# nanoporetech/scrappie

Measured on AMD Instinct MI355X. Metric: raw samples/sec, rgrgr_r94 4k-sample reads, higher is better.
Workload: dtype f32 (3xf16 split products, 22-bit operands, fp32 accumulate)

## Files before the change

### scrappie_amd/csrc/scrappie_hip.hip

```cpp
#include <hip/hip_runtime.h>
#include <sched.h>

#include <algorithm>
#include <atomic>
#include <cmath>
#include <cstdarg>
#include <cstdio>
#include <cstdlib>
#include <cstring>
#include <mutex>
#include <numeric>
#include <string>
#include <thread>
#include <type_traits>
#include <vector>
#include <chrono>
#include <condition_variable>
#include <deque>
#include <functional>
#include <map>
#include <memory>

#include "scrappie_hip.h"
#include "sh_internal.h"
// ... 223 lines not shown
        return tot;
    }
    bool create_events() {
        bool ok = true;
        for (auto &x : ev) ok &= hipEventCreate(&x) == hipSuccess;
        for (hipEvent_t *x : {&done, &kdone, &hdone, &pdone, &up}) ok &= hipEventCreateWithFlags(x, hipEventDisableTiming) == hipSuccess;
        return ok;
    }
    ~Slot() {
        for (auto &x : ev) if (x) (void)hipEventDestroy(x);
        for (hipEvent_t x : {done, kdone, hdone, pdone, up}) if (x) (void)hipEventDestroy(x);
    }
};

struct AltInput {
    const float *data = nullptr;
    std::vector<uint64_t> off;
    DBuf d_off;
    uint64_t key = 0; bool valid = false;
    explicit operator bool() const { return data != nullptr; }
    int set(const char *who, const float *d, const uint64_t *o, size_t n) {
        valid = false;
        if (!d) { data = nullptr; off.clear(); return 0; }
        if (!o || n == 0) return set_err("%s: no offsets", who);
        data = d; off.assign(o, o + n);
        return 0;
    }
};

struct scrappie_hip_engine {
    int device = 0;
    hipStream_t stream = nullptr;
    hipStream_t cstream = nullptr;
    hipStream_t ustream = nullptr;
    hipStream_t pstream = nullptr;
    size_t total_mem = (size_t)64 << 30;
    size_t max_launch_blocks = 0;
    std::vector<Model *> models;
    size_t max_launch_reads = 16384;
    bool profiling = false;
    scrappie_hip_timing timing{};
    bool ev_ok = false;
    Slot slots[2];
    int cur = 0;
    int oldest = 0;
    Slot &current() { return slots[cur]; }
    Slot &other(const Slot &sl) { return slots[&sl == &slots[0] ? 1 : 0]; }
    int index(const Slot &sl) const { return (int)(&sl - slots); }
    bool any_pending() const { return slots[0].pending || slots[1].pending; }
    void drain() {
        (void)sh_stream_wait(pstream); (void)sh_stream_wait(stream); (void)sh_stream_wait(cstream);
        slots[0].pending = slots[1].pending = false;
    }
    DBuf d_hstate, d_vstate, d_vflag;
    DBuf d_act[3];
    DBuf d_xaff, d_E, d_sums, d_tb, d_tbend, d_fstate;
    int ncu = 256;
    bool handover = true;
    AltInput alt_prob; DBuf d_Ealt, d_sums_alt;
    AltInput alt_trunk; DBuf d_act_alt;
    bool dbg_ff_separate = false;
    bool dbg_fv_single = false;
    bool dbg_dump_final = false;
    int dbg_fail_run = 0;
    bool dbg_redo_all = false;
    int dbg_gru_tiles = 0;
    bool dbg_force_f32 = false;
    int dbg_gru32 = -1;
    scrappie_hip_engine *tail = nullptr;
    scrappie_hip_engine *tail2 = nullptr;
    bool is_tail = false;
    int tail_mode = -1;
    int dbg_fail_tail = 0;
    double mem_frac = 0.7;
    struct Blob { std::string name; std::vector<unsigned char> bytes; bool force_f32; };
    std::vector<Blob> blobs;
    unsigned long long n_tail_calls = 0, n_tail_reads = 0;
    struct TailTicket {
        long id = 0; int model = 0; scrappie_hip_params p{};
        std::vector<raw_table> reads; std::vector<scrappie_hip_call> calls;
        std::vector<float> own;
        int rc = 0; std::string err; bool done = false;
    };
    std::thread tail_th, tail_th2;
    bool tail_th_live = false, tail_th2_live = false, tail_stop = false;
    int tail_busy = 0;
    std::mutex tail_mu;
    std::condition_variable tail_cv;
    std::deque<std::shared_ptr<TailTicket>> tail_q;
    std::map<long, std::shared_ptr<TailTicket>> tail_open;
    long tail_next = 1;
    unsigned long long n_redo_tail = 0;
    unsigned long long n_tail_groups = 0;
    unsigned host_thread_budget = 0;
    unsigned long long n_redo = 0;
    struct Carry { bool live = false; int slot = 0; std::vector<uint32_t> perm; scrappie_hip_call *out = nullptr; scrappie_hip_params p{}; } carry;
    std::mutex mu;
    double tail_frac = 0.3;
    double dbg_tail_free_frac = 0;
    BatchCoalescer batch_co;
    ShPresence batch_presence;
    PostStage post_stage[2]; unsigned post_turn = 0;
    HBuf h_dec_in, h_dec_out; DBuf d_dec[7];
    HBuf h_crf_in, h_crf_out; DBuf d_crf[4];
    DpBufs dp_map; DBuf d_map_seq, d_map_band, d_map_post;
    double map_ms[3] = {0, 0, 0};
    DpBufs dp_sq; DBuf d_sq_sig, d_sq_tab;
    double squig_ms[3] = {0, 0, 0};
    DBuf d_sqn[2]; HBuf h_sqn;
    double sqnet_ms[3] = {0, 0, 0};
    DBuf d_ev_sig, d_ev_rd, d_ev_sum, d_ev_sumsq, d_ev_t1, d_ev_t2, d_ev_peaks, d_ev_np, d_ev_off, d_ev_out; HBuf h_ev, h_ev_out;
    double event_ms[3] = {0, 0, 0};
    size_t dbg_events_budget = 0;
    size_t dbg_sqnet_budget = 0;
    size_t dbg_squig_budget = 0;
    std::mutex call_mu;
    ~scrappie_hip_engine() {
        for (Model *m : models) delete m;
        for (hipStream_t st : {stream, cstream, ustream, pstream}) if (st) (void)hipStreamDestroy(st);
// ... 121 lines not shown
```

### scrappie_amd/csrc/sh_decode.h

```cpp
#ifndef SH_DECODE_H
#define SH_DECODE_H

struct ShVitArgs {
    const float *E;
    const float *sums;
    long long strideT;
    int strideQ, strideB;
    int want_log;
    float min_prob, stay_pen, skip_pen, local_pen;
    int use_slip;
    unsigned *tb;
    int *tb_end;
    int *final_state;
    float *final_score;
    float *hp_side;
    const long long *hp_off;
    unsigned long long *dbg;
    const ShGruSegD *seg;
    float *vstate;
    unsigned *flag;
    unsigned *err;
    int dump_final;
};

__device__ __forceinline__ void argmax_merge(float &v, int &i, float ov, int oi) {
    const bool take = (ov > v) | ((ov == v) & (oi < i));
    v = take ? ov : v;
    i = take ? oi : i;
}

__device__ __forceinline__ void rows_argmax(float &bv, int &bi) {
    float ov = __shfl_xor(bv, 16); int oi = __shfl_xor(bi, 16);
    argmax_merge(bv, bi, ov, oi);
    ov = __shfl_xor(bv, 32); oi = __shfl_xor(bi, 32);
    argmax_merge(bv, bi, ov, oi);
}

#ifndef SH_FVT_GAP
#define SH_FVT_GAP 4.76837158203125e-07f
#endif
#ifndef SH_MAX4_ASM
#define SH_MAX4_ASM 1
#endif
__device__ __forceinline__ float d_max4(const f32x4 v) {
#if !SH_MAX4_ASM
    return __builtin_fmaxf(__builtin_fmaxf(v[0], v[1]), __builtin_fmaxf(v[2], v[3]));
#endif
    float t;
    asm("v_max3_f32 %0, %1, %2, %3" : "=v"(t) : "v"(v[0]), "v"(v[1]), "v"(v[2]));
    asm("v_max_f32 %0, %1, %2" : "=v"(t) : "v"(t), "v"(v[3]));
    return t;
}

#define SH_CODE_LT(E, codes, a, b, x)                                                                                       \
    asm("v_cmp_lt_f32 vcc, %1, %2\n\tv_cndmask_b32_sdwa %0, %0, %3, vcc dst_sel:BYTE_" #E                                   \
        " dst_unused:UNUSED_PRESERVE src0_sel:BYTE_" #E " src1_sel:BYTE_0"                                                  \
        : "+v"(codes) : "v"(a), "v"(b), "v"(x) : "vcc")

#ifndef SH_VIT_RING
#define SH_VIT_RING 4
#endif
template <int NTH, int PPT, bool FIN, bool SLIP, bool SKIP0>
__global__ __launch_bounds__(NTH, NTH / 256) void k_viterbi(ShVitArgs a, ShMeta md) {
    constexpr int RING = (PPT >= SH_VIT_RING) ? SH_VIT_RING : PPT;
    constexpr int QSTR = NTH / 16, NW = NTH / 64;
    constexpr int NQ = QSTR * PPT, NH = 4 * NQ;
    constexpr int NSKIP = NH / 16, NSLIP = (NH / 64 > 0) ? NH / 64 : 1;
    extern __shared__ __attribute__((aligned(16))) float smem[];
    float *scA = smem;
    float *scB = scA + NH * 16;
    float *skv = scB + NH * 16;
    int *ski = (int *)(skv + NSKIP * 16);
    float *slv = (float *)(ski + NSKIP * 16);
    int *sli = (int *)(slv + NSLIP * 16);
    float *redv = (float *)(sli + NSLIP * 16);
    int *redi = (int *)(redv + 2 * NW * 16);

    const int tid = threadIdx.x, b = tid & 15, qq = tid >> 4, wave = tid >> 6, lane = tid & 63;
    const float mp = a.min_prob, mpm1 = 1.0f - a.min_prob;
    const float slip_pen = (float)(2.0 * a.skip_pen);
    constexpr bool slip = SLIP && (NH / 64 > 0);
    unsigned long long vA = 0, vB = 0, vC = 0, vD = 0, vt0 = 0, vt1;
    long long vblocks = 0;
#define VSTAMP(acc) do { if (a.dbg) { vt1 = __builtin_readcyclecounter(); acc += vt1 - vt0; vt0 = vt1; } } while (0)

    int tile = blockIdx.x, s0 = 0, s1 = -1, ord = 0;
    if (a.seg) { const ShGruSegD sg = a.seg[blockIdx.x]; tile = sg.tile; s0 = sg.s0; s1 = sg.s1; ord = sg.pad; }
    tile = __builtin_amdgcn_readfirstlane(tile); s0 = __builtin_amdgcn_readfirstlane(s0); s1 = __builtin_amdgcn_readfirstlane(s1);
    const int Tt = __builtin_amdgcn_readfirstlane(md.tile_T[tile]);
    if (s1 < 0) s1 = Tt;
    const long long boff = __builtin_amdgcn_readfirstlane((int)md.tile_boff[tile]);
    const int rd = tile * 16 + b;
    const int myT = md.rT[rd];
    float pstart = 0.0f, pend = -SH_BIG;
    if (s0 == 0) {
#pragma unroll
        for (int i = 0; i < PPT; i++)
            *(f32x4 *)(scA + ((qq + QSTR * i) * 16 + b) * 4) = (f32x4){-SH_BIG, -SH_BIG, -SH_BIG, -SH_BIG};
        if (lane < 16) { redv[wave * 16 + b] = -SH_BIG - a.local_pen; redi[wave * 16 + b] = 4 * wave; }
    } else {
        if (tid == 0) {
            if (!sh_wait_flag(a.flag + tile, (unsigned)ord, a.err)) __hip_atomic_store(a.err, 1u, __ATOMIC_RELAXED, __HIP_MEMORY_SCOPE_AGENT);
        }
        __syncthreads();
        __builtin_amdgcn_fence(__ATOMIC_ACQUIRE, "agent");
        const float *vst = a.vstate + (long long)tile * (NH * 16 + 32);
        float bv = -INFINITY;
        int bi = 0x7fffffff;
#pragma unroll
        for (int i = 0; i < PPT; i++) {
            const int Q = qq + QSTR * i;
            const f32x4 pv = *(const f32x4 *)(vst + (Q * 16 + b) * 4);
            *(f32x4 *)(scA + (Q * 16 + b) * 4) = pv;
            {
                const float ve = __builtin_fmaxf(__builtin_fmaxf(pv[0], pv[1]), __builtin_fmaxf(pv[2], pv[3])) - a.local_pen;
                bi = (ve > bv) ? Q : bi;
                bv = __builtin_fmaxf(bv, ve);
            }
        }
        pstart = vst[NH * 16 + b];
        pend = vst[NH * 16 + 16 + b];
        float ov = __shfl_xor(bv, 16); int oi = __shfl_xor(bi, 16);
        argmax_merge(bv, bi, ov, oi);
        ov = __shfl_xor(bv, 32); oi = __shfl_xor(bi, 32);
        argmax_merge(bv, bi, ov, oi);
        if (lane < 16) { redv[((s0 & 1) * NW + wave) * 16 + b] = bv; redi[((s0 & 1) * NW + wave) * 16 + b] = bi; }
    }
    __syncthreads();
    float *cur = scA, *nxt = scB;

    f32x4 ring[RING];
    float stay_nx = 0.f, sum_nx = 1.f;
    float hp_nx[4] = {0.f, 0.f, 0.f, 0.f};
    const bool hp_lane = FIN && a.hp_side && qq == 0;
    auto fetch = [&](int t) {
        const float *Ecb = a.E + (boff + t) * a.strideT + b * a.strideB;
        stay_nx = Ecb[NQ * a.strideQ];
        if (FIN) sum_nx = a.sums[(boff + t) * 16 + b];
        if (hp_lane) {
#pragma unroll
// ... 259 lines not shown
#define SH_FV_LDS_FLOATS (2 * 1024 * 16 + 2 * 64 * 16 + 2 * 16 * 16 + 4 * 8 * 16 + 2 * 3 * 512 + 2 * 9 * 16 + 65 * 16 + 3 * 2 * 4 * 4)

template <bool SLIP, bool SKIP0, bool DIV>
__global__ __launch_bounds__(512, 2) void k_ff_viterbi(ShFfArgs f, ShVitArgs a, ShMeta md) {
    constexpr int NTH = 512, NW = 8, PPT = 8, NQ = 256, NH = 1024, NSKIP = NH / 16, NSLIP = NH / 64, KS = 3, KQ = 6;
    static_assert(PPT == SH_SUM_GROUP, "a wave's tiles are one row-sum group");
    extern __shared__ __attribute__((aligned(16))) float smem[];
    float *scA = smem;
    float *scB = scA + NH * 16;
    float *skv = scB + NH * 16;
    int *ski = (int *)(skv + NSKIP * 16);
    float *slv = (float *)(ski + NSKIP * 16);
    int *sli = (int *)(slv + NSLIP * 16);
    float *redv = (float *)(sli + NSLIP * 16);
    int *redi = (int *)(redv + 2 * NW * 16);
    unsigned *xp = (unsigned *)(redi + 2 * NW * 16);
    float *gsum = (float *)(xp + 2 * KS * 512);
    float *sBias = gsum + 2 * (NW + 1) * 16;
    unsigned *sStay = (unsigned *)(sBias + 65 * 16);

    const int tid = threadIdx.x, lane = tid & 63, b = lane & 15, q = lane >> 4;
    const int wave = __builtin_amdgcn_readfirstlane(tid >> 6);
    const float mp = a.min_prob, mpm1 = 1.0f - a.min_prob;
    const float slip_pen = (float)(2.0 * a.skip_pen);
    const float lbound = (mp > 0.0f) ? 1.0e-3f - __logf(mp) : INFINITY;
    unsigned long long vA = 0, vB = 0, vC = 0, vD = 0, vt0 = 0, vt1;
#if SH_FV_YOUNG_PRIO
    if (wave >= 4) __builtin_amdgcn_s_setprio(SH_FV_YOUNG_PRIO);
#endif

    const unsigned *wmine = f.wpiece + (long long)(PPT * wave) * KS * 512;
    ShSplit W[2][KS];
    const unsigned lofs = (unsigned)lane * 4u, tofs = (unsigned)lane;
    typedef const __attribute__((address_space(1))) unsigned *gu32;
    typedef const __attribute__((address_space(1))) u32x4 *gu32x4;
    gu32 wp = (gu32)wmine;
    auto w_load = [&](int i) {
        static_assert(KS == 3, "two bases per tile: immediate offsets reach 4095 bytes");
        gu32 b0 = wp, b1 = wp + 1024;
        asm volatile("" : "+s"(b0), "+s"(b1));
        W[i & 1][0].p1 = __builtin_bit_cast(f16x8, *(gu32x4)(b0 + lofs));
        W[i & 1][0].p2 = __builtin_bit_cast(f16x8, *(gu32x4)(b0 + 256 + lofs));
        W[i & 1][1].p1 = __builtin_bit_cast(f16x8, *(gu32x4)(b0 + 512 + lofs));
        W[i & 1][1].p2 = __builtin_bit_cast(f16x8, *(gu32x4)(b0 + 768 + lofs));
        W[i & 1][2].p1 = __builtin_bit_cast(f16x8, *(gu32x4)(b1 + lofs));
        W[i & 1][2].p2 = __builtin_bit_cast(f16x8, *(gu32x4)(b1 + 256 + lofs));
        wp = (i == PPT - 1) ? (gu32)wmine : wp + KS * 512;
        asm volatile("" : "+s"(wp));
    };
    if (tid < KS * 2 * 4 * 4) sStay[tid] = f.wpiece[(long long)(PPT * NW) * KS * 512 + (tid >> 4) * 256 + ((tid >> 2) & 3) * 64 + (tid & 3)];
    for (int j = tid; j < 65 * 16; j += NTH) sBias[j] = f.bfrag[((j >> 4) * 64 + ((j >> 2) & 3) * 16) * 4 + (j & 3)];

    int tile = blockIdx.x, s0 = 0, s1 = -1, ord = 0;
    if (a.seg) { const ShGruSegD sg = a.seg[blockIdx.x]; tile = sg.tile; s0 = sg.s0; s1 = sg.s1; ord = sg.pad; }
    tile = __builtin_amdgcn_readfirstlane(tile); s0 = __builtin_amdgcn_readfirstlane(s0); s1 = __builtin_amdgcn_readfirstlane(s1);
    const int Tt = __builtin_amdgcn_readfirstlane(md.tile_T[tile]);
    if (s1 < 0) s1 = Tt;
    const long long boff = __builtin_amdgcn_readfirstlane((int)md.tile_boff[tile]);
    const int rd = tile * 16 + b;
    const int myT = md.rT[rd];
    const long long hpo = a.hp_side ? a.hp_off[rd] : 0;
    float pstart = 0.0f, pend = -SH_BIG;
    if (s0 == 0) {
#pragma unroll
        for (int i = 0; i < PPT; i++)
            *(f32x4 *)(scA + ((32 * wave + 4 * i + q) * 16 + b) * 4) = (f32x4){-SH_BIG, -SH_BIG, -SH_BIG, -SH_BIG};
        if (lane < 16) { redv[wave * 16 + b] = -SH_BIG - a.local_pen; redi[wave * 16 + b] = 32 * wave; }
    } else {
        if (tid == 0) {
            if (!sh_wait_flag(a.flag + tile, (unsigned)ord, a.err)) __hip_atomic_store(a.err, 1u, __ATOMIC_RELAXED, __HIP_MEMORY_SCOPE_AGENT);
        }
        __syncthreads();
        __builtin_amdgcn_fence(__ATOMIC_ACQUIRE, "agent");
        const float *vst = a.vstate + (long long)tile * (NH * 16 + 32);
        float bv = -INFINITY;
        int bi = 0x7fffffff;
#pragma unroll
        for (int i = 0; i < PPT; i++) {
            const int Q = 32 * wave + 4 * i + q;
            const f32x4 pv = *(const f32x4 *)(vst + (Q * 16 + b) * 4);
            *(f32x4 *)(scA + (Q * 16 + b) * 4) = pv;
            {
                const float ve = __builtin_fmaxf(__builtin_fmaxf(pv[0], pv[1]), __builtin_fmaxf(pv[2], pv[3])) - a.local_pen;
                bi = (ve > bv) ? Q : bi;
                bv = __builtin_fmaxf(bv, ve);
            }
        }
        pstart = vst[NH * 16 + b];
        pend = vst[NH * 16 + 16 + b];
        float ov = __shfl_xor(bv, 16); int oi = __shfl_xor(bi, 16);
        argmax_merge(bv, bi, ov, oi);
        ov = __shfl_xor(bv, 32); oi = __shfl_xor(bi, 32);
        argmax_merge(bv, bi, ov, oi);
        if (lane < 16) { redv[((s0 & 1) * NW + wave) * 16 + b] = bv; redi[((s0 & 1) * NW + wave) * 16 + b] = bi; }
    }
    float *cur = scA, *nxt = scB;

    f32x4 xr0 = {0.f, 0.f, 0.f, 0.f}, xr1 = xr0;
    auto xraw_load = [&](int t) {
        if (wave < KS) {
            const float *p = f.in + ((boff + min(t, s1 - 1)) * KQ + 2 * wave) * 256;
            xr0 = *(const f32x4 *)(p + lofs);
            xr1 = *(const f32x4 *)(p + 256 + lofs);
        }
    };
    auto xp_publish = [&](int buf) {
        if (wave < KS) {
// ... 476 lines not shown
```

### scrappie_amd/csrc/sh_decode_teams.h

```cpp
#ifndef SH_DECODE_TEAMS_H
#define SH_DECODE_TEAMS_H

#ifndef SH_FVT_WBUF
#define SH_FVT_WBUF 3
#endif
#ifndef SH_FVT_PROD_PRIO
#define SH_FVT_PROD_PRIO 1
#endif
#ifndef SH_FVT_ABL
#define SH_FVT_ABL 0
#endif
#ifndef SH_FVT_FLIP
#define SH_FVT_FLIP 3
#endif
#ifndef SH_FVT_STAMP
#ifdef SH_EXPERIMENTS
#define SH_FVT_STAMP 1
#else
#define SH_FVT_STAMP 0
#endif
#endif
__device__ __forceinline__ unsigned long long end_key(float v, int i) {
    const unsigned u = __builtin_bit_cast(unsigned, v);
    const unsigned hi = u ^ ((unsigned)((int)u >> 31) | 0x80000000u);
    return ((unsigned long long)hi << 32) | (unsigned)~i;
}
__device__ __forceinline__ void end_unkey(unsigned long long k, float &v, int &i) {
    const unsigned hi = (unsigned)(k >> 32);
    v = __builtin_bit_cast(float, hi ^ (~(unsigned)((int)hi >> 31) | 0x80000000u));
    i = (int)~(unsigned)k;
}

#define SH_FVT_NTH 768
#define SH_FVT_LDS_FLOATS (1024 * 16 + 64 * 256 + 2 * 64 * 16 + 2 * 2 * 8 * 16 + 4 * 9 * 16 + 65 * 16 + 2 * 3 * 512 + 3 * 2 * 4 * 4)

template <bool SKIP0, bool DIV, bool NOCLAMP = false>
__global__ __launch_bounds__(SH_FVT_NTH) void k_ff_viterbi_teams(ShFfArgs f, ShVitArgs a, ShMeta md) {
    static_assert(!(DIV && NOCLAMP), "with temperatures the clamp stays");
    constexpr int NCW = 8, NPW = 4, PPT = 8, NQ = 256, NH = 1024, KS = 3, KQ = 6, TPP = 16, HT = 8, NG = 9, WB = SH_FVT_WBUF;
    static_assert(SH_SUM_GROUP == HT, "half a pass of a producer is one row-sum group");
    static_assert(WB >= 2 && WB <= 4, "weight ring");
    extern __shared__ __attribute__((aligned(16))) float smem[];
    float *sc = smem;
    float *ring = sc + NH * 16;
    float *skk = ring + 64 * 256;
    float *redv = skk + 2 * 64 * 16;
    int *redi = (int *)(redv + 2 * NCW * 16);
    typedef __attribute__((address_space(3))) unsigned long long *ldsk;
    ldsk redk = (ldsk)redv;
    float *gsum = (float *)(redi + 2 * NCW * 16);
    float *sBias = gsum + 4 * NG * 16;
    unsigned *xp = (unsigned *)(sBias + 65 * 16);
    unsigned *sStay = xp + 2 * KS * 512;

    const int tid = threadIdx.x, lane = tid & 63, b = lane & 15, q = lane >> 4;
    const int wave = __builtin_amdgcn_readfirstlane(tid >> 6);
    const bool decoder = wave < NCW;
    const float mp = a.min_prob, mpm1 = 1.0f - a.min_prob;
    const float lbound = (mp > 0.0f) ? 1.0e-3f - __logf(mp) : INFINITY;
    const float lbgap = lbound * SH_FVT_GAP;
    unsigned long long vA = 0, vB = 0, vC = 0, vD = 0, vt0 = 0, vt1 = 0;
    (void)vt0; (void)vt1;
#undef VSTAMP
#if SH_FVT_STAMP
#define VSTAMP(acc) do { if (a.dbg) { vt1 = __builtin_readcyclecounter(); acc += vt1 - vt0; vt0 = vt1; } } while (0)
#else
#define VSTAMP(acc) do { } while (0)
#endif

    if (tid < KS * 2 * 4 * 4) sStay[tid] = f.wpiece[(long long)(64) * KS * 512 + (tid >> 4) * 256 + ((tid >> 2) & 3) * 64 + (tid & 3)];
    for (int j = tid; j < 65 * 16; j += SH_FVT_NTH) sBias[j] = f.bfrag[((j >> 4) * 64 + ((j >> 2) & 3) * 16) * 4 + (j & 3)];

    int tile = blockIdx.x, s0 = 0, s1 = -1, ord = 0;
    if (a.seg) { const ShGruSegD sg = a.seg[blockIdx.x]; tile = sg.tile; s0 = sg.s0; s1 = sg.s1; ord = sg.pad; }
    tile = __builtin_amdgcn_readfirstlane(tile); s0 = __builtin_amdgcn_readfirstlane(s0); s1 = __builtin_amdgcn_readfirstlane(s1);
    const int Tt = __builtin_amdgcn_readfirstlane(md.tile_T[tile]);
    if (s1 < 0) s1 = Tt;
    const long long boff = __builtin_amdgcn_readfirstlane((int)md.tile_boff[tile]);
    const int rd = tile * 16 + b;
    int myT = md.rT[rd];
    asm volatile("" : "+v"(myT));
    const long long hpo = a.hp_side ? a.hp_off[rd] : 0;
    float pstart = 0.0f, pend = -SH_BIG;

    const int cw = decoder ? wave : 0;
    float *myq = sc + cw * 256 + lane * 4;
    const float *mye = ring + cw * 512 + lane * 4;
    const float *mysrc = sc + cw * 64 + b * 4 + q;
#define SH_FVT_MT(i) (16 * ((i) >> 1) + 8 * ((i) & 1))

    if (s0 == 0) {
        if (decoder) {
#pragma unroll
            for (int i = 0; i < PPT; i++) *(f32x4 *)(myq + SH_FVT_MT(i) * 256) = (f32x4){-SH_BIG, -SH_BIG, -SH_BIG, -SH_BIG};
            if (wave == 0 && lane < 16) { redk[b] = end_key(-SH_BIG - a.local_pen, 0); redk[16 + b] = 0; }
        }
    } else {
        if (tid < 32) redk[tid] = 0;
        if (tid == 0) {
            if (!sh_wait_flag(a.flag + tile, (unsigned)ord, a.err)) __hip_atomic_store(a.err, 1u, __ATOMIC_RELAXED, __HIP_MEMORY_SCOPE_AGENT);
        }
        __syncthreads();
        __builtin_amdgcn_fence(__ATOMIC_ACQUIRE, "agent");
        if (decoder) {
            const float *vst = a.vstate + (long long)tile * (NH * 16 + 32);
            float bv = -INFINITY;
            int bi = 0x7fffffff;
#pragma unroll
            for (int i = 0; i < PPT; i++) {
                const int Q = 4 * (SH_FVT_MT(i) + cw) + q;
                const f32x4 pv = *(const f32x4 *)(vst + (Q * 16 + b) * 4);
                *(f32x4 *)(myq + SH_FVT_MT(i) * 256) = pv;
                {
                    const float ve = __builtin_fmaxf(__builtin_fmaxf(pv[0], pv[1]), __builtin_fmaxf(pv[2], pv[3])) - a.local_pen;
                    bi = (ve > bv) ? Q : bi;
                    bv = __builtin_fmaxf(bv, ve);
                }
            }
            pstart = vst[NH * 16 + b];
            pend = vst[NH * 16 + 16 + b];
            float ov = __shfl_xor(bv, 16); int oi = __shfl_xor(bi, 16);
            argmax_merge(bv, bi, ov, oi);
            ov = __shfl_xor(bv, 32); oi = __shfl_xor(bi, 32);
            argmax_merge(bv, bi, ov, oi);
            if (lane < 16) __hip_atomic_fetch_max(redk + b, end_key(bv, bi), __ATOMIC_RELAXED, __HIP_MEMORY_SCOPE_WORKGROUP);
        }
    }
// ... 437 lines not shown
```

### scrappie_amd/csrc/sh_eng_batch.inc

```

#ifndef SH_CHAIN_NS
#define SH_CHAIN_NS 11400.0
#endif
#ifndef SH_WORK_NS
#define SH_WORK_NS 3.5
#endif
extern "C" long scrappie_hip_plan_tail(const uint32_t *lengths, size_t n, int stride, size_t max_long_blocks, unsigned char *is_long) {
    if ((!lengths && n) || stride < 1 || !is_long) return -1;
    memset(is_long, 0, n);
    if (n < 2) return 0;
    double W = 0;
    std::vector<uint32_t> T(n);
    for (size_t i = 0; i < n; i++) { T[i] = (uint32_t)(((unsigned long long)lengths[i] + stride - 1) / stride); W += T[i]; }
    const double thr = std::max(4096.0, W * SH_WORK_NS / SH_CHAIN_NS);
    std::vector<uint32_t> cand;
    for (size_t i = 0; i < n; i++) if ((double)T[i] > thr) cand.push_back((uint32_t)i);
    if (cand.empty() || cand.size() == n) return 0;
    std::stable_sort(cand.begin(), cand.end(), [&](uint32_t a, uint32_t b) { return T[a] > T[b]; });
    double blocks = 0, work = 0;
    long cnt = 0;
    for (size_t k = 0; k < cand.size(); k++) {
        if (k % 16 == 0) { if (max_long_blocks && blocks + T[cand[k]] > (double)max_long_blocks) break; blocks += T[cand[k]]; }
        if (work + T[cand[k]] > 0.15 * W) break;
        work += T[cand[k]];
        is_long[cand[k]] = 1; cnt++;
    }
    return cnt;
}

static int basecall_batch_one(scrappie_hip_engine *e, int model, const raw_table *reads, size_t n, const scrappie_hip_params *p, scrappie_hip_call *out);

static bool tail_two_helpers();
static double tail_mem_frac() {
    static const double f = [] { const char *v = getenv("SCRAPPIE_HIP_TAIL_MEM"); const double x = v ? atof(v) : 0; return x > 0 && x <= 0.4 ? x : (tail_two_helpers() ? 0.15 : 0.3); }();
    return f;
}
static bool tail_two_helpers() {
    static const bool on = [] { const char *v = getenv("SCRAPPIE_HIP_TAIL"); return v && atoi(v) == 2; }();
    return on;
}
static bool tail_enabled(const scrappie_hip_engine *e) {
    if (e->is_tail) return false;
    if (e->tail_mode >= 0) return e->tail_mode != 0;
    static const bool env_on = [] { const char *v = getenv("SCRAPPIE_HIP_TAIL"); return !(v && atoi(v) == 0); }();
    return env_on;
}

static scrappie_hip_engine *make_helper(scrappie_hip_engine *e) {
    scrappie_hip_engine *t = scrappie_hip_engine_create(e->device);
    if (!t) return nullptr;
    t->is_tail = true;
    for (const auto &b : e->blobs) {
        t->dbg_force_f32 = b.force_f32;
        const int want = scrappie_hip_find_model(e, b.name.c_str());
        if (load_model_mem_one(t, b.name.c_str(), b.bytes.data(), b.bytes.size()) != want) { scrappie_hip_engine_destroy(t); set_err("helper engine: model '%s' did not load at index %d", b.name.c_str(), want); return nullptr; }
    }
    return t;
}
static void sync_helper(scrappie_hip_engine *e, scrappie_hip_engine *t) {
    t->handover = e->handover; t->max_launch_reads = e->max_launch_reads; t->max_launch_blocks = e->max_launch_blocks;
    t->dbg_ff_separate = e->dbg_ff_separate; t->dbg_fv_single = e->dbg_fv_single; t->dbg_gru32 = e->dbg_gru32; t->dbg_gru_tiles = e->dbg_gru_tiles; t->dbg_redo_all = e->dbg_redo_all;
    t->profiling = false;
}
static scrappie_hip_engine *tail_engine(scrappie_hip_engine *e) {
    if (!e->tail) {
        (void)hipSetDevice(e->device);
        double frac = tail_mem_frac();
        size_t fr = 0, tot = 0;
        if (hipMemGetInfo(&fr, &tot) == hipSuccess && e->total_mem) frac = std::min(frac, 0.85 * (double)fr / (double)e->total_mem);
        if (e->dbg_tail_free_frac > 0) frac = std::min(frac, e->dbg_tail_free_frac);
        if (frac < 0.03) { e->tail_mode = 0; return nullptr; }
        e->tail = make_helper(e);
        if (!e->tail) return nullptr;
        e->mem_frac = 0.45; e->tail->mem_frac = frac; e->tail_frac = frac;
    }
    std::lock_guard<std::mutex> lk(e->tail_mu);
    if (e->tail_busy == 0) {
        sync_helper(e, e->tail);
        if (e->tail2) sync_helper(e, e->tail2);
        if (e->dbg_fail_tail) { e->tail->dbg_fail_run = e->dbg_fail_tail; e->dbg_fail_tail = 0; }
    }
    return e->tail;
}

typedef std::shared_ptr<scrappie_hip_engine::TailTicket> TicketPtr;
static void tail_worker(scrappie_hip_engine *e, scrappie_hip_engine *helper) {
    for (;;) {
        std::unique_lock<std::mutex> lk(e->tail_mu);
        e->tail_cv.wait(lk, [&] { return e->tail_stop || !e->tail_q.empty(); });
        if (e->tail_q.empty()) break;
        std::vector<TicketPtr> batch;
        const TicketPtr f = e->tail_q.front();
        while (!e->tail_q.empty() && e->tail_q.front()->model == f->model && memcmp(&e->tail_q.front()->p, &f->p, sizeof f->p) == 0) {
            batch.push_back(e->tail_q.front());
            e->tail_q.pop_front();
        }
        e->tail_busy++;
        lk.unlock();
        std::vector<raw_table> all;
        for (const TicketPtr &t : batch) all.insert(all.end(), t->reads.begin(), t->reads.end());
        std::vector<scrappie_hip_call> calls(all.size());
        const int rc = basecall_batch_one(helper, f->model, all.data(), all.size(), &f->p, calls.data());
        const std::string err = rc ? std::string(g_err) : std::string();
        lk.lock();
        size_t at = 0;
        for (const TicketPtr &t : batch) {
            t->rc = rc; t->err = err;
            if (!rc) t->calls.assign(calls.begin() + (long)at, calls.begin() + (long)(at + t->reads.size()));
            at += t->reads.size();
            t->done = true;
        }
        e->n_tail_groups++;
        e->n_redo_tail += helper->n_redo; helper->n_redo = 0;
        e->tail_busy--;
// ... 442 lines not shown
```

### scrappie_amd/csrc/sh_eng_debug.inc

```

extern "C" int scrappie_hip_set_decoder_input(scrappie_hip_engine *e, const float *d_prob, const uint64_t *prob_off, size_t n_prob) {
    if (!e) return set_err("set_decoder_input: null engine");
    if (e->any_pending()) return set_err("set_decoder_input: launch groups are in flight");
    return e->alt_prob.set("set_decoder_input", d_prob, prob_off, n_prob);
}

extern "C" int scrappie_hip_set_trunk_input(scrappie_hip_engine *e, const float *d_trunk, const uint64_t *trunk_off, size_t n_trunk) {
    if (!e) return set_err("set_trunk_input: null engine");
    if (e->any_pending()) return set_err("set_trunk_input: launch groups are in flight");
    return e->alt_trunk.set("set_trunk_input", d_trunk, trunk_off, n_trunk);
}

extern "C" int scrappie_hip_debug_option(scrappie_hip_engine *e, const char *name, int value) {
    if (!e || !name) return set_err("debug_option: null argument");
    if (e->any_pending()) return set_err("debug_option: launch groups are in flight");
    if (!strcmp(name, "ff_separate")) e->dbg_ff_separate = value != 0;
    else if (!strcmp(name, "fv_single")) e->dbg_fv_single = value != 0;
    else if (!strcmp(name, "dump_final")) e->dbg_dump_final = value != 0;
    else if (!strcmp(name, "fail_run")) e->dbg_fail_run = value;
    else if (!strcmp(name, "redo_all")) e->dbg_redo_all = value != 0;
    else if (!strcmp(name, "gru_tiles")) e->dbg_gru_tiles = value;
    else if (!strcmp(name, "force_f32_layers")) e->dbg_force_f32 = value != 0;
#ifdef SH_EXPERIMENTS
    else if (!strcmp(name, "gru32")) e->dbg_gru32 = value;
#endif
    else if (!strcmp(name, "tail")) e->tail_mode = value;
    else if (!strcmp(name, "fail_tail")) e->dbg_fail_tail = value;
    else if (!strcmp(name, "tail_free_frac")) e->dbg_tail_free_frac = value / 1000.0;
    else if (!strcmp(name, "squiggle_budget_kb")) e->dbg_squig_budget = value > 0 ? (size_t)value << 10 : 0;
    else if (!strcmp(name, "sqnet_budget_kb")) e->dbg_sqnet_budget = value > 0 ? (size_t)value << 10 : 0;
    else if (!strcmp(name, "events_budget_samples")) e->dbg_events_budget = value > 0 ? (size_t)value : 0;
    else return set_err("debug_option: unknown option '%s'", name);
    return 0;
}

extern "C" long long scrappie_hip_debug_fetch(scrappie_hip_engine *e, const char *what, void *dst, size_t nbytes) {
    if (!e || !what) return set_err("debug_fetch: null argument");
    (void)hipSetDevice(e->device);
    HIPCHK(sh_stream_wait(e->stream));
    HIPCHK(sh_stream_wait(e->cstream));
    const Slot &sl = e->current(); const LaunchGroup &lg = sl.lg;
    if (!lg.valid) return set_err("debug_fetch: no launch group has run");
    Model *m = get_model(e, lg.model);
    if (!m) return -1;
    const size_t NH = (size_t)std::max(m->NS - 1, 0);
    const void *src = nullptr; size_t have = 0; bool host = false;
    const int gru_tiles = lg.gru_two ? 2 : 1;
    if (!strcmp(what, "tb")) { src = e->d_tb.p; have = (size_t)lg.ncb * NH * 16; }
    else if (!strcmp(what, "tb_end")) { src = e->d_tbend.p; have = (size_t)lg.ncb * 16 * 4; }
    else if (!strcmp(what, "final_state")) { src = e->d_fstate.p; have = lg.npad * 4; }
    else if (!strcmp(what, "final_score")) { src = sl.d_fscore.p; have = lg.npad * 4; }
    else if (!strcmp(what, "final_scores")) { src = e->d_vstate.p; have = lg.ntile * (NH * 16 + 32) * 4; }
    else if (!strcmp(what, "order")) { src = lg.order.data(); have = lg.npad * 4; host = true; }
    else if (!strcmp(what, "tile_boff")) { src = lg.tile_boff.data(); have = lg.ntile * 8; host = true; }
    else if (!strcmp(what, "n_redo")) { static thread_local unsigned long long tot; tot = e->n_redo + e->n_redo_tail; src = &tot; have = 8; host = true; }
    else if (!strcmp(what, "n_tail_groups")) { src = &e->n_tail_groups; have = 8; host = true; }
    else if (!strcmp(what, "n_tail_calls")) { src = &e->n_tail_calls; have = 8; host = true; }
    else if (!strcmp(what, "n_tail_reads")) { src = &e->n_tail_reads; have = 8; host = true; }
    else if (!strcmp(what, "gru_tiles")) { src = &gru_tiles; have = 4; host = true; }
    else if (!strcmp(what, "pinned_bytes")) {
        static thread_local unsigned long long tot;
        tot = e->slots[0].pinned_bytes() + e->slots[1].pinned_bytes();
        src = &tot; have = 8; host = true;
    }
    else return set_err("debug_fetch: unknown buffer '%s'", what);
    if (!src && have) return set_err("debug_fetch: buffer '%s' was not allocated", what);
    const size_t cnt = std::min(have, nbytes);
    if (dst && cnt) {
        if (host) memcpy(dst, src, cnt);
        else HIPCHK(hipMemcpy(dst, src, cnt, hipMemcpyDeviceToHost));
    }
    return (long long)have;
}

// ... 48 lines not shown
```

### scrappie_amd/csrc/sh_eng_launch.inc

```

struct MetaPtrs { ShMeta md; const long long *seq_off, *hp_off, *bases_off; ShGruLanes lanes, lanes1; ShGruPairs pairs, pairs2; const ShGruSegD *vseg; };

static int build_group(scrappie_hip_engine *e, Slot &sl, Model *m, const uint64_t *offsets, const uint32_t *lengths,
                       size_t n, bool hp_on, MetaPtrs &mp) {
    LaunchGroup &lg = sl.lg;
    lg.valid = false;
    lg.n = n; lg.hp_on = hp_on;
    lg.ntile = (n + 15) / 16; lg.npad = lg.ntile * 16;
    const int st = m->stride;
    std::vector<int> T(n);
    for (size_t i = 0; i < n; i++)
        T[i] = (lengths[i] >= m->min_samples) ? (int)((lengths[i] + st - 1) / st) : 0;
    lg.order.assign(lg.npad, -1);
    std::vector<int> idx(n);
    std::iota(idx.begin(), idx.end(), 0);
    std::stable_sort(idx.begin(), idx.end(), [&](int a, int b) { return T[a] > T[b]; });
    for (size_t i = 0; i < n; i++) lg.order[i] = idx[i];
    lg.rT.assign(lg.npad, 0); lg.rN.assign(lg.npad, 0);
    lg.seq_off.assign(lg.npad, 0); lg.hp_off.assign(lg.npad, 0); lg.bases_off.assign(lg.npad, 0);
    long long nbases = 0;
    const long long per_entry = (m->arch == 1) ? 1 : 5;
    std::vector<unsigned long long> sig_off(lg.npad, 0);
    std::vector<int> tile_T(lg.ntile, 0);
    std::vector<long long> &tile_boff = lg.tile_boff;
    tile_boff.assign(lg.ntile, 0);
    long long ncb = 0, nseq = 0, nhp = 0;
    for (size_t i = 0; i < lg.npad; i++) {
        const int o = lg.order[i];
        if (o >= 0 && T[o] > 0) {
            lg.rT[i] = T[o]; lg.rN[i] = (int)lengths[o]; sig_off[i] = offsets[o];
        }
        lg.hp_off[i] = nhp; nhp += lg.rT[i];
        lg.bases_off[i] = nbases; nbases += lg.rT[i] ? ((per_entry * ((long long)lg.rT[i] + 1) + 16 + 15) & ~15ll) : 0;
        tile_T[i >> 4] = std::max(tile_T[i >> 4], lg.rT[i]);
    }
    for (size_t t = 0; t < lg.ntile; t++) { tile_boff[t] = ncb; ncb += tile_T[t]; }
    for (size_t t = 0; t < lg.ntile; t++) {
        for (int b = 0; b < 16; b++) lg.seq_off[t * 16 + b] = nseq + b;
        nseq += tile_T[t] ? ((long long)tile_T[t] + 1) * SH_SEQ_STRIDE : 0;
    }
    lg.ncb = ncb; lg.nseq = nseq; lg.nhp = nhp; lg.nbases_cap = nbases;
    ShGruSchedule sched;
    sh_lane_schedule(tile_T.data(), lg.ntile, e->ncu, 2, sched, e->handover);
    lg.gru_nwg = sched.nwg;
    ShGruSchedule sched1;
    sh_lane_schedule(tile_T.data(), lg.ntile, e->ncu, 1, sched1, e->handover);
    lg.gru1_nwg = sched1.nwg;
    { long long nlive = 0; int tmax = 0; for (int t : tile_T) { nlive += t > 0; tmax = std::max(tmax, t); }
      const int w1 = sched1.wg_iter.empty() ? 0 : *std::max_element(sched1.wg_iter.begin(), sched1.wg_iter.end());
      const int w2 = sched.wg_iter.empty() ? 0 : *std::max_element(sched.wg_iter.begin(), sched.wg_iter.end());
      lg.gru_two = nlive > e->ncu && tmax < 65536 && (double)w2 * tun().gru_two_ratio < (double)w1;
      if (e->dbg_gru_tiles == 1) lg.gru_two = false;
      if (e->dbg_gru_tiles == 2 && tmax < 65536) lg.gru_two = true; }
    std::vector<int> pair_tile, pair_T;
    for (size_t t = 0; t < lg.ntile; ) {
        const bool two = t + 1 < lg.ntile && tile_T[t] < (1 << 18) && tile_T[t + 1] > 0;
        pair_tile.push_back((int)t); pair_tile.push_back(two ? (int)t + 1 : -1);
        pair_T.push_back(std::max(tile_T[t], two ? tile_T[t + 1] : 0));
        t += two ? 2 : 1;
    }
    ShGruSchedule sched32;
    sh_lane_schedule(pair_T.data(), pair_T.size(), e->ncu, 1, sched32, e->handover);
    lg.gru32_nwg = sched32.nwg;
    ShGruSchedule sched32b;
    sh_lane_schedule(pair_T.data(), pair_T.size(), e->ncu, 2, sched32b, e->handover);
    lg.gru32x2_nwg = sched32b.nwg;
    std::vector<ShGruSeg> vseg;
    sh_piece_schedule(tile_T.data(), lg.ntile, e->ncu, vseg, e->handover);
    lg.vit_nwg = (int)vseg.size();
    const size_t b_u64 = lg.npad * 8, b_i32 = lg.npad * 4;
    const size_t b_loff = sched.lane_off.size() * 4, b_seg = sched.seg.size() * sizeof(ShGruSeg), b_wit = sched.wg_iter.size() * 4;
    const size_t b_vloff = 0, b_vseg = vseg.size() * sizeof(ShGruSeg);
    const size_t b_loff1 = sched1.lane_off.size() * 4, b_seg1 = sched1.seg.size() * sizeof(ShGruSeg);
    const size_t b_loff32 = sched32.lane_off.size() * 4, b_seg32 = sched32.seg.size() * sizeof(ShGruSeg), b_pt = pair_tile.size() * 4;
    const size_t b_loff32b = sched32b.lane_off.size() * 4, b_seg32b = sched32b.seg.size() * sizeof(ShGruSeg);
    const size_t total = 4 * b_u64 + lg.ntile * 8 + 2 * b_i32 + lg.ntile * 4 + 16 + b_seg + b_loff + b_wit + 16 + b_vseg + b_vloff + 16 + b_seg1 + b_loff1 +
                         16 + b_seg32 + b_loff32 + b_pt + 16 + b_seg32b + b_loff32b;
    if (sl.h_meta.ensure(total + 16) || sl.d_meta.ensure(total + 16)) return -1;
    char *h = sl.h_meta.as<char>();
    size_t o = 0;
    memcpy(h + o, sig_off.data(), b_u64); const size_t o_sig = o; o += b_u64;
    memcpy(h + o, lg.seq_off.data(), b_u64); const size_t o_seq = o; o += b_u64;
    memcpy(h + o, lg.hp_off.data(), b_u64); const size_t o_hp = o; o += b_u64;
    memcpy(h + o, lg.bases_off.data(), b_u64); const size_t o_bs = o; o += b_u64;
    memcpy(h + o, tile_boff.data(), lg.ntile * 8); const size_t o_tb = o; o += lg.ntile * 8;
    memcpy(h + o, lg.rN.data(), b_i32); const size_t o_n = o; o += b_i32;
    memcpy(h + o, lg.rT.data(), b_i32); const size_t o_t = o; o += b_i32;
    memcpy(h + o, tile_T.data(), lg.ntile * 4); const size_t o_tt = o; o += lg.ntile * 4;
    o = (o + 15) & ~(size_t)15;
    memcpy(h + o, sched.seg.data(), b_seg); const size_t o_seg = o; o += b_seg;
    memcpy(h + o, sched.lane_off.data(), b_loff); const size_t o_loff = o; o += b_loff;
    memcpy(h + o, sched.wg_iter.data(), b_wit); const size_t o_wit = o; o += b_wit;
    o = (o + 15) & ~(size_t)15;
    memcpy(h + o, vseg.data(), b_vseg); const size_t o_vseg = o; o += b_vseg;
    o = (o + 15) & ~(size_t)15;
    memcpy(h + o, sched1.seg.data(), b_seg1); const size_t o_seg1 = o; o += b_seg1;
    memcpy(h + o, sched1.lane_off.data(), b_loff1); const size_t o_loff1 = o; o += b_loff1;
    o = (o + 15) & ~(size_t)15;
    memcpy(h + o, sched32.seg.data(), b_seg32); const size_t o_seg32 = o; o += b_seg32;
    memcpy(h + o, sched32.lane_off.data(), b_loff32); const size_t o_loff32 = o; o += b_loff32;
    memcpy(h + o, pair_tile.data(), b_pt); const size_t o_pt = o; o += b_pt;
    o = (o + 15) & ~(size_t)15;
    memcpy(h + o, sched32b.seg.data(), b_seg32b); const size_t o_seg32b = o; o += b_seg32b;
    memcpy(h + o, sched32b.lane_off.data(), b_loff32b); const size_t o_loff32b = o; o += b_loff32b;
    hipStream_t ps = e->ev_ok ? e->pstream : e->stream;
    if (e->ev_ok) {
        const long long n16 = (long long)((total + 15) / 16);
        hipLaunchKernelGGL(k_upload_words, dim3((unsigned)std::min<long long>((n16 + 255) / 256, 64)), dim3(256), 0, ps, (const u32x4 *)h, sl.d_meta.as<u32x4>(), n16);
    } else HIPCHK(hipMemcpyAsync(sl.d_meta.p, h, total, hipMemcpyHostToDevice, ps));
    char *d = sl.d_meta.as<char>();
    mp.md.sig_off = (const unsigned long long *)(d + o_sig);
    mp.seq_off = (const long long *)(d + o_seq);
    mp.hp_off = (const long long *)(d + o_hp);
    mp.bases_off = (const long long *)(d + o_bs);
    mp.md.tile_boff = (const long long *)(d + o_tb);
    mp.md.rN = (const int *)(d + o_n);
    mp.md.rT = (const int *)(d + o_t);
    mp.md.tile_T = (const int *)(d + o_tt);
    static_assert(sizeof(ShGruSeg) == sizeof(ShGruSegD), "segment layout");
    mp.lanes.seg = (const ShGruSegD *)(d + o_seg);
    mp.lanes.lane_off = (const int *)(d + o_loff);
    mp.lanes.wg_iter = (const int *)(d + o_wit);
    mp.lanes.ntile = (int)lg.ntile;
    mp.vseg = (const ShGruSegD *)(d + o_vseg);
    if (e->d_hstate.ensure(std::max<size_t>(lg.ntile, 1) * 12 * 256 * 4) || sl.d_gflag.ensure((lg.ntile + 1) * 4)) return -1;
    mp.lanes.hstate = e->d_hstate.as<float>();
    mp.lanes.flag = sl.d_gflag.as<unsigned>();
    HIPCHK(hipMemsetAsync(sl.d_gflag.p, 0, (lg.ntile + 1) * 4, ps));
    if (sl.d_bad.ensure(lg.npad * 4)) return -1;
    HIPCHK(hipMemsetAsync(sl.d_bad.p, 0, lg.npad * 4, ps));
    mp.lanes1 = mp.lanes;
    mp.lanes1.seg = (const ShGruSegD *)(d + o_seg1);
    mp.lanes1.lane_off = (const int *)(d + o_loff1);
    mp.lanes1.wg_iter = nullptr;
    mp.pairs.seg = (const ShGruSegD *)(d + o_seg32);
    mp.pairs.lane_off = (const int *)(d + o_loff32);
    mp.pairs.pair_tile = (const int *)(d + o_pt);
    mp.pairs.hstate = mp.lanes.hstate;
    mp.pairs.flag = mp.lanes.flag;
    mp.pairs.err = mp.lanes.flag + lg.ntile;
    mp.pairs2 = mp.pairs;
    mp.pairs2.seg = (const ShGruSegD *)(d + o_seg32b);
    mp.pairs2.lane_off = (const int *)(d + o_loff32b);
    return 0;
}

template <int KQ>
static int launch_affine_k(hipStream_t s, const float *in, float *out, const float *wf, const unsigned *wp, const float *bf,
                           long long ncb, int mtiles) {
    const int mt = pick_mt(mtiles);
    long long gx = std::min<long long>((ncb + 3) / 4, 2048);
    if (gx < 1) gx = 1;
    dim3 grid((unsigned)gx, (unsigned)(mtiles / mt));
    int rc = 0;
    if (pick_int<6, 4, 3, 2, 1>(mt, rc, [&](auto m) { return launch_k<k_affine<KQ, m()>>(grid, dim3(256), 0, s, in, out, wf, wp, bf, ncb, mtiles); })) return rc;
    return set_err("unsupported layer of %d m-tiles", mtiles);
}

template <int KQ>
static int launch_affine_lds_k(hipStream_t s, const float *in, float *out, const float *wf, const unsigned *wp, const float *bf,
                               long long ncb, int mtiles) {
    constexpr int NB = SH_AFF_NB, NTH = SH_AFF_NTH;
    const size_t lds = ((size_t)mtiles * KQ * 256 + (size_t)mtiles * 256) * 4 + 16;
    long long gx = std::min<long long>((ncb + (NTH / 64) * NB - 1) / ((NTH / 64) * NB), 256);
    if (gx < 1) gx = 1;
    return launch_k<k_affine_lds<KQ, NB, NTH>>(dim3((unsigned)gx), dim3(NTH), lds, s, in, out, wf, wp, bf, ncb, mtiles);
}

template <int KQ>
static int launch_affine_f32_k(hipStream_t s, const float *in, float *out, const float *wf, const float *bf, long long ncb, int mtiles) {
    const int mt = (mtiles % 6 == 0) ? 6 : (mtiles % 2 == 0) ? 2 : 1;
    long long gx = std::min<long long>((ncb + 3) / 4, 2048);
    if (gx < 1) gx = 1;
    dim3 grid((unsigned)gx, (unsigned)(mtiles / mt));
    int rc = 0;
    if (pick_int<6, 2, 1>(mt, rc, [&](auto m) { return launch_k<k_affine<KQ, m(), true>>(grid, dim3(256), 0, s, in, out, wf, (const unsigned *)nullptr, bf, ncb, mtiles); })) return rc;
    return set_err("unsupported layer of %d m-tiles", mtiles);
}

static int launch_affine(hipStream_t s, int K, const float *in, float *out, const float *wf, const unsigned *wp, const float *bf_nat,
                         const float *bf_acc, long long ncb, int mtiles, bool force_f32 = false) {
    int rc = 0;
    if (force_f32 && pick_int<2, 4, 6, 8>(K / 16, rc, [&](auto kq) { return launch_affine_f32_k<kq()>(s, in, out, wf, bf_nat, ncb, mtiles); })) return rc;
    if (K % 32 == 0 && (!wp || !bf_acc)) return set_err("layer weights were not cut into pieces (input size %d)", K);
    const float *bf = (K % 32 == 0) ? bf_acc : bf_nat;
    const size_t lds_need = ((size_t)mtiles * (K / 16) * 256 + (size_t)mtiles * 256) * 4;
    if (mtiles >= 12 && lds_need <= 150 * 1024 && ncb >= 4096 && !tun().affine_reg &&
        pick_int<1, 2, 4, 6>(K / 16, rc, [&](auto kq) { return launch_affine_lds_k<kq()>(s, in, out, wf, wp, bf, ncb, mtiles); })) return rc;
    if (pick_int<1, 2, 4, 6, 8>(K / 16, rc, [&](auto kq) { return launch_affine_k<kq()>(s, in, out, wf, wp, bf, ncb, mtiles); })) return rc;
    return set_err("unsupported layer input size %d (need 16, 32, 64, 96 or 128)", K);
}

template <int KQ>
static int launch_affine2_k(hipStream_t s, const float *inF, const float *inB, float *out, const unsigned *wF, const unsigned *wB,
                            const float *bf, long long ncb, int mtiles) {
    long long gx = std::min<long long>((ncb + 3) / 4, 2048);
    if (gx < 1) gx = 1;
    const int mt = mtiles / 2;
    int rc = 0;
    if (mt * 2 == mtiles &&
        pick_int<3, 2, 1>(mt, rc, [&](auto m) { return launch_k<k_affine2_tanh<KQ, m()>>(dim3((unsigned)gx), dim3(512), 0, s, inF, inB, out, wF, wB, bf, ncb, mtiles); })) return rc;
    return set_err("unsupported joining layer of %d m-tiles", mtiles);
}

static int launch_affine2(hipStream_t s, int K, const float *inF, const float *inB, float *out, const unsigned *wF, const unsigned *wB,
                          const float *bf, long long ncb, int mtiles) {
    int rc = 0;
    if (pick_int<2, 4, 6>(K / 16, rc, [&](auto kq) { return launch_affine2_k<kq()>(s, inF, inB, out, wF, wB, bf, ncb, mtiles); })) return rc;
    return set_err("unsupported bi-GRU size %d (need 32, 64 or 96)", K);
}

static int launch_gru(hipStream_t s, int S, const float *xaff, float *out, const float *resid, const float *sW,
                      const float *sW2, const unsigned *sWp, const unsigned *sW2p, const ShMeta &md, int backward, size_t ntile, const ShGruLanes &lanes, int nwg,
                      bool force_f32 = false) {
    const int NU = S / 16;
    int rc = 0;
    if (!tun().gru_single && !tun().gru_stamp && tun().gru_debug < 0 && NU <= 6 && S % 32 == 0) {
        if (nwg <= 0) return 0;
        HIPCHK(hipMemsetAsync(lanes.flag, 0, (size_t)lanes.ntile * 4, s));
        dim3 lgrid((unsigned)nwg);
        const bool stamp = tun().gru_lanes_stamp;
        const bool f32_env = tun().gru_f32 || force_f32;
        if (!stamp && !f32_env) {
            const size_t plds = (size_t)2 * 2 * (NU / 2) * 2 * 64 * 4 * 4;
            if (pick_int<2, 4, 6>(NU, rc, [&](auto nu) { return launch_k<k_gru_split<nu()>>(lgrid, dim3(128 * nu()), plds, s, xaff, out, resid, sWp, sW2p, md, backward, lanes); })) return rc;
            return set_err("unsupported GRU size %d (need 32, 64 or 96 here)", S);
        }
        const size_t lds = (size_t)2 * 2 * NU * 256 * 4;
        static StampBuf st;
        if (!pick_int<2, 4, 6>(NU, rc, [&](auto nu) {
#ifdef SH_EXPERIMENTS
            if constexpr (nu() == 6)
                if (stamp) return launch_k<k_gru_lanes<6, true>>(lgrid, dim3(768), lds, s, xaff, out, resid, sW, sW2, md, backward, lanes, st.dev(4096 * 16 * 8));
#endif
            return launch_k<k_gru_lanes<nu(), false>>(lgrid, dim3(128 * nu()), lds, s, xaff, out, resid, sW, sW2, md, backward, lanes, (unsigned long long *)nullptr);
            })) return set_err("unsupported GRU size %d (need 32, 64 or 96 here)", S);
        if (stamp && NU == 6)
            st.dump_on(7, s, (size_t)nwg * 12 * 8, [&](const unsigned long long *h) {
                for (size_t g : {(size_t)nwg / 2}) for (int w = 0; w < 12; w++) {
                    const unsigned long long *d = &h[(g * 12 + w) * 8];
                    fprintf(stderr, "gru lanes stamp wg %zu wave %2d: phase1 %.0f bar %.0f phase2 %.0f bar %.0f cycles/step (%llu steps)\n",
                            g, w, d[0] / (double)d[4], d[1] / (double)d[4], d[2] / (double)d[4], d[3] / (double)d[4], d[4]);
                }
            });
        return rc;
    }
    if (tun().gru_debug >= 0) backward |= tun().gru_debug << 8;
    static StampBuf st1;
    unsigned long long *dbgbuf = tun().gru_stamp ? st1.dev(4096 * 8 * 8) : nullptr;
    if (dbgbuf)
        st1.dump_on(8, s, ntile * NU * 8, [&](const unsigned long long *h) {
            { unsigned long long first_end = ~0ull, mn = ~0ull, mx = 0; size_t late = 0;
              for (size_t tl = 0; tl < ntile; tl++) { first_end = std::min(first_end, h[tl * NU * 8 + 7]); mn = std::min(mn, h[tl * NU * 8 + 6]); mx = std::max(mx, h[tl * NU * 8 + 7]); }
              for (size_t tl = 0; tl < ntile; tl++) if (h[tl * NU * 8 + 6] >= first_end) late++;
              fprintf(stderr, "residency: %zu tiles, %zu started after the first one finished; span %.1f us\n", ntile, late, (mx - mn) / 100.0); }
            for (size_t tl : {size_t(0)}) for (int w = 0; w < 1; w++) {
                const unsigned long long *d = &h[(tl * NU + w) * 8];
                fprintf(stderr, "stamp tile %zu wave %d: rgemm %.0f zgemm+valu %.0f bar1 %.0f gemm2+valu %.0f bar2 %.0f (cycles/step)\n", tl, w, d[0] / (double)d[5], d[1] / (double)d[5], d[2] / (double)d[5], d[3] / (double)d[5], d[4] / (double)d[5]);
            }
        });
    if (pick_int<2, 4, 6, 8>(NU, rc, [&](auto nu) { return launch_k<k_gru<nu()>>(dim3((unsigned)ntile), dim3(64 * nu()), 0, s, xaff, out, resid, sW, sW2, md, backward, dbgbuf); })) return rc;
    return set_err("unsupported GRU size %d (need 32, 64, 96 or 128)", S);
}

#ifndef SH_FFL_NB
#define SH_FFL_NB 3
#endif
#ifndef SH_FFL_NTH
#define SH_FFL_NTH 512
#endif
static int ff_mtp(int KQ, int mtiles) {
    const size_t per_mt = ((size_t)KQ * 256 + 256) * 4;
// ... 25 lines not shown
}

static int launch_ff(hipStream_t s, int S, const float *in, float *E, float *sums, const unsigned *wf, const float *bf,
                     long long ncb, int mtiles, int NS, float in_div, float out_div, int ncu) {
    int rc = 0;
    if (ncb >= 8192 && !tun().ff_reg &&
        pick_int<2, 4, 6>(S / 16, rc, [&](auto kq) { return launch_ff_lds_k<kq()>(s, in, E, sums, wf, bf, ncb, mtiles, NS, in_div, out_div, ncu); })) return rc;
    constexpr int NB = SH_FF_NB;
    const int mtp = ff_mtp(S / 16, mtiles);
    const long long gx = (ncb + 4 * NB - 1) / (4 * NB);
    dim3 grid((unsigned)std::max<long long>(gx, 1));
    if (pick_int<2, 4, 6, 8>(S / 16, rc, [&](auto kq) {
            constexpr int KQ = kq();
            return pick_bool([&](auto dv) { return launch_k<k_ff_exp<KQ, NB, dv()>>(grid, dim3(256), 0, s, in, E, sums, wf, bf, ncb, mtiles, mtp, NS, in_div, out_div); },
                             out_div != 1.0f);
        })) return rc;
    return set_err("unsupported size %d", S);
}

static bool gru_proj_ok(int K, int S) { return K == S && S % 32 == 0 && S / 16 <= 6; }

static bool conv_edge_words(const ShConvGeom &g, int N, int T, int out[4]) {
    out[0] = out[1] = out[2] = out[3] = 0;
    if (T <= 0) return true;
    unsigned irr = 0;
    bool ok = true;
    for (int t = std::max(g.c0, T - 64); t < T; t++) {
        const int kk = (t - g.c0) / g.nstepC, ii = (t - g.c0) - kk * g.nstepC;
        if (!((kk + 1) * g.nstepX <= N - g.shiftX - ii * g.st)) {
            const int j = T - 1 - t;
            if (j >= 32) ok = false; else irr |= 1u << j;
        }
    }
    const int maxCol = (N - g.shiftX) / g.nstepX;
    const int rem = (N - g.shiftX) % g.nstepX;
    const int colR = g.c0 + g.nstepC * (maxCol - 1) + rem / g.st + 1;
    const int startR = g.st - (g.padL + N - g.WL) % g.st - 1;
    out[0] = (int)irr; out[1] = colR + startR / g.st; out[2] = startR; out[3] = N;
    return ok;
}

extern "C" int scrappie_hip_conv_edge_words(int WL, int st, int F, int N, int out[4]) {
    if (WL < 1 || st < 1 || N < 1 || !out) return -1;
    return conv_edge_words(conv_geom(WL, st, F), N, (N + st - 1) / st, out) ? 1 : 0;
}

#ifdef SH_EXPERIMENTS
static int launch_gru_conv(hipStream_t s, int kst, int act, float *out, const unsigned *iW, const float *ib, const unsigned *sW,
                           const unsigned *sW2, const ShMeta &md, int backward, const ShGruLanes &lanes1, int nwg1,
                           const ShGruLanes &lanes2, int nwg2, bool two, const ShConvFuse &cf) {
    const ShGruLanes &lanes = two ? lanes2 : lanes1;
    const int nwg = two ? nwg2 : nwg1;
    if (nwg <= 0) return 0;
    HIPCHK(hipMemsetAsync(lanes.flag, 0, (size_t)lanes.ntile * 4, s));
    const size_t lds = (two ? 2 : 1) * ((size_t)4 * 3 * 2 * 64 * 4 + (size_t)2 * 3 * 6 * 256) * 4;
    dim3 grid((unsigned)nwg);
    if (tun().proj_stamp && two && kst == 3 && !act) {
        static StampBuf st;
        if (launch_k<k_gru_conv_stamp<2, 3, 0>>(grid, dim3(768), lds, s, out, iW, ib, sW, sW2, md, backward, lanes, cf, st.dev(1024 * 12 * 16))) return -1;
        st.dump_on(3, s, (size_t)nwg * 12 * 16, [&](const unsigned long long *h) {
            for (int w = 0; w < 12; w++) {
                const unsigned long long *d = &h[((size_t)(nwg / 2) * 12 + w) * 16];
                fprintf(stderr, "conv-layer stamp wave %2d (%s): A %.0f bar %.0f B %.0f bar %.0f cycles per double step (%llu steps); chunk+fetch part of B (projection) / reads+MFMA issue (recurrence) %.0f\n", w,
                        w < 6 ? "recurrence" : "projection", d[0] / (double)d[4], d[1] / (double)d[4], d[2] / (double)d[4], d[3] / (double)d[4], d[4], d[5] / (double)d[4]);
            }
        });
        return 0;
    }
    return pick_bool([&](auto t2, auto k3, auto ac) {
        return launch_k<k_gru_conv<t2() ? 2 : 1, k3() ? 3 : 5, ac() ? 1 : 0>>(grid, dim3(768), lds, s, out, iW, ib, sW, sW2, md, backward, lanes, cf);
    }, two, kst == 3, act != 0);
}
#endif
static int launch_gru_proj(hipStream_t s, int S, const float *in, float *out, const float *resid, const unsigned *iW, const float *ib,
                           const unsigned *sW, const unsigned *sW2, const ShMeta &md, int backward, const ShGruLanes &lanes1, int nwg1,
                           const ShGruLanes &lanes2, int nwg2, bool two) {
    const ShGruLanes &lanes = two ? lanes2 : lanes1;
    const int nwg = two ? nwg2 : nwg1;
    if (nwg <= 0) return 0;
    HIPCHK(hipMemsetAsync(lanes.flag, 0, (size_t)lanes.ntile * 4, s));
    const int NU = S / 16;
    size_t lds = (two ? 2 : 1) * ((size_t)4 * (NU / 2) * 2 * 64 * 4 + (size_t)2 * 3 * NU * 256) * 4;
    if (resid && SH_RESID_LDS && lds + (size_t)(two ? 2 : 1) * 3 * NU * 256 * 4 <= 160 * 1024) lds += (size_t)(two ? 2 : 1) * 3 * NU * 256 * 4;
    dim3 grid((unsigned)nwg);
    unsigned long long *const no_dbg = nullptr;
    int rc = 0;
#ifdef SH_EXPERIMENTS
    static const bool mx_on = [] { const char *v = getenv("SH_GRU_MX"); return v && atoi(v) != 0; }();
    if (mx_on && NU == 6 && two) {
        static const bool mx_stamp = getenv("SH_MX_STAMP") != nullptr;
        if (mx_stamp && !resid) {
            static StampBuf st;
            if (launch_k<k_gru_mx<false, true>>(grid, dim3(1024), lds, s, in, out, resid, iW, ib, sW, sW2, md, backward, lanes, st.dev((size_t)1024 * 16 * 10))) return -1;
            st.dump_on(7, s, (size_t)nwg * 16 * 10, [&](const unsigned long long *hb) {
                for (int w = 0; w < 16; w++) {
                    const unsigned long long *d = &hb[((size_t)(nwg / 2) * 16 + w) * 10];
                    const double n = (double)std::max<unsigned long long>(d[8], 1);
                    fprintf(stderr, "mx stamp wave %2d (%s): P1 %.0f +bar %.0f | P2 %.0f +bar %.0f | P3 %.0f +bar %.0f | P4 %.0f +bar %.0f cycles per double step (%llu steps)\n", w,
                            w < 6 ? "recurrence " : w < 12 ? "projection " : "elementwise", d[0] / n, d[1] / n, d[2] / n, d[3] / n, d[4] / n, d[5] / n, d[6] / n, d[7] / n, d[8]);
                }
            });
            return 0;
        }
        if (pick_bool([&](auto rs) { return launch_k<k_gru_mx<rs()>>(grid, dim3(1024), lds, s, in, out, resid, iW, ib, sW, sW2, md, backward, lanes, no_dbg); }, resid != nullptr))
            return -1;
        HIPCHK(hipGetLastError());
        return 0;
    }
    const bool stamp = tun().proj_stamp && NU == 6 && two && !resid;
    const bool free_run = SH_GRU_FREE_DEFAULT ? !tun().gru_barrier : tun().gru_free;
    if (free_run) {
        const size_t flds = (two ? 2 : 1) * ((size_t)4 * (NU / 2) * 2 * 64 * 4 + (size_t)3 * 3 * NU * 256) * 4 + 64;
        if (stamp) {
            static StampBuf st;
            if (launch_k<k_gru_free<6, 2, false, true>>(grid, dim3(768), flds, s, in, out, resid, iW, ib, sW, sW2, md, backward, lanes, st.dev(1024 * 12 * 16))) return -1;
            st.dump_on(7, s, (size_t)nwg * 12 * 16, [&](const unsigned long long *h) {
                for (int w = 0; w < 12; w++) {
                    const unsigned long long *d = &h[((size_t)(nwg / 2) * 12 + w) * 16];
                    if (w < 6) fprintf(stderr, "free stamp wave %2d (recurrence): work %.0f, waiting for gate inputs %.0f, for r*h of all waves %.0f, for h of all waves %.0f cycles per double step (%llu steps)\n",
                                       w, d[0] / (double)d[4], d[1] / (double)d[4], d[2] / (double)d[4], d[3] / (double)d[4], d[4]);
                    else fprintf(stderr, "free stamp wave %2d (projection): work %.0f, waiting for the column's pieces %.0f, for a free ring slot %.0f cycles per double step (%llu steps)\n",
                                 w, d[0] / (double)d[4], d[1] / (double)d[4], d[2] / (double)d[4], d[4]);
                }
            });
            return 0;
        }
        if (pick_int<2, 4, 6>(NU, rc, [&](auto nu) {
                constexpr int N = nu();
                return pick_bool([&](auto t2, auto rs) {
                    return launch_k<k_gru_free<N, t2() ? 2 : 1, rs(), false>>(grid, dim3(128 * N), flds, s, in, out, resid, iW, ib, sW, sW2, md, backward, lanes, no_dbg);
                }, two, resid != nullptr);
            })) return rc;
        return set_err("unsupported GRU size %d (need 32, 64 or 96 here)", S);
    }
    if (stamp) {
        static StampBuf st;
        if (launch_k<k_gru_proj<6, 2, false, true>>(grid, dim3(768), lds, s, in, out, resid, iW, ib, sW, sW2, md, backward, lanes, st.dev(1024 * 12 * 16))) return -1;
        st.dump_on(7, s, (size_t)nwg * 12 * 16, [&](const unsigned long long *h) {
            for (int w = 0; w < 12; w++) {
                const unsigned long long *d = &h[((size_t)(nwg / 2) * 12 + w) * 16];
                fprintf(stderr, "proj stamp wave %2d (%s): A %.0f bar %.0f B %.0f bar %.0f cycles per double step (%llu steps)", w, w < 6 ? "recurrence" : "projection",
                        d[0] / (double)d[4], d[1] / (double)d[4], d[2] / (double)d[4], d[3] / (double)d[4], d[4]);
                if (w < 6) fprintf(stderr, "; inside B: reads+MFMA issue %.0f, logistic z %.0f, tanh+blend %.0f, store+bookkeeping %.0f, cut+publish %.0f",
                                   d[5] / (double)d[4], d[6] / (double)d[4], d[7] / (double)d[4], d[8] / (double)d[4], d[9] / (double)d[4]);
                fprintf(stderr, "\n");
            }
        });
        return 0;
    }
#endif
    if (pick_int<2, 4, 6>(NU, rc, [&](auto nu) {
            constexpr int N = nu();
            return pick_bool([&](auto t2) {
                constexpr int NT = t2() ? 2 : 1;
                if (resid) return launch_k<k_gru_proj_res<N, NT>>(grid, dim3(128 * N), lds, s, in, out, resid, iW, ib, sW, sW2, md, backward, lanes);
                return launch_k<k_gru_proj<N, NT, false>>(grid, dim3(128 * N), lds, s, in, out, resid, iW, ib, sW, sW2, md, backward, lanes, no_dbg);
            }, two);
        })) return rc;
    return set_err("unsupported GRU size %d (need 32, 64 or 96 here)", S);
}

#ifdef SH_EXPERIMENTS
#ifndef SH_GRU32_DEFAULT
#define SH_GRU32_DEFAULT 0
#endif
static int use_gru32(const scrappie_hip_engine *e) {
    if (e->dbg_gru32 >= 0) return e->dbg_gru32;
    if (SH_GRU32_DEFAULT ? tun().gru16 : !tun().gru32) return 0;
    const char *v = getenv("SH_GRU32");
    return (v && atoi(v) == 2) ? 2 : (SH_GRU32_DEFAULT ? SH_GRU32_DEFAULT : 1);
}
static const char *const g32_role[8] = {"R0 chain", "R1 chain", "R2 chain", "C cand-proj", "G0 z/r", "G1 z/r", "G2 z/r", "L loader"};
static int launch_gru_proj32x2(hipStream_t s, const float *in, float *out, bool resid, const unsigned *iW, const float *ib, const unsigned *sW,
                               const unsigned *sW2, const ShMeta &md, int backward, const ShGruPairs &pairs, int nwg, size_t ntile) {
    if (nwg <= 0) return 0;
    HIPCHK(hipMemsetAsync(pairs.flag, 0, ntile * 4, s));
    const size_t lds = (size_t)SH_G32X2_LDS_WORDS * 4;
    dim3 grid((unsigned)nwg);
    if (tun().gru32_stamp && !resid) {
        static StampBuf st;
        if (launch_k<k_gru_proj32x2<false, true>>(grid, dim3(512), lds, s, in, out, iW, ib, sW, sW2, md, backward, pairs, st.dev(1024 * 8 * 16))) return -1;
        st.dump_on(7, s, (size_t)nwg * 8 * 16, [&](const unsigned long long *h) {
            for (int w = 0; w < 8; w++) {
                const unsigned long long *d = &h[((size_t)(nwg / 2) * 8 + w) * 16];
                fprintf(stderr, "gru32x2 stamp wave %d (%s): work %.0f bar %.0f cycles per interval (%llu intervals = one tile-step of 32 reads each)\n", w, g32_role[w],
                        d[0] / (double)d[4], d[1] / (double)d[4], d[4]);
            }
        });
        return 0;
    }
    return pick_bool([&](auto rs) { return launch_k<k_gru_proj32x2<rs(), false>>(grid, dim3(512), lds, s, in, out, iW, ib, sW, sW2, md, backward, pairs, (unsigned long long *)nullptr); }, resid);
}
static int launch_gru_proj32(hipStream_t s, const float *in, float *out, bool resid, const unsigned *iW, const float *ib, const unsigned *sW,
                             const unsigned *sW2, const ShMeta &md, int backward, const ShGruPairs &pairs, int nwg, size_t ntile) {
    if (nwg <= 0) return 0;
    HIPCHK(hipMemsetAsync(pairs.flag, 0, ntile * 4, s));
    const size_t lds = (size_t)SH_G32_LDS_WORDS * 4;
    dim3 grid((unsigned)nwg);
    if (tun().gru32_stamp && !resid) {
        static StampBuf st;
        if (launch_k<k_gru_proj32<false, true>>(grid, dim3(512), lds, s, in, out, iW, ib, sW, sW2, md, backward, pairs, st.dev(1024 * 8 * 16))) return -1;
        st.dump_on(7, s, (size_t)nwg * 8 * 16, [&](const unsigned long long *h) {
            for (int w = 0; w < 8; w++) {
                const unsigned long long *d = &h[((size_t)(nwg / 2) * 8 + w) * 16];
                fprintf(stderr, "gru32 stamp wave %d (%s): A %.0f bar %.0f B %.0f bar %.0f cycles per step (%llu steps)", w, g32_role[w],
                        d[0] / (double)d[4], d[1] / (double)d[4], d[2] / (double)d[4], d[3] / (double)d[4], d[4]);
                if (w < 3) fprintf(stderr, "; A: reads+r products %.0f, logistic*h %.0f, cut+write %.0f; B: reads+candidate products %.0f, z/tanh/blend %.0f, store %.0f, cut+write %.0f",
                                   d[5] / (double)d[4], d[6] / (double)d[4], d[7] / (double)d[4], d[8] / (double)d[4], d[9] / (double)d[4], d[10] / (double)d[4], d[11] / (double)d[4]);
                fprintf(stderr, "\n");
            }
        });
        return 0;
    }
    return pick_bool([&](auto rs) { return launch_k<k_gru_proj32<rs(), false>>(grid, dim3(512), lds, s, in, out, iW, ib, sW, sW2, md, backward, pairs, (unsigned long long *)nullptr); }, resid);
}

#endif
static int launch_lstm(hipStream_t s, int S, const float *xaff, float *out, const unsigned *sW, const float *pf,
                       const ShMeta &md, int backward, const ShGruLanes &lanes, int nwg) {
    if (nwg <= 0) return 0;
    HIPCHK(hipMemsetAsync(lanes.flag, 0, (size_t)lanes.ntile * 4, s));
    int rc = 0;
    if (pick_int<2, 4, 6>(S / 16, rc, [&](auto nu) { return launch_k<k_lstm_lanes<nu()>>(dim3((unsigned)nwg), dim3(128 * nu()), 0, s, xaff, out, sW, pf, md, backward, lanes); })) return rc;
    return set_err("unsupported LSTM size %d (need 32, 64 or 96)", S);
}

static int launch_lstm_proj(hipStream_t s, int S, int I, const float *in, float *out, const unsigned *iW, const float *ib,
                            const unsigned *sW, const float *pf, const ShMeta &md, int backward, const ShGruLanes &lanes, int nwg) {
    if (nwg <= 0) return 0;
    HIPCHK(hipMemsetAsync(lanes.flag, 0, (size_t)lanes.ntile * 4, s));
    const int NU = S / 16;
    const size_t lds = ((size_t)4 * (NU / 2) * 2 * 64 * 4 + (size_t)2 * 4 * NU * 256 + (size_t)3 * NU * 256) * 4;
    if (I != S && I != 16) return set_err("unsupported LSTM input width %d", I);
    int rc = 0;
    if (pick_int<2, 4, 6>(NU, rc, [&](auto nu) {
            constexpr int N = nu();
            return pick_bool([&](auto wide) { return launch_k<k_lstm_proj<N, wide() ? N : 1>>(dim3((unsigned)nwg), dim3(128 * N), lds, s, in, out, iW, ib, sW, pf, md, backward, lanes); },
                             I == S);
        })) return rc;
    return set_err("unsupported LSTM size %d (need 32, 64 or 96)", S);
}

static size_t viterbi_lds_bytes(int NH) {
    const int nskip = NH / 16, nslip = std::max(NH / 64, 1);
    return (size_t)NH * 16 * 4 * 2 + (size_t)nskip * 16 * 8 + (size_t)nslip * 16 * 8 + 2 * 16 * 16 * 8;
}

static int launch_viterbi(hipStream_t s, int NH, const ShVitArgs &a, const ShMeta &md, size_t nwg) {
    const size_t lds = viterbi_lds_bytes(NH);
    if (nwg == 0) return 0;
    const bool fin = a.sums != nullptr, slip = a.use_slip != 0, skip0 = a.skip_pen == 0.0f;
    if (fin && !a.want_log) return set_err("decode: exp-value input implies log output");
    const auto go = [&](auto nth, auto ppt) {
        constexpr int NTH = nth(), PPT = ppt();
        return pick_bool([&](auto fi, auto sl, auto sk) { return launch_k<k_viterbi<NTH, PPT, fi(), sl(), sk()>>(dim3((unsigned)nwg), dim3(NTH), lds, s, a, md); },
                         fin, slip, skip0);
    };
    switch (NH) {
    case 64: return go(int_c<256>(), int_c<1>());
    case 256: return go(int_c<256>(), int_c<4>());
    case 1024:
#ifdef SH_EXPERIMENTS
        if (getenv("SH_VIT_1024")) return go(int_c<1024>(), int_c<4>());
#endif
        return go(int_c<512>(), int_c<8>());
    default: return set_err("unsupported transducer state count %d (need 4^3, 4^4 or 4^5 k-mers)", NH);
    }
}

static int launch_ff_viterbi(hipStream_t s, const ShFfArgs &f, const ShVitArgs &a, const ShMeta &md, size_t nwg, bool single) {
    const size_t lds = (size_t)SH_FV_LDS_FLOATS * 4;
    if (nwg == 0) return 0;
    dim3 grid((unsigned)nwg);
    const bool slip = a.use_slip != 0, skip0 = a.skip_pen == 0.0f, dv = f.out_div != 1.0f || f.in_div != 1.0f;
    if (!a.use_slip && !single) {
        const size_t ldt = (size_t)SH_FVT_LDS_FLOATS * 4;
        static const bool keep_clamp = getenv("SH_FVT_KEEP_CLAMP") != nullptr;
        const bool nc = f.no_clamp && !dv && !keep_clamp;
        return pick_bool([&](auto sk, auto d, auto n) {
            if constexpr (d() && n()) return -1;
            else return launch_k<k_ff_viterbi_teams<sk(), d(), n()>>(grid, dim3(SH_FVT_NTH), ldt, s, f, a, md);
        }, skip0, dv, nc);
    }
// ... 3 lines not shown
```

### scrappie_amd/csrc/sh_eng_load.inc

```

static const HostMat *find_mat(const std::vector<std::pair<std::string, HostMat>> &ms, const char *nm) {
    for (auto &kv : ms) if (kv.first == nm) return &kv.second;
    return nullptr;
}

static int load_model_mem_one(scrappie_hip_engine *e, const char *name, const void *blob, size_t nbytes);
static int sqnet_load(Model *m, const std::vector<std::pair<std::string, HostMat>> &mats);
extern "C" int scrappie_hip_load_model_mem(scrappie_hip_engine *e, const char *name, const void *blob, size_t nbytes) {
    const int idx = load_model_mem_one(e, name, blob, nbytes);
    if (idx < 0 || e->is_tail) return idx;
    scrappie_hip_engine::Blob b{name, std::vector<unsigned char>((const unsigned char *)blob, (const unsigned char *)blob + nbytes), e->dbg_force_f32};
    bool found = false;
    for (auto &x : e->blobs) if (x.name == b.name) { x = b; found = true; }
    if (!found) e->blobs.push_back(b);
    if (e->tail || e->tail2) {
        std::unique_lock<std::mutex> lk(e->tail_mu);
        e->tail_cv.wait(lk, [&] { return e->tail_busy == 0 && e->tail_q.empty(); });
    }
    for (scrappie_hip_engine **tp : {&e->tail, &e->tail2}) if (*tp) {
        (*tp)->dbg_force_f32 = e->dbg_force_f32;
        if (load_model_mem_one(*tp, name, blob, nbytes) != idx) return set_err("model '%s' did not load at the same index on the helper engine", name);
    }
    return idx;
}
// ... 178 lines not shown
    m->min_samples = (size_t)(g.shiftX + 2 * g.nstepX + g.WL);
    if (m->min_samples < (size_t)(g.st + 1)) m->min_samples = (size_t)(g.st + 1);
    }
    std::lock_guard<std::mutex> lk(e->mu);
    for (size_t i = 0; i < e->models.size(); i++)
        if (e->models[i]->name == name) { delete e->models[i]; e->models[i] = m; return (int)i; }
    e->models.push_back(m);
    return (int)e->models.size() - 1;
}

extern "C" int scrappie_hip_load_model(scrappie_hip_engine *e, const char *name, const char *path) {
    if (!path) return set_err("load_model: null path");
    FILE *fh = fopen(path, "rb");
    if (!fh) return set_err("cannot open model file %s", path);
    fseek(fh, 0, SEEK_END);
    long sz = ftell(fh);
    fseek(fh, 0, SEEK_SET);
    std::vector<unsigned char> buf((size_t)std::max(0L, sz));
    const size_t got = fread(buf.data(), 1, buf.size(), fh);
    fclose(fh);
    if (got != buf.size()) return set_err("short read on %s", path);
    return scrappie_hip_load_model_mem(e, name, buf.data(), buf.size());
}

extern "C" int scrappie_hip_find_model(scrappie_hip_engine *e, const char *name) {
    if (!e || !name) return -1;
    std::lock_guard<std::mutex> lk(e->mu);
    for (size_t i = 0; i < e->models.size(); i++) if (e->models[i]->name == name) return (int)i;
    return -1;
}

static Model *get_model(scrappie_hip_engine *e, int model) {
    if (!e || model < 0 || (size_t)model >= e->models.size()) { set_err("invalid model handle %d", model); return nullptr; }
    if (e->models[model]->arch == 4) { set_err("model '%s' predicts squiggles from sequences; it takes no signal", e->models[model]->name.c_str()); return nullptr; }
    return e->models[model];
}

extern "C" size_t scrappie_hip_min_samples(scrappie_hip_engine *e, int model) {
    Model *m = get_model(e, model);
    return m ? m->min_samples : 0;
}
extern "C" int scrappie_hip_model_stride(scrappie_hip_engine *e, int model) {
    Model *m = get_model(e, model);
    return m ? m->stride : -1;
}
extern "C" void scrappie_hip_set_profiling(scrappie_hip_engine *e, int on) { if (e) e->profiling = on != 0; }
static int resolve_spans(scrappie_hip_engine *e, Slot &sl) {
    scrappie_hip_timing &tm = sl.timing;
    float dbg_wait = 0.f, dbg_lead = 0.f;
    float *fields[F_COUNT] = {&tm.conv_ms, &tm.affine_ms, &tm.gru_ms, &tm.ff_ms, &tm.decode_ms, &tm.backtrace_ms, &tm.total_ms, &tm.fused_ms, &tm.stitch_ms,
                              &dbg_wait, &dbg_lead};
    for (auto &sp : sl.spans) {
        float ms = 0;
        HIPCHK(hipEventElapsedTime(&ms, sl.ev[sp.i], sl.ev[sp.j]));
        *fields[sp.field] += ms;
    }
    sl.spans.clear();
    if (tun().host_stamp) fprintf(stderr, "host stamp: main stream waited %.2f ms for the prologue; the convolution had ended %.2f ms before the main stream got there (negative: after)\n", dbg_wait, dbg_lead);
    e->timing = tm;
    return 0;
}

extern "C" int scrappie_hip_get_timing(scrappie_hip_engine *e, scrappie_hip_timing *t) {
    if (!e || !t) return -1;
    (void)hipSetDevice(e->device);
    Slot &sl = e->current();
    if (!sl.spans.empty() && !sl.pending) {
        HIPCHK(sh_stream_wait(e->stream));
        if (resolve_spans(e, sl)) return -1;
    }
    *t = e->timing;
    return 0;
}
extern "C" void scrappie_hip_set_max_launch_reads(scrappie_hip_engine *e, size_t n) { if (e && n >= 16) e->max_launch_reads = n; }
extern "C" void scrappie_hip_set_max_launch_blocks(scrappie_hip_engine *e, size_t n) { if (e) e->max_launch_blocks = n; }
extern "C" void *scrappie_hip_device_alloc(scrappie_hip_engine *e, size_t nbytes) {
    if (!e) return nullptr;
    (void)hipSetDevice(e->device);
    void *p = nullptr;
    if (hipMalloc(&p, nbytes) != hipSuccess) { set_err("hipMalloc(%zu) failed", nbytes); return nullptr; }
    return p;
}
extern "C" void scrappie_hip_device_free(scrappie_hip_engine *e, void *dptr) {
    if (e && dptr) { (void)hipSetDevice(e->device); (void)hipFree(dptr); }
}
extern "C" int scrappie_hip_memcpy_h2d(scrappie_hip_engine *e, void *dst, const void *src, size_t nbytes) {
    if (!e) return -1;
    (void)hipSetDevice(e->device);
    HIPCHK(hipMemcpy(dst, src, nbytes, hipMemcpyHostToDevice));
    return 0;
}
extern "C" int scrappie_hip_synchronize(scrappie_hip_engine *e) {
    if (!e) return -1;
    (void)hipSetDevice(e->device);
    HIPCHK(sh_stream_wait(e->stream));
    return 0;
}

extern "C" long scrappie_hip_lane_schedule(const int *tile_T, size_t ntile, int ncu, int lanes_per_wg, int *nwg, int *capacity,
                                           int *lane_off, int *seg, size_t cap) {
    if (!tile_T || ncu < 1 || lanes_per_wg < 1 || lanes_per_wg > 2) return -1;
    ShGruSchedule sc;
    sh_lane_schedule(tile_T, ntile, ncu, lanes_per_wg, sc);
    if (nwg) *nwg = sc.nwg;
    if (capacity) *capacity = sc.capacity;
    if (lane_off) memcpy(lane_off, sc.lane_off.data(), sc.lane_off.size() * sizeof(int));
    if (seg) for (size_t i = 0; i < sc.seg.size() && i < cap; i++) memcpy(seg + 4 * i, &sc.seg[i], 16);
// ... 56 lines not shown
```

### scrappie_amd/csrc/sh_eng_pipeline.inc

```

enum StopAt { STOP_NONE = 0, STOP_TRUNK = 1, STOP_POST = 2 };

struct RunOut {
    const float *act = nullptr;
    int act_units = 0;
    const float *E = nullptr;
    const float *sums = nullptr;
};

struct HostStamp {
    const std::chrono::steady_clock::time_point t0 = std::chrono::steady_clock::now();
    void operator()(const char *what, const char *after = "") const {
        if (tun().host_stamp) fprintf(stderr, "host stamp: %s %.2f ms%s\n", what, std::chrono::duration<double, std::milli>(std::chrono::steady_clock::now() - t0).count(), after);
    }
};

struct Marks {
    enum Mark { PROLOGUE_BEGIN, PROLOGUE_END,
                WAIT_BEGIN, MAIN_BEGIN,
                LAYER_BEGIN, LAYER_SPLIT, LAYER_END,
                S1_BEGIN, S1_END, DECODE_END, MAIN_END,
                WALK_BEGIN, WALK_END, STITCH_BEGIN, STITCH_END,
                N_MARKS };
    Slot *sl = nullptr;
    bool on = false;
    int at[N_MARKS] = {0};
    int mark(Mark k, hipStream_t st) {
        if (on && sl->nev < 48) { at[k] = sl->nev++; HIPCHK(hipEventRecord(sl->ev[at[k]], st)); }
        return 0;
    }
    void span(SpanField field, Mark from, Mark to) { if (on) sl->spans.push_back({field, at[from], at[to]}); }
};

struct GroupRun {
    scrappie_hip_engine *e = nullptr;
    const float *d_signal = nullptr; const uint64_t *offsets = nullptr; const scrappie_hip_params *p = nullptr;
    StopAt stop = STOP_NONE; int trunk_upto = 5; RunOut *ro = nullptr;
    bool transducer = false, hp_on = false;
    MetaPtrs mp;
    hipStream_t s = nullptr, ps = nullptr, cs = nullptr;
    long long ncb = 0; size_t act_bytes = 0;
    float *abuf[3] = {nullptr, nullptr, nullptr};
    bool fuse_conv = false;
    bool walk_on_cs = false;
    bool fold_tail = false;
    Marks pf;
    HostStamp stamp;
};

static int longest_tile(const LaunchGroup &lg) {
    int maxT = 0;
    for (size_t i = 0; i < lg.npad; i += 16) maxT = std::max(maxT, lg.rT[i]);
    return maxT;
}

static void mark_pending(scrappie_hip_engine *e, Slot &sl) {
    sl.pending = true;
    if (!e->other(sl).pending) e->oldest = e->index(sl);
}

static int begin_group(scrappie_hip_engine *e, Model *m, const uint32_t *lengths, size_t n, GroupRun &c, Slot **slot, bool *empty) {
    Slot *slp = nullptr;
    for (int k = 0; k < 2 && !slp; k++) { Slot &cand = e->slots[(e->cur + 1 + k) & 1]; if (!cand.pending) slp = &cand; }
    if (!slp) return set_err("two launch groups are already in flight: call scrappie_hip_collect first");
    Slot &sl = *slp;
    e->cur = e->index(sl);
    if (build_group(e, sl, m, c.offsets, lengths, n, c.hp_on, c.mp)) return -1;
    c.stamp("build_group");
    *slot = slp;
    *empty = sl.lg.ncb == 0;
    if (*empty) {
        sl.lg.valid = true; sl.lg.model = (int)(std::find(e->models.begin(), e->models.end(), m) - e->models.begin());
        if (c.stop == STOP_NONE) { if (e->ev_ok) HIPCHK(hipEventRecord(sl.done, c.s)); mark_pending(e, sl); }
    }
    return 0;
}

static int stage_prologue(Slot &sl, Model *m, GroupRun &c) {
    scrappie_hip_engine *e = c.e;
    LaunchGroup &lg = sl.lg;
    const hipStream_t s = c.s; hipStream_t &ps = c.ps;
    const int F = m->F;
#ifdef SH_EXPERIMENTS
// ... 12 lines not shown
    c.fuse_conv = tun().conv_in_layer && !tun().conv_valu && m->arch == 0 && F == 96 && m->S == 96 && (kst == 3 || kst == 5) &&
                  c.stop == STOP_NONE && c.trunk_upto >= 5 && !tun().gru_separate && !m->layer_f32[0] &&
                  !(SH_GRU_FREE_DEFAULT ? !tun().gru_barrier : tun().gru_free);
    if (c.fuse_conv) {
        if (sl.h_edge.ensure(lg.npad * 16) || sl.d_edge.ensure(lg.npad * 16)) return -1;
        int *ew = sl.h_edge.as<int>();
        for (size_t i = 0; i < lg.npad && c.fuse_conv; i++) {
            const int o = lg.order[i];
            if (!conv_edge_words(m->geom, lg.rN[i], lg.rT[i], ew + 4 * i)) c.fuse_conv = false;
            if (o >= 0 && lg.rT[i] > 0 && c.offsets[o] + (uint64_t)lg.rN[i] >= ((uint64_t)1 << 30)) c.fuse_conv = false;
        }
    }
#endif
    if (c.pf.mark(Marks::PROLOGUE_BEGIN, ps)) return -1;
    if (m->arch == 3) {
        dim3 grid((unsigned)lg.ntile, (unsigned)std::min(64, (longest_tile(lg) + 3) / 4));
        hipLaunchKernelGGL(k_feat_in, grid, dim3(256), 0, ps, c.d_signal, c.mp.md, m->nfeat, c.abuf[0], c.ncb, sl.d_bad.as<unsigned>());
    } else if (c.fuse_conv) {
        hipLaunchKernelGGL(k_upload_words, dim3((unsigned)std::min<size_t>((lg.npad + 255) / 256, 256)), dim3(256), 0, ps,
                           (const u32x4 *)sl.h_edge.p, sl.d_edge.as<u32x4>(), (long long)lg.npad);
    } else {
        const int tchunk = tun().conv_tchunk;
        dim3 grid((unsigned)lg.ntile, (unsigned)std::min(65535, (longest_tile(lg) + tchunk - 1) / tchunk));
        const bool bg = e->ev_ok && e->other(sl).pending && ps != s;
#ifdef SH_EXPERIMENTS
        static const int fake = getenv("SH_CONV_FAKE") ? atoi(getenv("SH_CONV_FAKE")) : 0;
#else
        const int fake = 0;
#endif
        const bool mfma_ok = !tun().conv_valu && F == 96 && (kst == 3 || kst == 5);
        const bool areg = kst == 3 && !bg;
        const size_t lds = ((size_t)m->WL * F + F + (mfma_ok && !areg ? (size_t)6 * kst * 64 : 0) + 16 * ((size_t)(tchunk - 1) * m->stride + m->WL)) * 4;
        using ConvKernel = void (*)(const float *, ShMeta, const float *, const float *, ShConvGeom, float *, int, unsigned *);
        auto act = [&](ConvKernel none, ConvKernel tanh_) { return m->conv_act == 1 ? tanh_ : none; };
        const ConvKernel kern = !mfma_ok ? (bg ? act(k_conv_act_bg<0>, k_conv_act_bg<1>) : act(k_conv_act<0>, k_conv_act<1>))
                              : areg     ? act(k_conv_mfma<0, 6, 3, true>, k_conv_mfma<1, 6, 3, true>)
                              : kst == 3 ? (bg ? act(k_conv_mfma_bg<0, 6, 3, false>, k_conv_mfma_bg<1, 6, 3, false>) : act(k_conv_mfma<0, 6, 3, false>, k_conv_mfma<1, 6, 3, false>))
                                         : (bg ? act(k_conv_mfma_bg<0, 6, 5, false>, k_conv_mfma_bg<1, 6, 5, false>) : act(k_conv_mfma<0, 6, 5, false>, k_conv_mfma<1, 6, 5, false>));
        if (fake == 1) HIPCHK(hipMemsetAsync(c.abuf[0], 0, c.act_bytes, ps));
        else if (fake != 2) hipLaunchKernelGGL(kern, grid, dim3(256), lds, ps, c.d_signal, c.mp.md, m->conv_W.as<float>(), m->conv_b.as<float>(), m->geom, c.abuf[0], tchunk, sl.d_bad.as<unsigned>());
    }
    if (c.pf.mark(Marks::PROLOGUE_END, ps)) return -1;
    c.pf.span(F_CONV, Marks::PROLOGUE_BEGIN, Marks::PROLOGUE_END);
    c.stamp("prologue enqueued at");
    if (c.pf.mark(Marks::WAIT_BEGIN, s)) return -1;
    if (e->ev_ok && ps != s) { HIPCHK(hipEventRecord(sl.pdone, ps)); HIPCHK(hipStreamWaitEvent(s, sl.pdone, 0)); }
    c.stamp("wait enqueued at");
    if (c.pf.mark(Marks::MAIN_BEGIN, s)) return -1;
    c.pf.span(F_WAIT, Marks::WAIT_BEGIN, Marks::MAIN_BEGIN); c.pf.span(F_LEAD, Marks::PROLOGUE_END, Marks::WAIT_BEGIN);
    if (tun().helper_fence && e->ev_ok && e->other(sl).pending) HIPCHK(hipStreamWaitEvent(s, e->other(sl).hdone, 0));
    return 0;
}

static int recurrent_layer(Slot &sl, Model *m, GroupRun &c, int l, int I, const float *in, float *out, int backward) {
    scrappie_hip_engine *e = c.e;
    const LaunchGroup &lg = sl.lg; const MetaPtrs &mp = c.mp;
    const hipStream_t s = c.s;
    const bool lstm = m->arch == 3;
    const int S = m->S, gates = lstm ? 4 : 3;
    const float *resid = m->arch == 1 ? in : nullptr;
    const bool f32 = !lstm && m->layer_f32[l];
    const bool one_kernel = !tun().gru_separate && (lstm ? (I == S || I == 16) && S % 32 == 0 : gru_proj_ok(I, S) && !f32);
    if (c.pf.mark(Marks::LAYER_BEGIN, s)) return -1;
#ifdef SH_EXPERIMENTS
    if (l == 0 && c.fuse_conv) {
        if (c.pf.mark(Marks::LAYER_SPLIT, s)) return -1;
        ShConvFuse cf;
        cf.sig = c.d_signal; cf.W = m->conv_W.as<float>(); cf.bias = m->conv_b.as<float>(); cf.edge = sl.d_edge.as<int>();
        cf.bad = sl.d_bad.as<unsigned>(); cf.g = m->geom;
        if (launch_gru_conv(s, (m->WL + 3) / 4, m->conv_act, out, m->iWp[l].as<unsigned>(), m->ibs[l].as<float>(), m->sWp[l].as<unsigned>(),
                            m->sW2p[l].as<unsigned>(), mp.md, 1, mp.lanes1, lg.gru1_nwg, mp.lanes, lg.gru_nwg, lg.gru_two, cf)) return -1;
    } else if (!lstm && one_kernel && use_gru32(e) && S == 96 && I == 96 && m->has32) {
        if (c.pf.mark(Marks::LAYER_SPLIT, s)) return -1;
        if (use_gru32(e) == 2 ? launch_gru_proj32x2(s, in, out, m->arch == 1, m->iWp32[l].as<unsigned>(), m->ib32[l].as<float>(), m->sWp32[l].as<unsigned>(),
                                                    m->sW2p32[l].as<unsigned>(), mp.md, backward, mp.pairs2, lg.gru32x2_nwg, lg.ntile)
                              : launch_gru_proj32(s, in, out, m->arch == 1, m->iWp32[l].as<unsigned>(), m->ib32[l].as<float>(), m->sWp32[l].as<unsigned>(),
                                                  m->sW2p32[l].as<unsigned>(), mp.md, backward, mp.pairs, lg.gru32_nwg, lg.ntile)) return -1;
    } else
#endif
    if (one_kernel) {
        if (c.pf.mark(Marks::LAYER_SPLIT, s)) return -1;
        if (lstm ? launch_lstm_proj(s, S, I, in, out, m->iWp[l].as<unsigned>(), m->ibs[l].as<float>(), m->sWp[l].as<unsigned>(), m->lp[l].as<float>(),
                                    mp.md, backward, mp.lanes1, lg.gru1_nwg)
                 : launch_gru_proj(s, S, in, out, resid, m->iWp[l].as<unsigned>(), m->ibs[l].as<float>(), m->sWp[l].as<unsigned>(), m->sW2p[l].as<unsigned>(),
                                   mp.md, backward, mp.lanes1, lg.gru1_nwg, mp.lanes, lg.gru_nwg, lg.gru_two)) return -1;
    } else {
        if (e->d_xaff.ensure((size_t)c.ncb * gates * S * 16 * 4)) return -1;
        if (launch_affine(s, I, in, e->d_xaff.as<float>(), m->iW[l].as<float>(), m->iWp[l].as<unsigned>(), m->ib[l].as<float>(), m->ibs[l].as<float>(), c.ncb, gates * S / 16, f32)) return -1;
        if (c.pf.mark(Marks::LAYER_SPLIT, s)) return -1;
        if (lstm ? launch_lstm(s, S, e->d_xaff.as<float>(), out, m->sWp[l].as<unsigned>(), m->lp[l].as<float>(), mp.md, backward, mp.lanes, lg.gru_nwg)
                 : launch_gru(s, S, e->d_xaff.as<float>(), out, resid, m->sW[l].as<float>(), m->sW2[l].as<float>(), m->sWp[l].as<unsigned>(), m->sW2p[l].as<unsigned>(),
                              mp.md, backward, lg.ntile, mp.lanes, lg.gru_nwg, f32)) return -1;
    }
    if (c.pf.mark(Marks::LAYER_END, s)) return -1;
    c.pf.span(F_AFFINE, Marks::LAYER_BEGIN, Marks::LAYER_SPLIT);
    c.pf.span(F_GRU, Marks::LAYER_SPLIT, Marks::LAYER_END);
    if (c.pf.on) {
        scrappie_hip_timing &tm = sl.timing;
        const double af = 2.0 * I * gates * S * 16.0 * (double)c.ncb, gf = 2.0 * gates * S * S * 16.0 * (double)c.ncb;
        tm.n_affine_launches++; tm.n_gru_launches++; tm.affine_flops += af; tm.gru_flops += gf;
        if (one_kernel) { tm.n_fused_launches++; tm.fused_flops += af + gf; }
    }
    if (one_kernel) c.pf.span(F_FUSED, Marks::LAYER_SPLIT, Marks::LAYER_END);
    return 0;
}

static int stage_trunk(Slot &sl, Model *m, GroupRun &c, int *top) {
    const hipStream_t s = c.s;
    const int S = m->S, F = m->F;
    float **abuf = c.abuf; *top = 0;
    if (m->arch == 2 || m->arch == 3) {
        for (int lvl = 0; lvl < 2 && lvl < c.trunk_upto; lvl++) {
            for (int dir = 0; dir < 2; dir++) if (recurrent_layer(sl, m, c, 2 * lvl + dir, lvl == 0 ? F : S, abuf[0], abuf[1 + dir], dir)) return -1;
            if (c.pf.mark(Marks::LAYER_BEGIN, s)) return -1;
            if (launch_affine2(s, S, abuf[1], abuf[2], abuf[0], m->ff2W[lvl][0].as<unsigned>(), m->ff2W[lvl][1].as<unsigned>(), m->ff2b[lvl].as<float>(), c.ncb, S / 16)) return -1;
            if (c.pf.mark(Marks::LAYER_SPLIT, s)) return -1;
            c.pf.span(F_AFFINE, Marks::LAYER_BEGIN, Marks::LAYER_SPLIT);
            if (c.pf.on) sl.timing.affine_flops += 2.0 * 2 * S * S * 16.0 * (double)c.ncb;
        }
    } else {
        for (int l = 0; l < 5 && l < c.trunk_upto; l++, *top ^= 1)
            if (recurrent_layer(sl, m, c, l, l == 0 ? F : S, abuf[*top], abuf[*top ^ 1], (l % 2 == 0) ? 1 : 0)) return -1;
    }
    HIPCHK(hipGetLastError());
    c.stamp("layers enqueued at");
    return 0;
}

template <class Grow, class Launch>
static int inject_alt(const Slot &sl, GroupRun &c, AltInput &alt, uint64_t seed, Grow grow, Launch launch) {
    const LaunchGroup &lg = sl.lg;
    std::vector<unsigned long long> aoff(lg.npad, ~0ull);
    uint64_t key = 1469598103934665603ull ^ seed;
    for (size_t i = 0; i < lg.npad; i++) {
        const int o = lg.order[i];
        if (o >= 0 && lg.rT[i] > 0) aoff[i] = alt.off[(size_t)o % alt.off.size()];
        key = (key ^ (uint64_t)(aoff[i] + 0x9e3779b97f4a7c15ull * (uint64_t)(lg.rT[i] + 1))) * 1099511628211ull;
    }
    if (alt.valid && key == alt.key) return 0;
    if (grow() || alt.d_off.ensure(lg.npad * 8)) return -1;
    HIPCHK(hipMemcpyAsync(alt.d_off.p, aoff.data(), lg.npad * 8, hipMemcpyHostToDevice, c.s));
    HIPCHK(sh_stream_wait(c.s));
    launch(dim3((unsigned)lg.ntile, (unsigned)std::min(longest_tile(lg), 1024)), alt.d_off.as<unsigned long long>());
    alt.key = key; alt.valid = true;
    return 0;
}

static int stage_decode_transducer(Slot &sl, Model *m, GroupRun &c, const float *top, bool fused, bool *stopped) {
    scrappie_hip_engine *e = c.e;
    LaunchGroup &lg = sl.lg; const MetaPtrs &mp = c.mp;
    const hipStream_t s = c.s; const scrappie_hip_params *p = c.p;
    const int S = m->S, mtiles = m->ff_mtiles;
    const long long ncb = c.ncb;
    if (e->d_sums.ensure((size_t)ncb * 16 * 4)) return -1;
    if (c.pf.mark(Marks::S1_BEGIN, s)) return -1;
    if (!fused && launch_ff(s, S, top, e->d_E.as<float>(), e->d_sums.as<float>(), m->ffWp.as<unsigned>(), m->ffbs.as<float>(),
                            ncb, mtiles, m->NS, p->tempW / p->tempb, p->tempb, e->ncu)) return -1;
    if (c.pf.mark(Marks::S1_END, s)) return -1;
    c.pf.span(F_FF, Marks::S1_BEGIN, Marks::S1_END);
    if (c.pf.on) sl.timing.ff_flops += 2.0 * S * m->NS * 16.0 * (double)ncb;
    const float *E_use = e->d_E.as<float>(), *sums_use = e->d_sums.as<float>();
    if (e->alt_prob) {
        if (inject_alt(sl, c, e->alt_prob, (uint64_t)lg.model,
                       [&] { return e->d_Ealt.ensure((size_t)ncb * mtiles * 256 * 4) || e->d_sums_alt.ensure((size_t)ncb * 16 * 4); },
                       [&](dim3 grid, const unsigned long long *off) {
                           hipLaunchKernelGGL(k_inject_prob, grid, dim3(256), 0, s, e->alt_prob.data, off, mp.md, m->NS, mtiles, e->d_Ealt.as<float>(), e->d_sums_alt.as<float>());
                       })) return -1;
        E_use = e->d_Ealt.as<float>(); sums_use = e->d_sums_alt.as<float>();
    }
    if (c.ro) { c.ro->E = E_use; c.ro->sums = sums_use; }
    if (c.stop == STOP_POST) { HIPCHK(hipGetLastError()); *stopped = true; return 0; }
    const int NH = m->NS - 1, NQ = NH / 4;
    if (e->d_tb.ensure((size_t)ncb * NQ * 16 * 4) || e->d_tbend.ensure((size_t)ncb * 16 * 4) || e->d_fstate.ensure(lg.npad * 4)) return -1;
    if (c.hp_on && sl.d_hp.ensure((size_t)std::max<long long>(lg.nhp, 1) * 5 * 4)) return -1;
    ShVitArgs va;
    va.E = E_use; va.sums = sums_use;
    va.strideT = (long long)mtiles * 256; va.strideQ = 64; va.strideB = 4;
    va.want_log = 1; va.min_prob = p->min_prob;
    va.stay_pen = p->stay_pen; va.skip_pen = p->skip_pen; va.local_pen = p->local_pen; va.use_slip = p->use_slip;
    va.tb = e->d_tb.as<unsigned>(); va.tb_end = e->d_tbend.as<int>();
    va.final_state = e->d_fstate.as<int>(); va.final_score = sl.d_fscore.as<float>();
    va.hp_side = c.hp_on ? sl.d_hp.as<float>() : nullptr; va.hp_off = mp.hp_off;
    va.dbg = nullptr;
    va.dump_final = e->dbg_dump_final ? 1 : 0;
    static StampBuf vst;
    if (tun().vit_stamp) va.dbg = vst.dev(4096 * 16 * 8);
    if (e->d_vstate.ensure(std::max<size_t>(lg.ntile, 1) * ((size_t)NH * 16 + 32) * 4) || e->d_vflag.ensure(std::max<size_t>(lg.ntile, 1) * 4)) return -1;
    HIPCHK(hipMemsetAsync(e->d_vflag.p, 0, std::max<size_t>(lg.ntile, 1) * 4, s));
    va.seg = mp.vseg;
    va.vstate = e->d_vstate.as<float>(); va.flag = e->d_vflag.as<unsigned>(); va.err = sl.d_gflag.as<unsigned>() + lg.ntile;
    if (e->ev_ok && e->other(sl).pending) HIPCHK(hipStreamWaitEvent(s, e->other(sl).done, 0));
    if (fused) {
        ShFfArgs fa;
        fa.in = top; fa.wpiece = m->ffWp.as<unsigned>(); fa.bfrag = m->ffbs.as<float>();
        fa.in_div = p->tempW / p->tempb; fa.out_div = p->tempb;
        fa.no_clamp = (m->ff_no_clamp && !e->alt_trunk) ? 1 : 0;
        va.E = nullptr; va.sums = nullptr;
        if (launch_ff_viterbi(s, fa, va, mp.md, (size_t)lg.vit_nwg, tun().fv_single || e->dbg_fv_single)) return -1;
    } else if (launch_viterbi(s, NH, va, mp.md, (size_t)lg.vit_nwg)) return -1;
    if (va.dbg) vst.dump_on(0, s, (size_t)std::max(lg.vit_nwg, 1) * 16 * 8, [&](const unsigned long long *h) {
        const int nwv = (fused && !va.use_slip && !(tun().fv_single || e->dbg_fv_single)) ? 12 : 8;
        for (int w = 0; w < nwv; w++) { const unsigned long long *d = &h[((size_t)(lg.vit_nwg / 2) * nwv + w) * 8]; fprintf(stderr, "vit stamp wave %d: phaseB %.0f bar %.0f phaseC %.0f bar %.0f cycles/block\n", w, d[0] / (double)d[4], d[1] / (double)d[4], d[2] / (double)d[4], d[3] / (double)d[4]); }
    });
    if (c.pf.mark(Marks::DECODE_END, s)) return -1;
    c.pf.span(F_DECODE, Marks::S1_END, Marks::DECODE_END);
    c.stamp("decoder enqueued at");
    c.walk_on_cs = e->ev_ok;
    if (c.walk_on_cs) { HIPCHK(hipEventRecord(sl.kdone, s)); HIPCHK(hipStreamWaitEvent(e->cstream, sl.kdone, 0)); }
    c.fold_tail = c.walk_on_cs && !tun().split_tail && !tun().host_stitch;
    if (!c.fold_tail) {
        hipStream_t bs = c.walk_on_cs ? e->cstream : s;
        if (c.pf.mark(Marks::WALK_BEGIN, bs)) return -1;
        hipLaunchKernelGGL(k_backtrace, dim3((unsigned)((lg.npad + 63) / 64)), dim3(64), 0, bs, e->d_tb.as<unsigned>(), e->d_tbend.as<int>(),
                           e->d_fstate.as<int>(), mp.md, mp.seq_off, sl.d_seq.as<int>(), (int)lg.npad, NQ, SH_SEQ_STRIDE);
        if (c.pf.mark(Marks::WALK_END, bs)) return -1;
        c.pf.span(F_BACKTRACE, Marks::WALK_BEGIN, Marks::WALK_END);
    }
    return 0;
}

static int stage_decode_crf(Slot &sl, Model *m, GroupRun &c, const float *top, bool *stopped) {
    scrappie_hip_engine *e = c.e;
    const LaunchGroup &lg = sl.lg; const MetaPtrs &mp = c.mp;
    const hipStream_t s = c.s;
    const int S = m->S, mtiles = m->ff_mtiles;
    const long long ncb = c.ncb;
    if (c.pf.mark(Marks::S1_BEGIN, s)) return -1;
    if (launch_affine(s, S, top, e->d_E.as<float>(), m->ffW.as<float>(), m->ffWp.as<unsigned>(), m->ffb.as<float>(), m->ffbs.as<float>(), ncb, mtiles)) return -1;
    if (c.pf.mark(Marks::S1_END, s)) return -1;
    c.pf.span(F_FF, Marks::S1_BEGIN, Marks::S1_END);
    if (c.pf.on) sl.timing.ff_flops += 2.0 * S * m->NS * 16.0 * (double)ncb;
    if (e->d_tb.ensure((size_t)ncb * 16 * 8)) return -1;
    if (e->ev_ok && e->other(sl).pending) HIPCHK(hipStreamWaitEvent(s, e->other(sl).done, 0));
    hipLaunchKernelGGL((c.ro || c.stop == STOP_POST) ? k_crf<true> : k_crf<false>, dim3((unsigned)(lg.npad / 16)), dim3(128), 0, s, e->d_E.as<float>(), mp.md,
                       e->d_tb.as<unsigned char>(), mp.seq_off, sl.d_seq.as<int>(), sl.d_fscore.as<float>(), (int)lg.npad, SH_SEQ_STRIDE);
    if (c.pf.mark(Marks::DECODE_END, s)) return -1;
    c.pf.span(F_DECODE, Marks::S1_END, Marks::DECODE_END);
    if (c.ro) { c.ro->E = e->d_E.as<float>(); c.ro->sums = nullptr; }
    if (c.stop == STOP_POST) { HIPCHK(hipGetLastError()); *stopped = true; }
    return 0;
}

static int stage_tail(Slot &sl, Model *m, GroupRun &c) {
    scrappie_hip_engine *e = c.e;
    LaunchGroup &lg = sl.lg; const MetaPtrs &mp = c.mp;
    const hipStream_t s = c.s, cs = c.cs;
    if (sl.h_score.ensure(lg.npad * 4)) return -1;
    if (sl.h_err.ensure(4) || sl.h_bad.ensure(lg.npad * 4)) return -1;
    if (c.pf.mark(Marks::MAIN_END, s)) return -1;
    c.pf.span(F_TOTAL, Marks::MAIN_BEGIN, Marks::MAIN_END);
    if (e->ev_ok && !c.walk_on_cs) { HIPCHK(hipEventRecord(sl.kdone, s)); HIPCHK(hipStreamWaitEvent(cs, sl.kdone, 0)); }
    lg.dev_stitch = !tun().host_stitch;
    lg.dev_pos = lg.dev_stitch && c.p->want_pos != 0 && c.transducer;
    if (lg.dev_stitch) {
        const size_t nseq = (size_t)std::max<long long>(lg.nseq, 1), ncap = (size_t)std::max<long long>(lg.nbases_cap, 1);
        if (sl.d_bases.ensure(ncap) || sl.d_blen.ensure(lg.npad * 4) || sl.d_redo.ensure(lg.npad * 4) ||
            sl.h_bases.ensure(ncap) || sl.h_blen.ensure(lg.npad * 4) || sl.h_redo.ensure(lg.npad * 4)) return -1;
        if (lg.dev_pos && (sl.d_pos.ensure(nseq * 4 + 16) || sl.h_pos.ensure(nseq * 4 + 16))) return -1;
        ShStitchArgs sa;
        sa.seq = sl.d_seq.as<int>(); sa.seq_off = mp.seq_off;
        sa.hp = c.hp_on ? sl.d_hp.as<float>() : nullptr; sa.hp_off = mp.hp_off;
        sa.pos = lg.dev_pos ? sl.d_pos.as<int>() : nullptr;
        sa.bases = sl.d_bases.as<char>(); sa.bases_off = mp.bases_off;
        sa.blen = sl.d_blen.as<int>(); sa.redo = sl.d_redo.as<unsigned>();
        sa.npad = (int)lg.npad; sa.nstate = m->NS; sa.crf = c.transducer ? 0 : 1; sa.sstride = SH_SEQ_STRIDE;
        ShResultArgs ra;
        ra.d_bases = sl.d_bases.as<char>(); ra.h_bases = sl.h_bases.as<char>(); ra.bases_off = mp.bases_off;
        ra.d_blen = sl.d_blen.as<int>(); ra.h_blen = sl.h_blen.as<int>();
        ra.d_redo = sl.d_redo.as<unsigned>(); ra.h_redo = sl.h_redo.as<unsigned>();
        ra.d_score = sl.d_fscore.as<float>(); ra.h_score = sl.h_score.as<float>();
        ra.d_bad = sl.d_bad.as<unsigned>(); ra.h_bad = sl.h_bad.as<unsigned>();
        ra.d_err = sl.d_gflag.as<unsigned>() + lg.ntile; ra.h_err = sl.h_err.as<unsigned>();
        ra.npad = (int)lg.npad;
        if (c.pf.mark(Marks::STITCH_BEGIN, cs)) return -1;
        if (c.fold_tail) {
            ShWalkArgs wa;
            wa.tb = e->d_tb.as<unsigned>(); wa.tb_end = e->d_tbend.as<int>(); wa.final_state = e->d_fstate.as<int>();
            wa.seq_off = mp.seq_off; wa.seq = sl.d_seq.as<int>(); wa.NQ = (m->NS - 1) / 4;
            hipLaunchKernelGGL(k_walk_stitch_out, dim3((unsigned)((lg.npad + 63) / 64)), dim3(64), 0, cs, wa, sa, ra, mp.md);
        } else
            hipLaunchKernelGGL(k_stitch, dim3((unsigned)((lg.npad + 63) / 64)), dim3(64), 0, cs, sa, mp.md);
        if (c.pf.mark(Marks::STITCH_END, cs)) return -1;
        c.pf.span(F_STITCH, Marks::STITCH_BEGIN, Marks::STITCH_END);
        if (e->ev_ok) HIPCHK(hipEventRecord(sl.hdone, cs));
        c.stamp("stitch enqueued at");
        if (!c.fold_tail) hipLaunchKernelGGL(k_results_out, dim3((unsigned)((lg.npad + 3) / 4)), dim3(256), 0, cs, ra);
        if (lg.dev_pos) {
            const long long n16 = (lg.nseq * 4 + 15) / 16;
            hipLaunchKernelGGL(k_upload_words, dim3((unsigned)std::min<long long>((n16 + 255) / 256, 256)), dim3(256), 0, cs, (const u32x4 *)sl.d_pos.p, sl.h_pos.as<u32x4>(), n16);
        }
    } else {
        if (sl.h_seq.ensure((size_t)std::max<long long>(lg.nseq, 1) * 4)) return -1;
        if (c.hp_on && sl.h_hp.ensure((size_t)std::max<long long>(lg.nhp, 1) * 5 * 4)) return -1;
        HIPCHK(hipMemcpyAsync(sl.h_seq.p, sl.d_seq.p, (size_t)lg.nseq * 4, hipMemcpyDeviceToHost, cs));
        if (c.hp_on) HIPCHK(hipMemcpyAsync(sl.h_hp.p, sl.d_hp.p, (size_t)lg.nhp * 5 * 4, hipMemcpyDeviceToHost, cs));
        HIPCHK(hipMemcpyAsync(sl.h_score.p, sl.d_fscore.p, lg.npad * 4, hipMemcpyDeviceToHost, cs));
        HIPCHK(hipMemcpyAsync(sl.h_err.p, sl.d_gflag.as<unsigned>() + lg.ntile, 4, hipMemcpyDeviceToHost, cs));
        HIPCHK(hipMemcpyAsync(sl.h_bad.p, sl.d_bad.p, lg.npad * 4, hipMemcpyDeviceToHost, cs));
    }
    HIPCHK(hipGetLastError());
    c.stamp("copies enqueued at");
    if (e->ev_ok) HIPCHK(hipEventRecord(sl.done, cs));
    return 0;
}

static int run_pipeline(scrappie_hip_engine *e, Model *m, const float *d_signal, const uint64_t *offsets,
                        const uint32_t *lengths, size_t n, const scrappie_hip_params *p, StopAt stop,
                        int trunk_upto, RunOut *ro) {
    (void)hipSetDevice(e->device);
    if (n == 0) return set_err("empty batch");
    GroupRun c;
    c.e = e; c.d_signal = d_signal; c.offsets = offsets; c.p = p; c.stop = stop; c.trunk_upto = trunk_upto; c.ro = ro;
    c.transducer = (m->arch != 1);
    c.hp_on = c.transducer && p->homopolymer == HOMOPOLYMER_MEAN && stop == STOP_NONE;
    c.s = e->stream; c.ps = e->ev_ok ? e->pstream : e->stream; c.cs = e->ev_ok ? e->cstream : e->stream;
    Slot *slp = nullptr; bool empty = false;
    if (begin_group(e, m, lengths, n, c, &slp, &empty)) return -1;
    if (empty) return 0;
    Slot &sl = *slp;
    LaunchGroup &lg = sl.lg;
    const long long ncb = c.ncb = lg.ncb;
    const int S = m->S, F = m->F;
    c.act_bytes = (size_t)ncb * std::max(S, F) * 16 * 4;
    if (e->d_act[1].ensure(c.act_bytes)) return -1;
    bool any_f32 = false;
    for (bool b : m->layer_f32) any_f32 |= b;
    const bool need_xaff = m->arch == 3 || !gru_proj_ok(F, S) || tun().gru_separate || any_f32;
    if (need_xaff && e->d_xaff.ensure((size_t)ncb * (m->arch == 3 ? 4 : 3) * S * 16 * 4)) return -1;
    if ((m->arch == 2 || m->arch == 3) && e->d_act[2].ensure(c.act_bytes)) return -1;
    c.pf.sl = &sl; c.pf.on = e->profiling && e->ev_ok;
    if (c.pf.on) { memset(&sl.timing, 0, sizeof sl.timing); sl.nev = 0; sl.spans.clear(); }
    if (stage_prologue(sl, m, c)) return -1;
    int cur = 0;
    if (stage_trunk(sl, m, c, &cur)) return -1;
    if (ro) { ro->act = c.abuf[cur]; ro->act_units = (trunk_upto == 0) ? F : S; }
    lg.model = (int)(std::find(e->models.begin(), e->models.end(), m) - e->models.begin());
    if (stop == STOP_TRUNK) { lg.valid = true; return 0; }
    const float *top = c.abuf[cur];
    if (e->alt_trunk) {
        if (inject_alt(sl, c, e->alt_trunk, (uint64_t)lg.model ^ ((uint64_t)S << 32),
                       [&] { return e->d_act_alt.ensure((size_t)ncb * S * 16 * 4); },
                       [&](dim3 grid, const unsigned long long *off) {
                           hipLaunchKernelGGL(k_inject_trunk, grid, dim3(256), 0, c.s, e->alt_trunk.data, off, c.mp.md, S, e->d_act_alt.as<float>());
                       })) return -1;
        top = e->d_act_alt.as<float>();
    }
    const bool fused = c.transducer && stop == STOP_NONE && decoder_fused(e, m);
    if (!fused && e->d_E.ensure((size_t)ncb * m->ff_mtiles * 256 * 4)) return -1;
    if (sl.d_seq.ensure((size_t)std::max<long long>(lg.nseq, 1) * 4) || sl.d_fscore.ensure(lg.npad * 4)) return -1;
    bool stopped = false;
// ... 37 lines not shown
```

### scrappie_amd/csrc/sh_gru.h

```cpp
#ifndef SH_GRU_H
#define SH_GRU_H

template <int NU>
__global__ __launch_bounds__(64 * NU) void k_gru(const float *__restrict__ xaff, float *__restrict__ out,
                                                 const float *__restrict__ resid,
                                                 const float *__restrict__ sWfrag ,
                                                 const float *__restrict__ sW2frag ,
                                                 ShMeta md, int backward, unsigned long long *dbgbuf) {
    constexpr int KR = NU * 4;
    const int dbg = backward >> 8;
    backward &= 1;
    __shared__ __attribute__((aligned(16))) float lds[2 * NU * 256];
    float *lds_h = lds, *lds_rh = lds + NU * 256;
    const int lane = threadIdx.x & 63, u = threadIdx.x >> 6;
    const int tile = blockIdx.x;
    const int Tt = md.tile_T[tile];
    const long long boff = md.tile_boff[tile];
    const int myT = md.rT[tile * 16 + (lane & 15)];

    float wz[KR], wr[KR], wh[KR];
#pragma unroll
    for (int r = 0; r < KR; r++) {
        wz[r] = sWfrag[((long long)u * KR + r) * 64 + lane];
        wr[r] = sWfrag[((long long)(NU + u) * KR + r) * 64 + lane];
// ... 55 lines not shown
        if (dbg != 1)
#pragma unroll
        for (int mm = 0; mm < NU; mm++) {
            accz = mfma4(wz[mm * 4 + 0], hb[mm][0], accz);
            accz2 = mfma4(wz[mm * 4 + 1], hb[mm][1], accz2);
            accz = mfma4(wz[mm * 4 + 2], hb[mm][2], accz);
            accz2 = mfma4(wz[mm * 4 + 3], hb[mm][3], accz2);
        }
        f32x4 acch2 = {0.f, 0.f, 0.f, 0.f};
        if (dbg != 1)
#pragma unroll
        for (int mm = 0; mm < NU; mm++) {
            acch = mfma4(wh[mm * 4 + 0], rb[mm][0], acch);
            acch2 = mfma4(wh[mm * 4 + 1], rb[mm][1], acch2);
            acch = mfma4(wh[mm * 4 + 2], rb[mm][2], acch);
            acch2 = mfma4(wh[mm * 4 + 3], rb[mm][3], acch2);
        }
        accz += accz2;
        f32x4 z;
#pragma unroll
        for (int i = 0; i < 4; i++) z[i] = d_logistic(accz[i]);
        acch += acch2;
        const bool active = t < myT;
        f32x4 o;
#pragma unroll
        for (int i = 0; i < 4; i++) {
            const float hbar = d_tanh(acch[i]);
            const float hn = z[i] * h[i] + (1.0f - z[i]) * hbar;
            h[i] = active ? hn : 0.0f;
            o[i] = h[i];
        }
        *(f32x4 *)(lds_h + u * 256 + lane * 4) = h;
        if (resid) {
            const f32x4 rv = *(const f32x4 *)(resid + ((boff + t) * NU + u) * 256 + lane * 4);
            o += rv;
        }
        if (dbg != 2) *(f32x4 *)(out + ((boff + t) * NU + u) * 256 + lane * 4) = o;
        STAMP(tD);
        __syncthreads();
        STAMP(tE);
    }
    if (dbgbuf && lane == 0) { unsigned long long *d = dbgbuf + ((long long)blockIdx.x * NU + u) * 8; d[0] = tA; d[1] = tB; d[2] = tC; d[3] = tD; d[4] = tE; d[5] = Tt; d[6] = wall0; d[7] = wall_clock64(); }
    if (dbg == 2) *(f32x4 *)(out + (boff * NU + u) * 256 + lane * 4) = h;
}


struct ShGruSegD { int tile, s0, s1, pad; };
struct ShGruLanes {
    const int *lane_off;
    const ShGruSegD *seg;
    const int *wg_iter;
    float *hstate;
    unsigned *flag;
    int ntile;
};

struct ShGruPairs {
    const int *lane_off;
    const ShGruSegD *seg;
    const int *pair_tile;
    float *hstate;
    unsigned *flag;
    unsigned *err;
};

template <int NU, bool STAMP = false>
__global__ __launch_bounds__(128 * NU) void k_gru_lanes(const float *__restrict__ xaff, float *__restrict__ out,
                                                       const float *__restrict__ resid,
                                                       const float *__restrict__ sWfrag,
                                                       const float *__restrict__ sW2frag, ShMeta md,
                                                       int backward, ShGruLanes L, unsigned long long *dbgbuf = nullptr) {
    constexpr int KR = NU * 4;
    extern __shared__ __attribute__((aligned(16))) float lds[];
    const int lane = threadIdx.x & 63;
    const int wave = __builtin_amdgcn_readfirstlane(threadIdx.x >> 6);
    const int u = wave % NU, grp = wave / NU;
    const int ln = blockIdx.x * 2 + grp;

    float wz[KR], wr[KR], wh[KR];
#pragma unroll
    for (int r = 0; r < KR; r++) {
        wz[r] = sWfrag[((long long)u * KR + r) * 64 + lane];
        wr[r] = sWfrag[((long long)(NU + u) * KR + r) * 64 + lane];
        wh[r] = sW2frag[((long long)u * KR + r) * 64 + lane];
    }
    float *lds_h = lds + grp * 2 * NU * 256, *lds_rh = lds_h + NU * 256;
    const long long xstride = 3LL * NU * 256;
    const int nit = L.wg_iter[blockIdx.x];
    int sgi = __builtin_amdgcn_readfirstlane(L.lane_off[ln]);
    const int sge = __builtin_amdgcn_readfirstlane(L.lane_off[ln + 1]);
    int my_it = 0;
    for (int i = sgi; i < sge; i++) my_it += L.seg[i].s1 - L.seg[i].s0;
    my_it = __builtin_amdgcn_readfirstlane(my_it);

    int tile = 0, s = 0, s1 = 0, Tt = 0, boff = 0;
    int n_tile = 0, n_s0 = 0, n_s1 = 0, n_Tt = 0, n_boff = 0;
    bool n_ok = false;
    int myT = 0, n_myT = 0;
    auto fetch_next = [&](int i) {
        n_ok = i < sge;
        if (n_ok) {
            const ShGruSegD sg = L.seg[i];
            n_tile = __builtin_amdgcn_readfirstlane(sg.tile);
            n_s0 = __builtin_amdgcn_readfirstlane(sg.s0);
            n_s1 = __builtin_amdgcn_readfirstlane(sg.s1);
            n_Tt = __builtin_amdgcn_readfirstlane(md.tile_T[n_tile]);
            n_boff = __builtin_amdgcn_readfirstlane((int)md.tile_boff[n_tile]);
            n_myT = md.rT[n_tile * 16 + (lane & 15)];
        }
    };
    auto advance = [&]() { tile = n_tile; s = n_s0; s1 = n_s1; Tt = n_Tt; boff = n_boff; myT = n_myT; };
    f32x4 h = {0.f, 0.f, 0.f, 0.f};
    auto take_over = [&]() {
        h = (f32x4){0.f, 0.f, 0.f, 0.f};
        if (s > 0) {
            if (!sh_wait_flag(L.flag + tile, (unsigned)NU, L.flag + L.ntile) && lane == 0)
                __hip_atomic_store(L.flag + L.ntile, 1u, __ATOMIC_RELAXED, __HIP_MEMORY_SCOPE_AGENT);
            __builtin_amdgcn_fence(__ATOMIC_ACQUIRE, "agent");
            const float *hs = L.hstate + ((long long)tile * NU + u) * 256 + lane * 4;
#pragma unroll
            for (int k = 0; k < 4; k++) h[k] = __hip_atomic_load(hs + k, __ATOMIC_RELAXED, __HIP_MEMORY_SCOPE_AGENT);
        }
    };
    f32x4 xz = h, xr = h, xh = h;
    auto xload = [&](long long col) {
        const float *p = xaff + col * xstride + lane * 4;
        xz = *(const f32x4 *)(p + u * 256);
        xr = *(const f32x4 *)(p + (NU + u) * 256);
        xh = *(const f32x4 *)(p + (2 * NU + u) * 256);
    };
    if (my_it > 0) {
        fetch_next(sgi);
        advance();
        fetch_next(++sgi);
        take_over();
        *(f32x4 *)(lds_h + u * 256 + lane * 4) = h;
        xload(boff + (backward ? Tt - 1 - s : s));
    }
    __syncthreads();

    unsigned long long g1 = 0, g2 = 0, g3 = 0, g4 = 0, gt0 = 0, gt1;
#define LSTAMP(acc) do { if (STAMP) { gt1 = __builtin_readcyclecounter(); acc += gt1 - gt0; gt0 = gt1; } } while (0)
    if (STAMP) gt0 = __builtin_readcyclecounter();
    int it = 0;
    for (; it < my_it; it++) {
        f32x4 hb[NU];
#pragma unroll
        for (int mm = 0; mm < NU; mm++) hb[mm] = *(const f32x4 *)(lds_h + mm * 256 + lane * 4);
        f32x4 ar = xr, ar2 = {0.f, 0.f, 0.f, 0.f}, az = xz, ah = xh;
        const int t = backward ? Tt - 1 - s : s;
        {
            long long ncol = boff + t;
            if (s + 1 < s1) ncol = boff + (backward ? t - 1 : t + 1);
            else if (n_ok) ncol = n_boff + (backward ? n_Tt - 1 - n_s0 : n_s0);
            xload(ncol);
        }
#pragma unroll
        for (int mm = 0; mm < NU; mm++) {
            ar = mfma4(wr[mm * 4 + 0], hb[mm][0], ar);
            ar2 = mfma4(wr[mm * 4 + 1], hb[mm][1], ar2);
            ar = mfma4(wr[mm * 4 + 2], hb[mm][2], ar);
            ar2 = mfma4(wr[mm * 4 + 3], hb[mm][3], ar2);
        }
        ar += ar2;
        const f32x4 rh = d_logistic4(ar) * h;
        *(f32x4 *)(lds_rh + u * 256 + lane * 4) = rh;
        LSTAMP(g1);
        lds_barrier();
        LSTAMP(g2);
        f32x4 rb[NU];
// ... 64 lines not shown
    const int lane = threadIdx.x & 63;
    const int wave = __builtin_amdgcn_readfirstlane(threadIdx.x >> 6);
    const int u = wave % NU, grp = wave / NU;
    const int ln = blockIdx.x * 2 + grp;

    ShSplit wz[KS], wr[KS], wh[KS];
#pragma unroll
    for (int ks = 0; ks < KS; ks++) {
        wz[ks] = load_pieces(sWp + ((long long)u * KS + ks) * 512, lane);
        wr[ks] = load_pieces(sWp + ((long long)(NU + u) * KS + ks) * 512, lane);
        wh[ks] = load_pieces(sW2p + ((long long)u * KS + ks) * 512, lane);
    }
    unsigned *lds_h = ldsw + grp * 2 * PBUF, *lds_rh = lds_h + PBUF;
    const int wofs = (((u >> 1) * 2) * 64 + lane) * 4 + (u & 1) * 2;
    auto publish = [&](unsigned *buf, f32x4 v) {
        unsigned a1, a2, b1, b2;
        split_pair(v[0], v[1], a1, a2);
        split_pair(v[2], v[3], b1, b2);
        *(uint2 *)(buf + wofs) = make_uint2(a1, b1);
        *(uint2 *)(buf + wofs + 256) = make_uint2(a2, b2);
    };
    auto pieces = [&](const unsigned *buf, int ks) {
        return load_pieces(buf + ks * 512, lane);
    };
    const long long xstride = 3LL * NU * 256;
    const int nit = L.wg_iter[blockIdx.x];
    int sgi = __builtin_amdgcn_readfirstlane(L.lane_off[ln]);
    const int sge = __builtin_amdgcn_readfirstlane(L.lane_off[ln + 1]);
    int my_it = 0;
    for (int i = sgi; i < sge; i++) my_it += L.seg[i].s1 - L.seg[i].s0;
    my_it = __builtin_amdgcn_readfirstlane(my_it);

    int tile = 0, s = 0, s1 = 0, Tt = 0, boff = 0;
    int n_tile = 0, n_s0 = 0, n_s1 = 0, n_Tt = 0, n_boff = 0;
    bool n_ok = false;
    int myT = 0, n_myT = 0;
    auto fetch_next = [&](int i) {
        n_ok = i < sge;
        if (n_ok) {
            const ShGruSegD sg = L.seg[i];
            n_tile = __builtin_amdgcn_readfirstlane(sg.tile);
            n_s0 = __builtin_amdgcn_readfirstlane(sg.s0);
            n_s1 = __builtin_amdgcn_readfirstlane(sg.s1);
            n_Tt = __builtin_amdgcn_readfirstlane(md.tile_T[n_tile]);
            n_boff = __builtin_amdgcn_readfirstlane((int)md.tile_boff[n_tile]);
            n_myT = md.rT[n_tile * 16 + (lane & 15)];
        }
    };
    auto advance = [&]() { tile = n_tile; s = n_s0; s1 = n_s1; Tt = n_Tt; boff = n_boff; myT = n_myT; };
    f32x4 h = {0.f, 0.f, 0.f, 0.f};
    auto take_over = [&]() {
        h = (f32x4){0.f, 0.f, 0.f, 0.f};
        if (s > 0) {
            if (!sh_wait_flag(L.flag + tile, (unsigned)NU, L.flag + L.ntile) && lane == 0)
                __hip_atomic_store(L.flag + L.ntile, 1u, __ATOMIC_RELAXED, __HIP_MEMORY_SCOPE_AGENT);
            __builtin_amdgcn_fence(__ATOMIC_ACQUIRE, "agent");
            const float *hs = L.hstate + ((long long)tile * NU + u) * 256 + lane * 4;
#pragma unroll
            for (int k = 0; k < 4; k++) h[k] = __hip_atomic_load(hs + k, __ATOMIC_RELAXED, __HIP_MEMORY_SCOPE_AGENT);
        }
    };
    f32x4 xz = h, xr = h, xh = h;
    auto xload = [&](long long col) {
        const float *p = xaff + col * xstride + lane * 4;
        xz = *(const f32x4 *)(p + u * 256);
        xr = *(const f32x4 *)(p + (NU + u) * 256);
        xh = *(const f32x4 *)(p + (2 * NU + u) * 256);
    };
    if (my_it > 0) {
        fetch_next(sgi);
        advance();
        fetch_next(++sgi);
        take_over();
        publish(lds_h, h);
        xload(boff + (backward ? Tt - 1 - s : s));
    }
    __syncthreads();

    int it = 0;
    for (; it < my_it; it++) {
        f32x4 ar = xr * SH_OSCALE, az = xz * SH_OSCALE, ah = xh * SH_OSCALE;
        const int t = backward ? Tt - 1 - s : s;
        {
            long long ncol = boff + t;
            if (s + 1 < s1) ncol = boff + (backward ? t - 1 : t + 1);
            else if (n_ok) ncol = n_boff + (backward ? n_Tt - 1 - n_s0 : n_s0);
            xload(ncol);
        }
        {
            ShSplit hp[KS];
#pragma unroll
            for (int ks = 0; ks < KS; ks++) hp[ks] = pieces(lds_h, ks);
            split_dot2<KS>(wr, wz, hp, ar, az);
        }
        publish(lds_rh, d_logistic4_acc(ar) * h);
        const f32x4 z = d_logistic4_acc(az);
        lds_barrier();
        {
            ShSplit rp[KS];
#pragma unroll
            for (int ks = 0; ks < KS; ks++) rp[ks] = pieces(lds_rh, ks);
            ah = split_dot<KS>(wh, rp, ah);
        }
        const bool active = t < myT;
        {
            const f32x4 hbar = d_tanh4_acc(ah);
            const f32x4 hn = z * h + (1.0f - z) * hbar;
#pragma unroll
// ... 333 lines not shown
        } else
        for (int it = 0; it < nit; it++) {
            const int np = (it + 1) & 1;
            if (SH_PDELAY_A) __builtin_amdgcn_s_sleep(SH_PDELAY_A);
#pragma unroll
            for (int tl = 0; tl < NT; tl++) project_h(lds_in(tl, np), lds_x(tl, np));
            PSTAMP(pa);
            lds_barrier();
            PSTAMP(pb);
            if (SH_PROJ_VALU_FIRST) {
#pragma unroll
                for (int tl = 0; tl < NT; tl++) {
                    publish(lds_in(tl, it & 1), chunk_of(xq1[tl]));
                    if constexpr (RLDS) *(f32x4 *)lds_raw(tl, wslot) = chunk_of(xq1[tl]);
                    xq1[tl] = xq2[tl];
                    xq2[tl] = fetch(c[tl], tl);
                }
                __builtin_amdgcn_sched_barrier(0);
            }
            if (SH_PDELAY_B) __builtin_amdgcn_s_sleep(SH_PDELAY_B);
#pragma unroll
            for (int tl = 0; tl < NT; tl++) project_zr(lds_in(tl, np), lds_x(tl, np));
            if (!SH_PROJ_VALU_FIRST) {
#pragma unroll
                for (int tl = 0; tl < NT; tl++) {
                    publish(lds_in(tl, it & 1), chunk_of(xq1[tl]));
                    if constexpr (RLDS) *(f32x4 *)lds_raw(tl, wslot) = chunk_of(xq1[tl]);
                    xq1[tl] = xq2[tl];
                    xq2[tl] = fetch(c[tl], tl);
                }
            }
            if constexpr (RLDS) wslot = wslot == 2 ? 0 : wslot + 1;
            PSTAMP(pc);
            lds_barrier();
            PSTAMP(pd);
        }
        PDUMP();
        return;
    }

    if (SH_REC_PRIO) __builtin_amdgcn_s_setprio(SH_REC_PRIO);
    if (SH_REC45_PRIO && NU == 6 && wave >= 4) __builtin_amdgcn_s_setprio(SH_REC45_PRIO);
    static_assert(NT <= 2, "two block counts per register");
    unsigned myT2 = 0;
    f32x4 h[NT];
    auto take_over = [&](int tl) {
        h[tl] = (f32x4){0.f, 0.f, 0.f, 0.f};
        int mt = 0;
        if (c[tl].ok) mt = md.rT[c[tl].tile * 16 + (lane & 15)];
        if (NT == 1) myT2 = (unsigned)mt;
        else myT2 = tl ? ((myT2 & 0xffffu) | ((unsigned)mt << 16)) : ((myT2 & 0xffff0000u) | ((unsigned)mt & 0xffffu));
        if (!c[tl].ok) return;
        if (c[tl].s > 0) {
            if (!sh_wait_flag(L.flag + c[tl].tile, (unsigned)NU, L.flag + L.ntile) && lane == 0)
                __hip_atomic_store(L.flag + L.ntile, 1u, __ATOMIC_RELAXED, __HIP_MEMORY_SCOPE_AGENT);
            __builtin_amdgcn_fence(__ATOMIC_ACQUIRE, "agent");
            const float *hs = L.hstate + ((long long)c[tl].tile * NU + u) * 256 + lane * 4;
#pragma unroll
            for (int k = 0; k < 4; k++) h[tl][k] = __hip_atomic_load(hs + k, __ATOMIC_RELAXED, __HIP_MEMORY_SCOPE_AGENT);
        }
        asm volatile("" : "+v"(myT2), "+v"(h[tl][0]), "+v"(h[tl][1]), "+v"(h[tl][2]), "+v"(h[tl][3]));
    };
    long long oix[NT];
    const long long dstep = backward ? -(long long)(NU * 256) : (long long)(NU * 256);
    auto cur_off = [&](int tl) {
        const long long v = c[tl].ok ? (column(c[tl]) * NU + u) * 256 : (long long)(u * 256);
        const unsigned lo = __builtin_amdgcn_readfirstlane((unsigned)v), hi = __builtin_amdgcn_readfirstlane((unsigned)(v >> 32));
        return (long long)(((unsigned long long)hi << 32) | lo);
    };
#pragma unroll
    for (int tl = 0; tl < NT; tl++) {
        enter(c[tl]);
        take_over(tl);
        oix[tl] = cur_off(tl);
        publish(lds_h(tl), h[tl]);
    }
    lds_barrier();
    lds_barrier();
    if (STAMP) pt0 = __builtin_readcyclecounter();
    f32x4 rs[NT];
    auto resid_fetch = [&](int tl) {
        rs[tl] = gload(resid + oix[tl]);
    };
    if (RESID && !RLDS) {
#pragma unroll
        for (int tl = 0; tl < NT; tl++) resid_fetch(tl);
    }
    int rslot = 0;
    for (int it = 0; it < nit; it++) {
        const int par = it & 1;
        f32x4 cr[NT], cz[NT];
        f32x4 z[NT];
        if (SH_RFIRST) {
            ShSplit hp[NT][KS];
#pragma unroll
            for (int tl = 0; tl < NT; tl++) {
                const float *xs = lds_x(tl, par);
                cz[tl] = *(const f32x4 *)(xs + (u * 64 + lane) * 4);
                cr[tl] = *(const f32x4 *)(xs + ((NU + u) * 64 + lane) * 4);
#pragma unroll
                for (int ks = 0; ks < KS; ks++) hp[tl][ks] = pieces(lds_h(tl), ks);
                cr[tl] = split_dot<KS>(w1, hp[tl], cr[tl]);
            }
#pragma unroll
            for (int tl = 0; tl < NT; tl++) cz[tl] = split_dot<KS>(w0, hp[tl], cz[tl]);
#pragma unroll
            for (int tl = 0; tl < NT; tl++) publish(lds_rh(tl), abl_logistic4(cr[tl]) * h[tl]);
        } else {
// ... 134 lines not shown
```

### scrappie_amd/csrc/sh_gru_free.h

```cpp
#ifndef SH_GRU_FREE_H
#define SH_GRU_FREE_H

template <int NU, int NT, bool RESID, bool STAMP = false>
__global__ __launch_bounds__(128 * NU) void k_gru_free(const float *__restrict__ in, float *__restrict__ out,
                                                       const float *__restrict__ resid,
                                                       const unsigned *__restrict__ iWp, const float *__restrict__ ibfrag,
                                                       const unsigned *__restrict__ sWp, const unsigned *__restrict__ sW2p,
                                                       ShMeta md, int backward, ShGruLanes L,
                                                       unsigned long long *dbg = nullptr) {
    static_assert(NU % 2 == 0, "k steps of 32 units");
    constexpr int KS = NU / 2, RING = 3;
    constexpr int PBUF = KS * 2 * 64 * 4;
    constexpr int XBUF = 3 * NU * 256;
    constexpr int TBUF = 4 * PBUF + RING * XBUF;
    enum { C_FULL = 0, C_SYNCA = 1, C_SYNCB = 2, C_PCNT = 3 };
    extern __shared__ __attribute__((aligned(16))) unsigned ldsw[];
    volatile unsigned *cnt = (volatile unsigned *)(ldsw + NT * TBUF);
    unsigned long long s_work = 0, s_w0 = 0, s_w1 = 0, s_w2 = 0, s_t0 = 0, s_t1;
#define FSTAMP(acc) do { if (STAMP) { s_t1 = __builtin_readcyclecounter(); acc += s_t1 - s_t0; s_t0 = s_t1; } } while (0)
    const int lane = threadIdx.x & 63;
    const unsigned lofs = (unsigned)lane * 4u;
    typedef __attribute__((address_space(1))) float *gf32;
    typedef __attribute__((address_space(1))) f32x4 *gf32x4;
    auto gload = [&](const float *base) { gf32 b = (gf32)base; asm volatile("" : "+s"(b)); return *(gf32x4)(b + lofs); };
// ... 91 lines not shown
        f32x4 q0[NT], q1[NT], q2[NT];
#pragma unroll
        for (int tl = 0; tl < NT; tl++) {
            enter(c[tl]);
            q0[tl] = fetch(c[tl]); q1[tl] = fetch(c[tl]); q2[tl] = fetch(c[tl]);
        }
        if (STAMP) s_t0 = __builtin_readcyclecounter();
        int slot = 0;
        for (int j = 0; j < nit; j++) {
#pragma unroll
            for (int tl = 0; tl < NT; tl++) {
                publish(lds_in(tl, j & 1), q0[tl]);
                q0[tl] = q1[tl]; q1[tl] = q2[tl];
                q2[tl] = fetch(c[tl]);
            }
            arrive(C_PCNT);
            FSTAMP(s_work);
            wait_for(C_PCNT, (unsigned)NU * (unsigned)(j + 1));
            FSTAMP(s_w0);
            if (j >= RING) wait_for(C_SYNCB, (unsigned)NU * (unsigned)(j - RING + 2));
            FSTAMP(s_w1);
#pragma unroll
            for (int tl = 0; tl < NT; tl++) {
                ShSplit ip[KS];
#pragma unroll
                for (int ks = 0; ks < KS; ks++) ip[ks] = pieces(lds_in(tl, j & 1), ks);
                const f32x4 ah = split_dot<KS>(w2, ip, bh);
                f32x4 cz = bz, cr = br;
                split_dot2<KS>(w0, w1, ip, cz, cr);
                float *xdst = lds_x(tl, slot);
                *(f32x4 *)(xdst + (u * 64 + lane) * 4) = cz;
                *(f32x4 *)(xdst + ((NU + u) * 64 + lane) * 4) = cr;
                *(f32x4 *)(xdst + ((2 * NU + u) * 64 + lane) * 4) = ah;
            }
            arrive(C_FULL);
            slot = (slot == RING - 1) ? 0 : slot + 1;
            FSTAMP(s_work);
        }
        if (STAMP && dbg && lane == 0) { unsigned long long *d_ = dbg + ((long long)blockIdx.x * 2 * NU + wave) * 16; d_[0] = s_work; d_[1] = s_w0; d_[2] = s_w1; d_[3] = 0; d_[4] = nit; }
        return;
    }

    static_assert(NT <= 2, "two block counts per register");
    unsigned myT2 = 0;
    f32x4 h[NT];
    auto take_over = [&](int tl) {
        h[tl] = (f32x4){0.f, 0.f, 0.f, 0.f};
        int mt = 0;
        if (c[tl].ok) mt = md.rT[c[tl].tile * 16 + (lane & 15)];
        if (NT == 1) myT2 = (unsigned)mt;
        else myT2 = tl ? ((myT2 & 0xffffu) | ((unsigned)mt << 16)) : ((myT2 & 0xffff0000u) | ((unsigned)mt & 0xffffu));
        if (!c[tl].ok) return;
        if (c[tl].s > 0) {
            if (!sh_wait_flag(L.flag + c[tl].tile, (unsigned)NU, L.flag + L.ntile) && lane == 0)
                __hip_atomic_store(L.flag + L.ntile, 1u, __ATOMIC_RELAXED, __HIP_MEMORY_SCOPE_AGENT);
            __builtin_amdgcn_fence(__ATOMIC_ACQUIRE, "agent");
            const float *hs = L.hstate + ((long long)c[tl].tile * NU + u) * 256 + lane * 4;
#pragma unroll
            for (int k = 0; k < 4; k++) h[tl][k] = __hip_atomic_load(hs + k, __ATOMIC_RELAXED, __HIP_MEMORY_SCOPE_AGENT);
        }
        asm volatile("" : "+v"(myT2), "+v"(h[tl][0]), "+v"(h[tl][1]), "+v"(h[tl][2]), "+v"(h[tl][3]));
    };
#pragma unroll
    for (int tl = 0; tl < NT; tl++) {
        enter(c[tl]);
        take_over(tl);
        publish(lds_h(tl), h[tl]);
    }
    arrive(C_SYNCB);
    f32x4 rs[NT];
    auto resid_fetch = [&](int tl) {
        const long long col = c[tl].ok ? column(c[tl]) : 0;
        rs[tl] = gload(resid + (col * NU + u) * 256);
    };
    if (RESID) {
#pragma unroll
        for (int tl = 0; tl < NT; tl++) resid_fetch(tl);
    }
    if (STAMP) s_t0 = __builtin_readcyclecounter();
    int slot = 0;
    for (int it = 0; it < nit; it++) {
        const unsigned need = (unsigned)NU * (unsigned)(it + 1);
        wait_for(C_FULL, need);
        FSTAMP(s_w0);
        wait_for(C_SYNCB, need);
        FSTAMP(s_w2);
        f32x4 cr[NT], cz[NT], z[NT];
        {
            ShSplit hp[NT][KS];
#pragma unroll
            for (int tl = 0; tl < NT; tl++) {
                const float *xs = lds_x(tl, slot);
                cz[tl] = *(const f32x4 *)(xs + (u * 64 + lane) * 4);
                cr[tl] = *(const f32x4 *)(xs + ((NU + u) * 64 + lane) * 4);
#pragma unroll
                for (int ks = 0; ks < KS; ks++) hp[tl][ks] = pieces(lds_h(tl), ks);
                cr[tl] = split_dot<KS>(w1, hp[tl], cr[tl]);
            }
#pragma unroll
            for (int tl = 0; tl < NT; tl++) cz[tl] = split_dot<KS>(w0, hp[tl], cz[tl]);
#pragma unroll
            for (int tl = 0; tl < NT; tl++) publish(lds_rh(tl), d_logistic4_acc(cr[tl]) * h[tl]);
        }
        arrive(C_SYNCA);
        FSTAMP(s_work);
        wait_for(C_SYNCA, need);
        FSTAMP(s_w1);
        f32x4 ch[NT];
// ... 52 lines not shown
```

### scrappie_amd/csrc/sh_gru_mx.h

```cpp
#ifndef SH_GRU_MX_H
#define SH_GRU_MX_H

template <bool RESID, bool STAMP = false>
__global__ __launch_bounds__(1024) __attribute__((amdgpu_num_vgpr(64))) void k_gru_mx(const float *__restrict__ in, float *__restrict__ out,
                                                       const float *__restrict__ resid,
                                                       const unsigned *__restrict__ iWp, const float *__restrict__ ibfrag,
                                                       const unsigned *__restrict__ sWp, const unsigned *__restrict__ sW2p,
                                                       ShMeta md, int backward, ShGruLanes L, unsigned long long *dbg = nullptr) {
    constexpr int NU = 6, NT = 2, KS = 3;
    unsigned long long st[8] = {0, 0, 0, 0, 0, 0, 0, 0}, st0 = 0;
#define MXS(i) do { if (STAMP) { const unsigned long long t_ = __builtin_readcyclecounter(); st[i] += t_ - st0; st0 = t_; } } while (0)
#define MXBAR(i) do { MXS(2 * (i)); lds_barrier(); MXS(2 * (i) + 1); } while (0)
#define MXDUMP() do { if (STAMP && dbg && lane == 0) { unsigned long long *d_ = dbg + ((long long)blockIdx.x * 16 + wave) * 10; for (int i_ = 0; i_ < 8; i_++) d_[i_] = st[i_]; d_[8] = (unsigned long long)nit; } } while (0)
    constexpr int PBUF = KS * 2 * 64 * 4;
    constexpr int XBUF = 3 * NU * 256;
    constexpr int TBUF = 4 * PBUF + 2 * XBUF;
    extern __shared__ __attribute__((aligned(16))) unsigned ldsw[];
    const int lane = threadIdx.x & 63;
    const unsigned lofs = (unsigned)lane * 4u;
    typedef __attribute__((address_space(1))) float *gf32;
    typedef __attribute__((address_space(1))) f32x4 *gf32x4;
    auto gload = [&](const float *base) { gf32 b = (gf32)base; asm volatile("" : "+s"(b)); return *(gf32x4)(b + lofs); };
    auto gstore = [&](float *base, f32x4 v) { gf32 b = (gf32)base; asm volatile("" : "+s"(b)); *(gf32x4)(b + lofs) = v; };
    const int wave = __builtin_amdgcn_readfirstlane(threadIdx.x >> 6);
// ... 100 lines not shown
            MXBAR(1);
            if (spread) project_h(1, np);
            MXBAR(2);
            if (!spread) project_h(1, np);
            project_zr(1, np);
            MXBAR(3);
        }
        MXDUMP();
        return;
    }

    const int v = wave - 2 * NU, tl = v >> 1, u0 = 3 * (v & 1);
    auto wofs = [&](int u) { return (((u >> 1) * 2) * 64 + lane) * 4 + (u & 1) * 2; };
    auto publish = [&](unsigned *buf, int u, f32x4 x) {
        unsigned a1, a2, b1, b2;
        split_pair(x[0], x[1], a1, a2); split_pair(x[2], x[3], b1, b2);
        *(uint2 *)(buf + wofs(u)) = make_uint2(a1, b1);
        *(uint2 *)(buf + wofs(u) + 256) = make_uint2(a2, b2);
    };
    ShLaneCursor ci = {}, co = {};
    ci.sgi = co.sgi = sgi0[tl]; ci.sge = co.sge = sge0[tl];
    auto enter = [&](ShLaneCursor &cc) {
        cc.ok = cc.sgi < cc.sge;
        if (cc.ok) {
            const ShGruSegD sg = L.seg[cc.sgi];
            cc.tile = __builtin_amdgcn_readfirstlane(sg.tile);
            cc.s = __builtin_amdgcn_readfirstlane(sg.s0);
            cc.s1 = __builtin_amdgcn_readfirstlane(sg.s1);
            cc.Tt = __builtin_amdgcn_readfirstlane(md.tile_T[cc.tile]);
            cc.boff = __builtin_amdgcn_readfirstlane((int)md.tile_boff[cc.tile]);
        }
    };
    auto column = [&](const ShLaneCursor &cc) { return (long long)cc.boff + (backward ? cc.Tt - 1 - cc.s : cc.s); };
    struct X3 { f32x4 a[3]; };
    auto fetch = [&]() {
        X3 x;
        const long long col = ci.ok ? column(ci) : 0;
#pragma unroll
        for (int k = 0; k < 3; k++) x.a[k] = gload(in + (col * NU + u0 + k) * 256);
        if (ci.ok) {
            ci.s++;
            if (ci.s == ci.s1) { ci.sgi++; enter(ci); }
        }
        return x;
    };
    f32x4 h[3], z[3];
    int myT = 0;
    auto take_over = [&]() {
#pragma unroll
        for (int k = 0; k < 3; k++) h[k] = (f32x4){0.f, 0.f, 0.f, 0.f};
        myT = co.ok ? md.rT[co.tile * 16 + (lane & 15)] : 0;
        if (!co.ok) return;
        if (co.s > 0) {
            if (!sh_wait_flag(L.flag + co.tile, (unsigned)NU, L.flag + L.ntile) && lane == 0)
                __hip_atomic_store(L.flag + L.ntile, 1u, __ATOMIC_RELAXED, __HIP_MEMORY_SCOPE_AGENT);
            __builtin_amdgcn_fence(__ATOMIC_ACQUIRE, "agent");
#pragma unroll
            for (int k = 0; k < 3; k++) {
                const float *hs = L.hstate + ((long long)co.tile * NU + u0 + k) * 256 + lane * 4;
#pragma unroll
                for (int j = 0; j < 4; j++) h[k][j] = __hip_atomic_load(hs + j, __ATOMIC_RELAXED, __HIP_MEMORY_SCOPE_AGENT);
            }
        }
        asm volatile("" : "+v"(myT), "+v"(h[0]), "+v"(h[1]), "+v"(h[2]));
    };
    enter(ci); enter(co);
    take_over();
    {
        const X3 x0 = fetch();
#pragma unroll
        for (int k = 0; k < 3; k++) { publish(lds_in(tl, 0), u0 + k, x0.a[k]); publish(lds_h(tl), u0 + k, h[k]); }
    }
    X3 xq1 = fetch(), xq2 = fetch();
    lds_barrier();
#pragma unroll
    for (int k = 0; k < 3; k++) publish(lds_in(tl, 1), u0 + k, xq1.a[k]);
    xq1 = xq2; xq2 = fetch();
    lds_barrier();
    f32x4 rs[3];
    auto resid_fetch = [&]() {
        const long long col = co.ok ? column(co) : 0;
#pragma unroll
        for (int k = 0; k < 3; k++) rs[k] = gload(resid + (col * NU + u0 + k) * 256);
    };
    if (RESID) resid_fetch();
    if (STAMP) st0 = __builtin_readcyclecounter();
    for (int it = 0; it < nit; it++) {
        const int par = it & 1;
        const float *xs = lds_x(tl, par);
#pragma unroll
        for (int k = 0; k < 3; k++) publish(lds_in(tl, par), u0 + k, xq1.a[k]);
        xq1 = xq2; xq2 = fetch();
        MXBAR(0);
#pragma unroll
        for (int k = 0; k < 3; k++) {
            const f32x4 cr = *(const f32x4 *)(xs + ((NU + u0 + k) * 64 + lane) * 4);
            publish(lds_rh(tl), u0 + k, d_logistic4_acc(cr) * h[k]);
        }
        MXBAR(1);
#pragma unroll
        for (int k = 0; k < 3; k++) z[k] = d_logistic4_acc(*(const f32x4 *)(xs + ((u0 + k) * 64 + lane) * 4));
        MXBAR(2);
        const bool live = it < my_it[tl];
        const int t = backward ? co.Tt - 1 - co.s : co.s;
        const bool active = t < myT;
#pragma unroll
        for (int k = 0; k < 3; k++) {
            const f32x4 hbar = d_tanh4_acc(*(const f32x4 *)(xs + ((2 * NU + u0 + k) * 64 + lane) * 4));
// ... 41 lines not shown
```

### scrappie_amd/csrc/sh_lstm.h

```cpp
#ifndef SH_LSTM_H
#define SH_LSTM_H

__global__ __launch_bounds__(256) void k_feat_in(const float *__restrict__ feat, ShMeta md, int nfeat,
                                                 float *__restrict__ act, long long ncb_total, unsigned *__restrict__ bad ) {
    bool out_of_range = false;
    const int tile = blockIdx.x;
    const int Tt = md.tile_T[tile];
    const long long boff = md.tile_boff[tile];
    const int lane = threadIdx.x & 63, b = lane & 15, q = lane >> 4;
    const int rd = tile * 16 + b;
    const int myT = md.rT[rd];
    const unsigned long long off = md.sig_off[rd];
    for (int t = blockIdx.y * 4 + (threadIdx.x >> 6); t < Tt; t += gridDim.y * 4) {
        f32x4 v = {0.f, 0.f, 0.f, 0.f};
        if (t < myT) {
#pragma unroll
            for (int k = 0; k < 4; k++) if (4 * q + k < nfeat) v[k] = feat[off + (unsigned long long)t * nfeat + 4 * q + k];
#pragma unroll
            for (int k = 0; k < 4; k++) {
                out_of_range |= !(__builtin_fabsf(v[k]) < SH_ACT_LIMIT);
                v[k] = (v[k] == v[k]) ? __builtin_amdgcn_fmed3f(v[k], -SH_ACT_LIMIT, SH_ACT_LIMIT) : 0.0f;
            }
        }
        *(f32x4 *)(act + (boff + t) * 256 + lane * 4) = v;
// ... 21 lines not shown
    for (int ks = 0; ks < KS; ks++) {
        wi[ks] = load_pieces(sWp + ((long long)u * KS + ks) * 512, lane);
        wu[ks] = load_pieces(sWp + ((long long)(NU + u) * KS + ks) * 512, lane);
        wf[ks] = load_pieces(sWp + ((long long)(2 * NU + u) * KS + ks) * 512, lane);
        wo[ks] = load_pieces(sWp + ((long long)(3 * NU + u) * KS + ks) * 512, lane);
    }
    if (grp == 0) {
#pragma unroll
        for (int g = 0; g < 3; g++)
            *(f32x4 *)(peep + ((g * NU + u) * 64 + lane) * 4) = *(const f32x4 *)(pfrag + ((long long)(g * NU + u) * 64 + lane) * 4);
    }
#pragma unroll
    for (int ks = 0; ks < KS; ks++)
        asm volatile("" : "+v"(wi[ks].p1), "+v"(wi[ks].p2), "+v"(wu[ks].p1), "+v"(wu[ks].p2), "+v"(wf[ks].p1), "+v"(wf[ks].p2), "+v"(wo[ks].p1), "+v"(wo[ks].p2));
    unsigned *lds_h = lds + grp * 2 * PBUF;
    const int wofs = (((u >> 1) * 2) * 64 + lane) * 4 + (u & 1) * 2;
    auto publish = [&](unsigned *buf, f32x4 v) {
        unsigned a1, a2, b1, b2;
        split_pair(v[0], v[1], a1, a2);
        split_pair(v[2], v[3], b1, b2);
        *(uint2 *)(buf + wofs) = make_uint2(a1, b1);
        *(uint2 *)(buf + wofs + 256) = make_uint2(a2, b2);
    };
    const long long xstride = 4LL * NU * 256;
    const int nit = L.wg_iter[blockIdx.x];
    int sgi = __builtin_amdgcn_readfirstlane(L.lane_off[ln]);
    const int sge = __builtin_amdgcn_readfirstlane(L.lane_off[ln + 1]);
    int my_it = 0;
    for (int i = sgi; i < sge; i++) my_it += L.seg[i].s1 - L.seg[i].s0;
    my_it = __builtin_amdgcn_readfirstlane(my_it);

    int tile = 0, s = 0, s1 = 0, Tt = 0, boff = 0;
    int n_tile = 0, n_s0 = 0, n_s1 = 0, n_Tt = 0, n_boff = 0;
    bool n_ok = false;
    int myT = 0, n_myT = 0;
    auto fetch_next = [&](int i) {
        n_ok = i < sge;
        if (n_ok) {
            const ShGruSegD sg = L.seg[i];
            n_tile = __builtin_amdgcn_readfirstlane(sg.tile);
            n_s0 = __builtin_amdgcn_readfirstlane(sg.s0);
            n_s1 = __builtin_amdgcn_readfirstlane(sg.s1);
            n_Tt = __builtin_amdgcn_readfirstlane(md.tile_T[n_tile]);
            n_boff = __builtin_amdgcn_readfirstlane((int)md.tile_boff[n_tile]);
            n_myT = md.rT[n_tile * 16 + (lane & 15)];
            asm volatile("" : "+v"(n_myT));
        }
    };
    auto advance = [&]() { tile = n_tile; s = n_s0; s1 = n_s1; Tt = n_Tt; boff = n_boff; myT = n_myT; };
    f32x4 h = {0.f, 0.f, 0.f, 0.f}, c = h;
    auto take_over = [&]() {
        h = (f32x4){0.f, 0.f, 0.f, 0.f}; c = h;
        if (s > 0) {
            if (!sh_wait_flag(L.flag + tile, (unsigned)NU, L.flag + L.ntile) && lane == 0)
                __hip_atomic_store(L.flag + L.ntile, 1u, __ATOMIC_RELAXED, __HIP_MEMORY_SCOPE_AGENT);
            __builtin_amdgcn_fence(__ATOMIC_ACQUIRE, "agent");
            const float *hs = L.hstate + ((long long)tile * 2 * NU + u) * 256 + lane * 4;
#pragma unroll
            for (int k = 0; k < 4; k++) {
                h[k] = __hip_atomic_load(hs + k, __ATOMIC_RELAXED, __HIP_MEMORY_SCOPE_AGENT);
                c[k] = __hip_atomic_load(hs + NU * 256 + k, __ATOMIC_RELAXED, __HIP_MEMORY_SCOPE_AGENT);
            }
            asm volatile("" : "+v"(h), "+v"(c));
        }
    };
    f32x4 xi = h, xu = h, xf = h, xo = h;
    auto xload = [&](long long col) {
        const float *p = xaff + col * xstride + lane * 4;
        xi = *(const f32x4 *)(p + u * 256);
        xu = *(const f32x4 *)(p + (NU + u) * 256);
        xf = *(const f32x4 *)(p + (2 * NU + u) * 256);
        xo = *(const f32x4 *)(p + (3 * NU + u) * 256);
    };
    int par = 0;
    if (my_it > 0) {
        fetch_next(sgi);
        advance();
        fetch_next(++sgi);
        take_over();
        publish(lds_h + par * PBUF, h);
        xload(boff + (backward ? Tt - 1 - s : s));
    }
    __syncthreads();

    int it = 0;
    for (; it < my_it; it++) {
        const int t = backward ? Tt - 1 - s : s;
        ShSplit hp[KS];
#pragma unroll
        for (int ks = 0; ks < KS; ks++) hp[ks] = load_pieces(lds_h + par * PBUF + ks * 512, lane);
        f32x4 ai = xi * SH_OSCALE, au = xu * SH_OSCALE, af = xf * SH_OSCALE, ao = xo * SH_OSCALE;
        {
            long long ncol = boff + t;
            if (s + 1 < s1) ncol = boff + (backward ? t - 1 : t + 1);
            else if (n_ok) ncol = n_boff + (backward ? n_Tt - 1 - n_s0 : n_s0);
            xload(ncol);
        }
#pragma unroll
        for (int ks = 0; ks < KS; ks++) {
            ai = mfma16(wi[ks].p1, hp[ks].p2, ai); au = mfma16(wu[ks].p1, hp[ks].p2, au);
            af = mfma16(wf[ks].p1, hp[ks].p2, af); ao = mfma16(wo[ks].p1, hp[ks].p2, ao);
        }
#pragma unroll
        for (int ks = 0; ks < KS; ks++) {
            ai = mfma16(wi[ks].p2, hp[ks].p1, ai); au = mfma16(wu[ks].p2, hp[ks].p1, au);
            af = mfma16(wf[ks].p2, hp[ks].p1, af); ao = mfma16(wo[ks].p2, hp[ks].p1, ao);
        }
#pragma unroll
// ... 133 lines not shown
#pragma unroll
            for (int ks = 0; ks < KSI; ks++) ip[ks] = load_pieces(ibuf + ks * 512, lane);
            f32x4 a0 = bias[0], a1 = bias[1], a2 = bias[2], a3 = bias[3];
            split_dot2<KSI>(w[0], w[1], ip, a0, a1);
            split_dot2<KSI>(w[2], w[3], ip, a2, a3);
            *(f32x4 *)(xdst + ((0 * NU + u) * 64 + lane) * 4) = a0;
            *(f32x4 *)(xdst + ((1 * NU + u) * 64 + lane) * 4) = a1;
            *(f32x4 *)(xdst + ((2 * NU + u) * 64 + lane) * 4) = a2;
            *(f32x4 *)(xdst + ((3 * NU + u) * 64 + lane) * 4) = a3;
        };
        enter(c);
        f32x4 xq1, xq2;
        {
            const f32x4 x0 = fetch();
            xq1 = fetch(); xq2 = fetch();
            if (u < NUI) publish(lds_in, x0);
        }
        lds_barrier();
        project(lds_in, lds_x);
        if (u < NUI) publish(lds_in + PBUF, xq1);
        xq1 = xq2;
        xq2 = fetch();
        lds_barrier();
        auto step = [&](int it, f32x4 &e) {
            const int np = (it + 1) & 1;
            if (u < NUI) publish(lds_in + (it & 1) * PBUF, e);
            e = fetch();
            project(lds_in + np * PBUF, lds_x + np * XBUF);
            lds_barrier();
        };
        for (int it = 0; it < nit; it += 2) {
            step(it, xq1);
            if (it + 1 < nit) step(it + 1, xq2);
        }
        return;
    }

    ShSplit w[4][KS];
#pragma unroll
    for (int g = 0; g < 4; g++)
#pragma unroll
        for (int ks = 0; ks < KS; ks++) {
            w[g][ks] = load_pieces(sWp + ((long long)(g * NU + u) * KS + ks) * 512, lane);
            asm volatile("" : "+v"(w[g][ks].p1), "+v"(w[g][ks].p2));
        }
    int myT = 0;
    f32x4 h = {0.f, 0.f, 0.f, 0.f}, cs = h;
    auto take_over = [&]() {
        h = (f32x4){0.f, 0.f, 0.f, 0.f}; cs = h;
        myT = 0;
        if (!c.ok) return;
        myT = md.rT[c.tile * 16 + (lane & 15)];
        if (c.s > 0) {
            if (!sh_wait_flag(L.flag + c.tile, (unsigned)NU, L.flag + L.ntile) && lane == 0)
                __hip_atomic_store(L.flag + L.ntile, 1u, __ATOMIC_RELAXED, __HIP_MEMORY_SCOPE_AGENT);
            __builtin_amdgcn_fence(__ATOMIC_ACQUIRE, "agent");
            const float *hs = L.hstate + ((long long)c.tile * 2 * NU + u) * 256 + lane * 4;
#pragma unroll
            for (int k = 0; k < 4; k++) {
                h[k] = __hip_atomic_load(hs + k, __ATOMIC_RELAXED, __HIP_MEMORY_SCOPE_AGENT);
                cs[k] = __hip_atomic_load(hs + NU * 256 + k, __ATOMIC_RELAXED, __HIP_MEMORY_SCOPE_AGENT);
            }
        }
        asm volatile("" : "+v"(myT), "+v"(h), "+v"(cs));
    };
    enter(c);
    take_over();
    publish(lds_h, h);
    lds_barrier();
    lds_barrier();
    for (int it = 0; it < nit; it++) {
        const int par = it & 1;
        ShSplit hp[KS];
#pragma unroll
        for (int ks = 0; ks < KS; ks++) hp[ks] = load_pieces(lds_h + par * PBUF + ks * 512, lane);
        const float *xs = lds_x + par * XBUF;
        f32x4 ai = *(const f32x4 *)(xs + ((0 * NU + u) * 64 + lane) * 4), au = *(const f32x4 *)(xs + ((1 * NU + u) * 64 + lane) * 4);
        f32x4 af = *(const f32x4 *)(xs + ((2 * NU + u) * 64 + lane) * 4), ao = *(const f32x4 *)(xs + ((3 * NU + u) * 64 + lane) * 4);
#pragma unroll
        for (int ks = 0; ks < KS; ks++) { ai = mfma16(w[0][ks].p1, hp[ks].p2, ai); au = mfma16(w[1][ks].p1, hp[ks].p2, au); af = mfma16(w[2][ks].p1, hp[ks].p2, af); ao = mfma16(w[3][ks].p1, hp[ks].p2, ao); }
#pragma unroll
        for (int ks = 0; ks < KS; ks++) { ai = mfma16(w[0][ks].p2, hp[ks].p1, ai); au = mfma16(w[1][ks].p2, hp[ks].p1, au); af = mfma16(w[2][ks].p2, hp[ks].p1, af); ao = mfma16(w[3][ks].p2, hp[ks].p1, ao); }
#pragma unroll
        for (int ks = 0; ks < KS; ks++) { ai = mfma16(w[0][ks].p1, hp[ks].p1, ai); au = mfma16(w[1][ks].p1, hp[ks].p1, au); af = mfma16(w[2][ks].p1, hp[ks].p1, af); ao = mfma16(w[3][ks].p1, hp[ks].p1, ao); }
        const int t = backward ? c.Tt - 1 - c.s : c.s;
        const bool active = t < myT;
        const f32x4 ti = d_tanh4_acc(ai);
        const f32x4 pu = *(const f32x4 *)(peep + (u * 64 + lane) * 4);
        const f32x4 pf = *(const f32x4 *)(peep + ((NU + u) * 64 + lane) * 4);
        const f32x4 po = *(const f32x4 *)(peep + ((2 * NU + u) * 64 + lane) * 4);
#pragma unroll
        for (int k = 0; k < 4; k++) {
            const float forget = d_logistic(af[k] * SH_OINV + cs[k] * pf[k]) * cs[k];
            const float update = d_logistic(au[k] * SH_OINV + cs[k] * pu[k]) * ti[k];
            const float ns = forget + update;
            const float ho = d_logistic(ao[k] * SH_OINV + ns * po[k]) * d_tanh(ns);
            cs[k] = active ? ns : 0.0f;
            h[k] = active ? ho : 0.0f;
        }
        gstore(out + ((long long)(c.boff + t) * NU + u) * 256, h);
        c.s++;
        if (c.s == c.s1) {
            if (c.s1 < c.Tt) {
                float *hs = L.hstate + ((long long)c.tile * 2 * NU + u) * 256 + lane * 4;
#pragma unroll
                for (int k = 0; k < 4; k++) {
                    __hip_atomic_store(hs + k, h[k], __ATOMIC_RELAXED, __HIP_MEMORY_SCOPE_AGENT);
                    __hip_atomic_store(hs + NU * 256 + k, cs[k], __ATOMIC_RELAXED, __HIP_MEMORY_SCOPE_AGENT);
// ... 15 lines not shown
```

### scrappie_amd/csrc/sh_sched.h

```cpp
#ifndef SH_SCHED_H
#define SH_SCHED_H
#include <algorithm>
#include <vector>

struct ShGruSeg { int tile, s0, s1, pad; };

struct ShGruSchedule {
    int nwg = 0;
    int capacity = 0;
    std::vector<int> lane_off;
    std::vector<ShGruSeg> seg;
    std::vector<int> wg_iter;
};

static inline void sh_lane_schedule(const int *tile_T, size_t ntile, int ncu, int lpw, ShGruSchedule &out,
                                    bool allow_split = true) {
    out = ShGruSchedule();
    std::vector<int> live;
    long long W = 0;
    int maxT = 0;
    for (size_t t = 0; t < ntile; t++) if (tile_T[t] > 0) { live.push_back((int)t); W += tile_T[t]; maxT = std::max(maxT, tile_T[t]); }
    if (live.empty()) { out.lane_off.assign(1, 0); return; }
    const long long nlive = (long long)live.size();
    const int nwg = (int)std::min<long long>(ncu, nlive);
// ... 12 lines not shown
        }
    } else if (!allow_split) {
        std::vector<int> load(L, 0);
        for (long long i = 0; i < nlive; i++) {
            const int p = (int)(std::min_element(load.begin(), load.end()) - load.begin());
            pos[p].push_back({live[i], 0, tile_T[live[i]], 0});
            load[p] += tile_T[live[i]];
        }
        M = *std::max_element(load.begin(), load.end());
    } else {
        M = (int)std::max<long long>(maxT, (W + L - 1) / L);
        int p = 0, used = 0;
        for (int t : live) {
            const int T = tile_T[t];
            const int room = M - used;
            if (T <= room) {
                pos[p].push_back({t, 0, T, 0});
                used += T;
            } else {
                if (room > 0) pos[p].push_back({t, T - room, T, 0});
                p++;
                pos[p].push_back({t, 0, T - room, 0});
                used = T - room;
            }
            if (used == M && p + 1 < L) { p++; used = 0; }
        }
    }
    out.nwg = nwg; out.capacity = M;
    out.lane_off.assign(L + 1, 0);
    out.wg_iter.assign(nwg, 0);
    for (int ln = 0; ln < L; ln++) {
        const std::vector<ShGruSeg> &v = pos[L - 1 - ln];
        int steps = 0;
        for (const ShGruSeg &sg : v) { out.seg.push_back(sg); steps += sg.s1 - sg.s0; }
        out.lane_off[ln + 1] = (int)out.seg.size();
        out.wg_iter[ln / lpw] = std::max(out.wg_iter[ln / lpw], steps);
    }
}
static inline void sh_gru_schedule(const int *tile_T, size_t ntile, int ncu, ShGruSchedule &out) {
    sh_lane_schedule(tile_T, ntile, ncu, 2, out);
}

static inline int sh_pieces_per_tile(long long nlive, int ncu) {
    if (nlive <= ncu) return 1;
    int best = 1;
    double bestv = 1e30;
    for (int k = 1; k <= 4; k++) {
        const double v = (double)((nlive * k + ncu - 1) / ncu) / k;
        if (v < bestv - 1e-9) { bestv = v; best = k; }
    }
    return best;
}
static inline void sh_piece_schedule(const int *tile_T, size_t ntile, int ncu, std::vector<ShGruSeg> &seg,
                                     bool allow_split = true) {
    seg.clear();
    long long nlive = 0;
    for (size_t t = 0; t < ntile; t++) nlive += tile_T[t] > 0;
    const int K = allow_split ? sh_pieces_per_tile(nlive, ncu) : 1;
    for (int k = 0; k < K; k++)
        for (size_t t = 0; t < ntile; t++) {
            const int T = tile_T[t];
            if (T <= 0) continue;
            const int len = (T + K - 1) / K;
            const int s0 = std::min(T, k * len), s1 = std::min(T, (k + 1) * len);
            if (s1 > s0) seg.push_back({(int)t, s0, s1, k});
        }
}
#endif
```

Measured before the change: 1.624 billion.

## Use dynamic piece claiming and per-layer flag slices to drop per-launch flag memsets

Viterbi decode blocks now claim their segment through an atomic counter, so pieces are taken in dispatch order. The piece schedule now follows the single-lane GRU schedule's handover segments, ordered by start time. Per-layer flag slices are zeroed once per group, which removes the hipMemsetAsync before every recurrent launch. Profiling marks between back-to-back layers are merged. The change risks deadlock or ordering problems if a piece's predecessor is claimed late, and it caps the layer count at eight slices per memset.

Result: no change. 1.619 billion (-0.3%).

```diff
diff --git a/scrappie_amd/csrc/scrappie_hip.hip b/scrappie_amd/csrc/scrappie_hip.hip
--- a/scrappie_amd/csrc/scrappie_hip.hip
+++ b/scrappie_amd/csrc/scrappie_hip.hip
@@ -299,7 +299,7 @@
         (void)sh_stream_wait(pstream); (void)sh_stream_wait(stream); (void)sh_stream_wait(cstream);
         slots[0].pending = slots[1].pending = false;
     }
-    DBuf d_hstate, d_vstate, d_vflag;
+    DBuf d_hstate, d_vstate;
     DBuf d_act[3];
     DBuf d_xaff, d_E, d_sums, d_tb, d_tbend, d_fstate;
     int ncu = 256;
@@ -312,6 +312,7 @@
     int dbg_fail_run = 0;
     bool dbg_redo_all = false;
     int dbg_gru_tiles = 0;
+    int dbg_sched_ncu = 0;
     bool dbg_force_f32 = false;
     int dbg_gru32 = -1;
     scrappie_hip_engine *tail = nullptr;
diff --git a/scrappie_amd/csrc/sh_decode.h b/scrappie_amd/csrc/sh_decode.h
--- a/scrappie_amd/csrc/sh_decode.h
+++ b/scrappie_amd/csrc/sh_decode.h
@@ -23,6 +23,14 @@
     int dump_final;
 };
 
+__device__ __forceinline__ int sh_take_piece(unsigned *counter, int *word) {
+    if (threadIdx.x == 0) *word = (int)__hip_atomic_fetch_add(counter, 1u, __ATOMIC_RELAXED, __HIP_MEMORY_SCOPE_AGENT);
+    __syncthreads();
+    const int g = __builtin_amdgcn_readfirstlane(*word);
+    __syncthreads();
+    return g < (int)gridDim.x ? g : -1;
+}
+
 __device__ __forceinline__ void argmax_merge(float &v, int &i, float ov, int oi) {
     const bool take = (ov > v) | ((ov == v) & (oi < i));
     v = take ? ov : v;
@@ -85,7 +93,11 @@
 #define VSTAMP(acc) do { if (a.dbg) { vt1 = __builtin_readcyclecounter(); acc += vt1 - vt0; vt0 = vt1; } } while (0)
 
     int tile = blockIdx.x, s0 = 0, s1 = -1, ord = 0;
-    if (a.seg) { const ShGruSegD sg = a.seg[blockIdx.x]; tile = sg.tile; s0 = sg.s0; s1 = sg.s1; ord = sg.pad; }
+    if (a.seg) {
+        const int g = sh_take_piece(a.err + 1, (int *)smem);
+        if (g < 0) { if (tid == 0) __hip_atomic_store(a.err, 1u, __ATOMIC_RELAXED, __HIP_MEMORY_SCOPE_AGENT); return; }
+        const ShGruSegD sg = a.seg[g]; tile = sg.tile; s0 = sg.s0; s1 = sg.s1; ord = sg.pad;
+    }
     tile = __builtin_amdgcn_readfirstlane(tile); s0 = __builtin_amdgcn_readfirstlane(s0); s1 = __builtin_amdgcn_readfirstlane(s1);
     const int Tt = __builtin_amdgcn_readfirstlane(md.tile_T[tile]);
     if (s1 < 0) s1 = Tt;
@@ -451,7 +463,11 @@
     for (int j = tid; j < 65 * 16; j += NTH) sBias[j] = f.bfrag[((j >> 4) * 64 + ((j >> 2) & 3) * 16) * 4 + (j & 3)];
 
     int tile = blockIdx.x, s0 = 0, s1 = -1, ord = 0;
-    if (a.seg) { const ShGruSegD sg = a.seg[blockIdx.x]; tile = sg.tile; s0 = sg.s0; s1 = sg.s1; ord = sg.pad; }
+    if (a.seg) {
+        const int g = sh_take_piece(a.err + 1, (int *)smem);
+        if (g < 0) { if (tid == 0) __hip_atomic_store(a.err, 1u, __ATOMIC_RELAXED, __HIP_MEMORY_SCOPE_AGENT); return; }
+        const ShGruSegD sg = a.seg[g]; tile = sg.tile; s0 = sg.s0; s1 = sg.s1; ord = sg.pad;
+    }
     tile = __builtin_amdgcn_readfirstlane(tile); s0 = __builtin_amdgcn_readfirstlane(s0); s1 = __builtin_amdgcn_readfirstlane(s1);
     const int Tt = __builtin_amdgcn_readfirstlane(md.tile_T[tile]);
     if (s1 < 0) s1 = Tt;
diff --git a/scrappie_amd/csrc/sh_decode_teams.h b/scrappie_amd/csrc/sh_decode_teams.h
--- a/scrappie_amd/csrc/sh_decode_teams.h
+++ b/scrappie_amd/csrc/sh_decode_teams.h
@@ -72,7 +72,11 @@
     for (int j = tid; j < 65 * 16; j += SH_FVT_NTH) sBias[j] = f.bfrag[((j >> 4) * 64 + ((j >> 2) & 3) * 16) * 4 + (j & 3)];
 
     int tile = blockIdx.x, s0 = 0, s1 = -1, ord = 0;
-    if (a.seg) { const ShGruSegD sg = a.seg[blockIdx.x]; tile = sg.tile; s0 = sg.s0; s1 = sg.s1; ord = sg.pad; }
+    if (a.seg) {
+        const int g = sh_take_piece(a.err + 1, (int *)smem);
+        if (g < 0) { if (tid == 0) __hip_atomic_store(a.err, 1u, __ATOMIC_RELAXED, __HIP_MEMORY_SCOPE_AGENT); return; }
+        const ShGruSegD sg = a.seg[g]; tile = sg.tile; s0 = sg.s0; s1 = sg.s1; ord = sg.pad;
+    }
     tile = __builtin_amdgcn_readfirstlane(tile); s0 = __builtin_amdgcn_readfirstlane(s0); s1 = __builtin_amdgcn_readfirstlane(s1);
     const int Tt = __builtin_amdgcn_readfirstlane(md.tile_T[tile]);
     if (s1 < 0) s1 = Tt;
diff --git a/scrappie_amd/csrc/sh_eng_batch.inc b/scrappie_amd/csrc/sh_eng_batch.inc
--- a/scrappie_amd/csrc/sh_eng_batch.inc
+++ b/scrappie_amd/csrc/sh_eng_batch.inc
@@ -59,7 +59,7 @@
 }
 static void sync_helper(scrappie_hip_engine *e, scrappie_hip_engine *t) {
     t->handover = e->handover; t->max_launch_reads = e->max_launch_reads; t->max_launch_blocks = e->max_launch_blocks;
-    t->dbg_ff_separate = e->dbg_ff_separate; t->dbg_fv_single = e->dbg_fv_single; t->dbg_gru32 = e->dbg_gru32; t->dbg_gru_tiles = e->dbg_gru_tiles; t->dbg_redo_all = e->dbg_redo_all;
+    t->dbg_ff_separate = e->dbg_ff_separate; t->dbg_fv_single = e->dbg_fv_single; t->dbg_gru32 = e->dbg_gru32; t->dbg_gru_tiles = e->dbg_gru_tiles; t->dbg_sched_ncu = e->dbg_sched_ncu; t->dbg_redo_all = e->dbg_redo_all;
     t->profiling = false;
 }
 static scrappie_hip_engine *tail_engine(scrappie_hip_engine *e) {
diff --git a/scrappie_amd/csrc/sh_eng_debug.inc b/scrappie_amd/csrc/sh_eng_debug.inc
--- a/scrappie_amd/csrc/sh_eng_debug.inc
+++ b/scrappie_amd/csrc/sh_eng_debug.inc
@@ -20,6 +20,7 @@
     else if (!strcmp(name, "fail_run")) e->dbg_fail_run = value;
     else if (!strcmp(name, "redo_all")) e->dbg_redo_all = value != 0;
     else if (!strcmp(name, "gru_tiles")) e->dbg_gru_tiles = value;
+    else if (!strcmp(name, "sched_ncu")) e->dbg_sched_ncu = value > 0 ? value : 0;
     else if (!strcmp(name, "force_f32_layers")) e->dbg_force_f32 = value != 0;
 #ifdef SH_EXPERIMENTS
     else if (!strcmp(name, "gru32")) e->dbg_gru32 = value;
diff --git a/scrappie_amd/csrc/sh_eng_launch.inc b/scrappie_amd/csrc/sh_eng_launch.inc
--- a/scrappie_amd/csrc/sh_eng_launch.inc
+++ b/scrappie_amd/csrc/sh_eng_launch.inc
@@ -1,5 +1,11 @@
 
 struct MetaPtrs { ShMeta md; const long long *seq_off, *hp_off, *bases_off; ShGruLanes lanes, lanes1; ShGruPairs pairs, pairs2; const ShGruSegD *vseg; };
+
+enum { SH_FLAG_SLICES = 8 };
+static size_t flag_words(size_t ntile) { return (SH_FLAG_SLICES + 1) * ntile + 2; }
+static unsigned *flag_slice(const Slot &sl, int l) { return sl.d_gflag.as<unsigned>() + (size_t)(l % SH_FLAG_SLICES) * sl.lg.ntile; }
+static unsigned *flag_decoder(const Slot &sl) { return sl.d_gflag.as<unsigned>() + (size_t)SH_FLAG_SLICES * sl.lg.ntile; }
+static unsigned *flag_err(const Slot &sl) { return flag_decoder(sl) + sl.lg.ntile; }
 
 static int build_group(scrappie_hip_engine *e, Slot &sl, Model *m, const uint64_t *offsets, const uint32_t *lengths,
                        size_t n, bool hp_on, MetaPtrs &mp) {
@@ -40,16 +46,17 @@
         nseq += tile_T[t] ? ((long long)tile_T[t] + 1) * SH_SEQ_STRIDE : 0;
     }
     lg.ncb = ncb; lg.nseq = nseq; lg.nhp = nhp; lg.nbases_cap = nbases;
+    const int ncu = e->dbg_sched_ncu > 0 ? e->dbg_sched_ncu : e->ncu;
     ShGruSchedule sched;
-    sh_lane_schedule(tile_T.data(), lg.ntile, e->ncu, 2, sched, e->handover);
+    sh_lane_schedule(tile_T.data(), lg.ntile, ncu, 2, sched, e->handover);
     lg.gru_nwg = sched.nwg;
     ShGruSchedule sched1;
-    sh_lane_schedule(tile_T.data(), lg.ntile, e->ncu, 1, sched1, e->handover);
+    sh_lane_schedule(tile_T.data(), lg.ntile, ncu, 1, sched1, e->handover);
     lg.gru1_nwg = sched1.nwg;
     { long long nlive = 0; int tmax = 0; for (int t : tile_T) { nlive += t > 0; tmax = std::max(tmax, t); }
       const int w1 = sched1.wg_iter.empty() ? 0 : *std::max_element(sched1.wg_iter.begin(), sched1.wg_iter.end());
       const int w2 = sched.wg_iter.empty() ? 0 : *std::max_element(sched.wg_iter.begin(), sched.wg_iter.end());
-      lg.gru_two = nlive > e->ncu && tmax < 65536 && (double)w2 * tun().gru_two_ratio < (double)w1;
+      lg.gru_two = nlive > ncu && tmax < 65536 && (double)w2 * tun().gru_two_ratio < (double)w1;
       if (e->dbg_gru_tiles == 1) lg.gru_two = false;
       if (e->dbg_gru_tiles == 2 && tmax < 65536) lg.gru_two = true; }
     std::vector<int> pair_tile, pair_T;
@@ -60,13 +67,13 @@
         t += two ? 2 : 1;
     }
     ShGruSchedule sched32;
-    sh_lane_schedule(pair_T.data(), pair_T.size(), e->ncu, 1, sched32, e->handover);
+    sh_lane_schedule(pair_T.data(), pair_T.size(), ncu, 1, sched32, e->handover);
     lg.gru32_nwg = sched32.nwg;
     ShGruSchedule sched32b;
-    sh_lane_schedule(pair_T.data(), pair_T.size(), e->ncu, 2, sched32b, e->handover);
+    sh_lane_schedule(pair_T.data(), pair_T.size(), ncu, 2, sched32b, e->handover);
     lg.gru32x2_nwg = sched32b.nwg;
     std::vector<ShGruSeg> vseg;
-    sh_piece_schedule(tile_T.data(), lg.ntile, e->ncu, vseg, e->handover);
+    sh_piece_schedule(tile_T.data(), lg.ntile, ncu, vseg, e->handover, &sched1);
     lg.vit_nwg = (int)vseg.size();
     const size_t b_u64 = lg.npad * 8, b_i32 = lg.npad * 4;
     const size_t b_loff = sched.lane_off.size() * 4, b_seg = sched.seg.size() * sizeof(ShGruSeg), b_wit = sched.wg_iter.size() * 4;
@@ -121,12 +128,12 @@
     mp.lanes.seg = (const ShGruSegD *)(d + o_seg);
     mp.lanes.lane_off = (const int *)(d + o_loff);
     mp.lanes.wg_iter = (const int *)(d + o_wit);
-    mp.lanes.ntile = (int)lg.ntile;
     mp.vseg = (const ShGruSegD *)(d + o_vseg);
-    if (e->d_hstate.ensure(std::max<size_t>(lg.ntile, 1) * 12 * 256 * 4) || sl.d_gflag.ensure((lg.ntile + 1) * 4)) return -1;
+    if (e->d_hstate.ensure(std::max<size_t>(lg.ntile, 1) * 12 * 256 * 4) || sl.d_gflag.ensure(flag_words(lg.ntile) * 4)) return -1;
     mp.lanes.hstate = e->d_hstate.as<float>();
-    mp.lanes.flag = sl.d_gflag.as<unsigned>();
-    HIPCHK(hipMemsetAsync(sl.d_gflag.p, 0, (lg.ntile + 1) * 4, ps));
+    mp.lanes.flag = flag_slice(sl, 0);
+    mp.lanes.err_off = (int)(flag_err(sl) - flag_slice(sl, 0));
+    HIPCHK(hipMemsetAsync(sl.d_gflag.p, 0, flag_words(lg.ntile) * 4, ps));
     if (sl.d_bad.ensure(lg.npad * 4)) return -1;
     HIPCHK(hipMemsetAsync(sl.d_bad.p, 0, lg.npad * 4, ps));
     mp.lanes1 = mp.lanes;
@@ -138,7 +145,7 @@
     mp.pairs.pair_tile = (const int *)(d + o_pt);
     mp.pairs.hstate = mp.lanes.hstate;
     mp.pairs.flag = mp.lanes.flag;
-    mp.pairs.err = mp.lanes.flag + lg.ntile;
+    mp.pairs.err = flag_err(sl);
     mp.pairs2 = mp.pairs;
     mp.pairs2.seg = (const ShGruSegD *)(d + o_seg32b);
     mp.pairs2.lane_off = (const int *)(d + o_loff32b);
@@ -217,7 +224,6 @@
     int rc = 0;
     if (!tun().gru_single && !tun().gru_stamp && tun().gru_debug < 0 && NU <= 6 && S % 32 == 0) {
         if (nwg <= 0) return 0;
-        HIPCHK(hipMemsetAsync(lanes.flag, 0, (size_t)lanes.ntile * 4, s));
         dim3 lgrid((unsigned)nwg);
         const bool stamp = tun().gru_lanes_stamp;
         const bool f32_env = tun().gru_f32 || force_f32;
@@ -349,7 +355,6 @@
     const ShGruLanes &lanes = two ? lanes2 : lanes1;
     const int nwg = two ? nwg2 : nwg1;
     if (nwg <= 0) return 0;
-    HIPCHK(hipMemsetAsync(lanes.flag, 0, (size_t)lanes.ntile * 4, s));
     const size_t lds = (two ? 2 : 1) * ((size_t)4 * 3 * 2 * 64 * 4 + (size_t)2 * 3 * 6 * 256) * 4;
     dim3 grid((unsigned)nwg);
     if (tun().proj_stamp && two && kst == 3 && !act) {
@@ -375,7 +380,6 @@
     const ShGruLanes &lanes = two ? lanes2 : lanes1;
     const int nwg = two ? nwg2 : nwg1;
     if (nwg <= 0) return 0;
-    HIPCHK(hipMemsetAsync(lanes.flag, 0, (size_t)lanes.ntile * 4, s));
     const int NU = S / 16;
     size_t lds = (two ? 2 : 1) * ((size_t)4 * (NU / 2) * 2 * 64 * 4 + (size_t)2 * 3 * NU * 256) * 4;
     if (resid && SH_RESID_LDS && lds + (size_t)(two ? 2 : 1) * 3 * NU * 256 * 4 <= 160 * 1024) lds += (size_t)(two ? 2 : 1) * 3 * NU * 256 * 4;
@@ -469,9 +473,8 @@
 }
 static const char *const g32_role[8] = {"R0 chain", "R1 chain", "R2 chain", "C cand-proj", "G0 z/r", "G1 z/r", "G2 z/r", "L loader"};
 static int launch_gru_proj32x2(hipStream_t s, const float *in, float *out, bool resid, const unsigned *iW, const float *ib, const unsigned *sW,
-                               const unsigned *sW2, const ShMeta &md, int backward, const ShGruPairs &pairs, int nwg, size_t ntile) {
+                               const unsigned *sW2, const ShMeta &md, int backward, const ShGruPairs &pairs, int nwg) {
     if (nwg <= 0) return 0;
-    HIPCHK(hipMemsetAsync(pairs.flag, 0, ntile * 4, s));
     const size_t lds = (size_t)SH_G32X2_LDS_WORDS * 4;
     dim3 grid((unsigned)nwg);
     if (tun().gru32_stamp && !resid) {
@@ -489,9 +492,8 @@
     return pick_bool([&](auto rs) { return launch_k<k_gru_proj32x2<rs(), false>>(grid, dim3(512), lds, s, in, out, iW, ib, sW, sW2, md, backward, pairs, (unsigned long long *)nullptr); }, resid);
 }
 static int launch_gru_proj32(hipStream_t s, const float *in, float *out, bool resid, const unsigned *iW, const float *ib, const unsigned *sW,
-                             const unsigned *sW2, const ShMeta &md, int backward, const ShGruPairs &pairs, int nwg, size_t ntile) {
+                             const unsigned *sW2, const ShMeta &md, int backward, const ShGruPairs &pairs, int nwg) {
     if (nwg <= 0) return 0;
-    HIPCHK(hipMemsetAsync(pairs.flag, 0, ntile * 4, s));
     const size_t lds = (size_t)SH_G32_LDS_WORDS * 4;
     dim3 grid((unsigned)nwg);
     if (tun().gru32_stamp && !resid) {
@@ -516,7 +518,6 @@
 static int launch_lstm(hipStream_t s, int S, const float *xaff, float *out, const unsigned *sW, const float *pf,
                        const ShMeta &md, int backward, const ShGruLanes &lanes, int nwg) {
     if (nwg <= 0) return 0;
-    HIPCHK(hipMemsetAsync(lanes.flag, 0, (size_t)lanes.ntile * 4, s));
     int rc = 0;
     if (pick_int<2, 4, 6>(S / 16, rc, [&](auto nu) { return launch_k<k_lstm_lanes<nu()>>(dim3((unsigned)nwg), dim3(128 * nu()), 0, s, xaff, out, sW, pf, md, backward, lanes); })) return rc;
     return set_err("unsupported LSTM size %d (need 32, 64 or 96)", S);
@@ -525,7 +526,6 @@
 static int launch_lstm_proj(hipStream_t s, int S, int I, const float *in, float *out, const unsigned *iW, const float *ib,
                             const unsigned *sW, const float *pf, const ShMeta &md, int backward, const ShGruLanes &lanes, int nwg) {
     if (nwg <= 0) return 0;
-    HIPCHK(hipMemsetAsync(lanes.flag, 0, (size_t)lanes.ntile * 4, s));
     const int NU = S / 16;
     const size_t lds = ((size_t)4 * (NU / 2) * 2 * 64 * 4 + (size_t)2 * 4 * NU * 256 + (size_t)3 * NU * 256) * 4;
     if (I != S && I != 16) return set_err("unsupported LSTM input width %d", I);
diff --git a/scrappie_amd/csrc/sh_eng_load.inc b/scrappie_amd/csrc/sh_eng_load.inc
--- a/scrappie_amd/csrc/sh_eng_load.inc
+++ b/scrappie_amd/csrc/sh_eng_load.inc
@@ -254,7 +254,7 @@
                               &dbg_wait, &dbg_lead};
     for (auto &sp : sl.spans) {
         float ms = 0;
-        HIPCHK(hipEventElapsedTime(&ms, sl.ev[sp.i], sl.ev[sp.j]));
+        if (sp.i != sp.j) HIPCHK(hipEventElapsedTime(&ms, sl.ev[sp.i], sl.ev[sp.j]));
         *fields[sp.field] += ms;
     }
     sl.spans.clear();
diff --git a/scrappie_amd/csrc/sh_eng_pipeline.inc b/scrappie_amd/csrc/sh_eng_pipeline.inc
--- a/scrappie_amd/csrc/sh_eng_pipeline.inc
+++ b/scrappie_amd/csrc/sh_eng_pipeline.inc
@@ -29,6 +29,7 @@
         if (on && sl->nev < 48) { at[k] = sl->nev++; HIPCHK(hipEventRecord(sl->ev[at[k]], st)); }
         return 0;
     }
+    void same(Mark k, Mark as) { if (on) at[k] = at[as]; }
     void span(SpanField field, Mark from, Mark to) { if (on) sl->spans.push_back({field, at[from], at[to]}); }
 };
 
@@ -147,34 +148,38 @@
     return 0;
 }
 
-static int recurrent_layer(Slot &sl, Model *m, GroupRun &c, int l, int I, const float *in, float *out, int backward) {
+static int recurrent_layer(Slot &sl, Model *m, GroupRun &c, int l, int I, const float *in, float *out, int backward, bool follows_layer = false) {
     scrappie_hip_engine *e = c.e;
-    const LaunchGroup &lg = sl.lg; const MetaPtrs &mp = c.mp;
+    const LaunchGroup &lg = sl.lg;
+    MetaPtrs mp = c.mp;
+    mp.lanes.flag = mp.lanes1.flag = mp.pairs.flag = mp.pairs2.flag = flag_slice(sl, l);
+    mp.lanes.err_off = mp.lanes1.err_off = (int)(flag_err(sl) - flag_slice(sl, l));
     const hipStream_t s = c.s;
     const bool lstm = m->arch == 3;
     const int S = m->S, gates = lstm ? 4 : 3;
     const float *resid = m->arch == 1 ? in : nullptr;
     const bool f32 = !lstm && m->layer_f32[l];
     const bool one_kernel = !tun().gru_separate && (lstm ? (I == S || I == 16) && S % 32 == 0 : gru_proj_ok(I, S) && !f32);
-    if (c.pf.mark(Marks::LAYER_BEGIN, s)) return -1;
+    if (follows_layer) c.pf.same(Marks::LAYER_BEGIN, Marks::LAYER_END);
+    else if (c.pf.mark(Marks::LAYER_BEGIN, s)) return -1;
 #ifdef SH_EXPERIMENTS
     if (l == 0 && c.fuse_conv) {
-        if (c.pf.mark(Marks::LAYER_SPLIT, s)) return -1;
+        c.pf.same(Marks::LAYER_SPLIT, Marks::LAYER_BEGIN);
         ShConvFuse cf;
         cf.sig = c.d_signal; cf.W = m->conv_W.as<float>(); cf.bias = m->conv_b.as<float>(); cf.edge = sl.d_edge.as<int>();
         cf.bad = sl.d_bad.as<unsigned>(); cf.g = m->geom;
         if (launch_gru_conv(s, (m->WL + 3) / 4, m->conv_act, out, m->iWp[l].as<unsigned>(), m->ibs[l].as<float>(), m->sWp[l].as<unsigned>(),
                             m->sW2p[l].as<unsigned>(), mp.md, 1, mp.lanes1, lg.gru1_nwg, mp.lanes, lg.gru_nwg, lg.gru_two, cf)) return -1;
     } else if (!lstm && one_kernel && use_gru32(e) && S == 96 && I == 96 && m->has32) {
-        if (c.pf.mark(Marks::LAYER_SPLIT, s)) return -1;
+        c.pf.same(Marks::LAYER_SPLIT, Marks::LAYER_BEGIN);
         if (use_gru32(e) == 2 ? launch_gru_proj32x2(s, in, out, m->arch == 1, m->iWp32[l].as<unsigned>(), m->ib32[l].as<float>(), m->sWp32[l].as<unsigned>(),
-                                                    m->sW2p32[l].as<unsigned>(), mp.md, backward, mp.pairs2, lg.gru32x2_nwg, lg.ntile)
+                                                    m->sW2p32[l].as<unsigned>(), mp.md, backward, mp.pairs2, lg.gru32x2_nwg)
                               : launch_gru_proj32(s, in, out, m->arch == 1, m->iWp32[l].as<unsigned>(), m->ib32[l].as<float>(), m->sWp32[l].as<unsigned>(),
-                                                  m->sW2p32[l].as<unsigned>(), mp.md, backward, mp.pairs, lg.gru32_nwg, lg.ntile)) return -1;
+                                                  m->sW2p32[l].as<unsigned>(), mp.md, backward, mp.pairs, lg.gru32_nwg)) return -1;
     } else
 #endif
     if (one_kernel) {
-        if (c.pf.mark(Marks::LAYER_SPLIT, s)) return -1;
+        c.pf.same(Marks::LAYER_SPLIT, Marks::LAYER_BEGIN);
         if (lstm ? launch_lstm_proj(s, S, I, in, out, m->iWp[l].as<unsigned>(), m->ibs[l].as<float>(), m->sWp[l].as<unsigned>(), m->lp[l].as<float>(),
                                     mp.md, backward, mp.lanes1, lg.gru1_nwg)
                  : launch_gru_proj(s, S, in, out, resid, m->iWp[l].as<unsigned>(), m->ibs[l].as<float>(), m->sWp[l].as<unsigned>(), m->sW2p[l].as<unsigned>(),
@@ -206,7 +211,7 @@
     float **abuf = c.abuf; *top = 0;
     if (m->arch == 2 || m->arch == 3) {
         for (int lvl = 0; lvl < 2 && lvl < c.trunk_upto; lvl++) {
-            for (int dir = 0; dir < 2; dir++) if (recurrent_layer(sl, m, c, 2 * lvl + dir, lvl == 0 ? F : S, abuf[0], abuf[1 + dir], dir)) return -1;
+            for (int dir = 0; dir < 2; dir++) if (recurrent_layer(sl, m, c, 2 * lvl + dir, lvl == 0 ? F : S, abuf[0], abuf[1 + dir], dir, dir == 1)) return -1;
             if (c.pf.mark(Marks::LAYER_BEGIN, s)) return -1;
             if (launch_affine2(s, S, abuf[1], abuf[2], abuf[0], m->ff2W[lvl][0].as<unsigned>(), m->ff2W[lvl][1].as<unsigned>(), m->ff2b[lvl].as<float>(), c.ncb, S / 16)) return -1;
             if (c.pf.mark(Marks::LAYER_SPLIT, s)) return -1;
@@ -215,7 +220,7 @@
         }
     } else {
         for (int l = 0; l < 5 && l < c.trunk_upto; l++, *top ^= 1)
-            if (recurrent_layer(sl, m, c, l, l == 0 ? F : S, abuf[*top], abuf[*top ^ 1], (l % 2 == 0) ? 1 : 0)) return -1;
+            if (recurrent_layer(sl, m, c, l, l == 0 ? F : S, abuf[*top], abuf[*top ^ 1], (l % 2 == 0) ? 1 : 0, l > 0)) return -1;
     }
     HIPCHK(hipGetLastError());
     c.stamp("layers enqueued at");
@@ -251,7 +256,8 @@
     if (c.pf.mark(Marks::S1_BEGIN, s)) return -1;
     if (!fused && launch_ff(s, S, top, e->d_E.as<float>(), e->d_sums.as<float>(), m->ffWp.as<unsigned>(), m->ffbs.as<float>(),
                             ncb, mtiles, m->NS, p->tempW / p->tempb, p->tempb, e->ncu)) return -1;
-    if (c.pf.mark(Marks::S1_END, s)) return -1;
+    if (fused) c.pf.same(Marks::S1_END, Marks::S1_BEGIN);
+    else if (c.pf.mark(Marks::S1_END, s)) return -1;
     c.pf.span(F_FF, Marks::S1_BEGIN, Marks::S1_END);
     if (c.pf.on) sl.timing.ff_flops += 2.0 * S * m->NS * 16.0 * (double)ncb;
     const float *E_use = e->d_E.as<float>(), *sums_use = e->d_sums.as<float>();
@@ -280,10 +286,9 @@
     va.dump_final = e->dbg_dump_final ? 1 : 0;
     static StampBuf vst;
     if (tun().vit_stamp) va.dbg = vst.dev(4096 * 16 * 8);
-    if (e->d_vstate.ensure(std::max<size_t>(lg.ntile, 1) * ((size_t)NH * 16 + 32) * 4) || e->d_vflag.ensure(std::max<size_t>(lg.ntile, 1) * 4)) return -1;
-    HIPCHK(hipMemsetAsync(e->d_vflag.p, 0, std::max<size_t>(lg.ntile, 1) * 4, s));
+    if (e->d_vstate.ensure(std::max<size_t>(lg.ntile, 1) * ((size_t)NH * 16 + 32) * 4)) return -1;
     va.seg = mp.vseg;
-    va.vstate = e->d_vstate.as<float>(); va.flag = e->d_vflag.as<unsigned>(); va.err = sl.d_gflag.as<unsigned>() + lg.ntile;
+    va.vstate = e->d_vstate.as<float>(); va.flag = flag_decoder(sl); va.err = flag_err(sl);
     if (e->ev_ok && e->other(sl).pending) HIPCHK(hipStreamWaitEvent(s, e->other(sl).done, 0));
     if (fused) {
         ShFfArgs fa;
@@ -342,7 +347,8 @@
     const hipStream_t s = c.s, cs = c.cs;
     if (sl.h_score.ensure(lg.npad * 4)) return -1;
     if (sl.h_err.ensure(4) || sl.h_bad.ensure(lg.npad * 4)) return -1;
-    if (c.pf.mark(Marks::MAIN_END, s)) return -1;
+    if (!c.transducer || c.walk_on_cs) c.pf.same(Marks::MAIN_END, Marks::DECODE_END);
+    else if (c.pf.mark(Marks::MAIN_END, s)) return -1;
     c.pf.span(F_TOTAL, Marks::MAIN_BEGIN, Marks::MAIN_END);
     if (e->ev_ok && !c.walk_on_cs) { HIPCHK(hipEventRecord(sl.kdone, s)); HIPCHK(hipStreamWaitEvent(cs, sl.kdone, 0)); }
     lg.dev_stitch = !tun().host_stitch;
@@ -365,7 +371,7 @@
         ra.d_redo = sl.d_redo.as<unsigned>(); ra.h_redo = sl.h_redo.as<unsigned>();
         ra.d_score = sl.d_fscore.as<float>(); ra.h_score = sl.h_score.as<float>();
         ra.d_bad = sl.d_bad.as<unsigned>(); ra.h_bad = sl.h_bad.as<unsigned>();
-        ra.d_err = sl.d_gflag.as<unsigned>() + lg.ntile; ra.h_err = sl.h_err.as<unsigned>();
+        ra.d_err = flag_err(sl); ra.h_err = sl.h_err.as<unsigned>();
         ra.npad = (int)lg.npad;
         if (c.pf.mark(Marks::STITCH_BEGIN, cs)) return -1;
         if (c.fold_tail) {
@@ -390,7 +396,7 @@
         HIPCHK(hipMemcpyAsync(sl.h_seq.p, sl.d_seq.p, (size_t)lg.nseq * 4, hipMemcpyDeviceToHost, cs));
         if (c.hp_on) HIPCHK(hipMemcpyAsync(sl.h_hp.p, sl.d_hp.p, (size_t)lg.nhp * 5 * 4, hipMemcpyDeviceToHost, cs));
         HIPCHK(hipMemcpyAsync(sl.h_score.p, sl.d_fscore.p, lg.npad * 4, hipMemcpyDeviceToHost, cs));
-        HIPCHK(hipMemcpyAsync(sl.h_err.p, sl.d_gflag.as<unsigned>() + lg.ntile, 4, hipMemcpyDeviceToHost, cs));
+        HIPCHK(hipMemcpyAsync(sl.h_err.p, flag_err(sl), 4, hipMemcpyDeviceToHost, cs));
         HIPCHK(hipMemcpyAsync(sl.h_bad.p, sl.d_bad.p, lg.npad * 4, hipMemcpyDeviceToHost, cs));
     }
     HIPCHK(hipGetLastError());
diff --git a/scrappie_amd/csrc/sh_gru.h b/scrappie_amd/csrc/sh_gru.h
--- a/scrappie_amd/csrc/sh_gru.h
+++ b/scrappie_amd/csrc/sh_gru.h
@@ -131,7 +131,7 @@
     const int *wg_iter;
     float *hstate;
     unsigned *flag;
-    int ntile;
+    int err_off;
 };
 
 struct ShGruPairs {
@@ -193,8 +193,8 @@
     auto take_over = [&]() {
         h = (f32x4){0.f, 0.f, 0.f, 0.f};
         if (s > 0) {
-            if (!sh_wait_flag(L.flag + tile, (unsigned)NU, L.flag + L.ntile) && lane == 0)
-                __hip_atomic_store(L.flag + L.ntile, 1u, __ATOMIC_RELAXED, __HIP_MEMORY_SCOPE_AGENT);
+            if (!sh_wait_flag(L.flag + tile, (unsigned)NU, L.flag + L.err_off) && lane == 0)
+                __hip_atomic_store(L.flag + L.err_off, 1u, __ATOMIC_RELAXED, __HIP_MEMORY_SCOPE_AGENT);
             __builtin_amdgcn_fence(__ATOMIC_ACQUIRE, "agent");
             const float *hs = L.hstate + ((long long)tile * NU + u) * 256 + lane * 4;
 #pragma unroll
@@ -365,8 +365,8 @@
     auto take_over = [&]() {
         h = (f32x4){0.f, 0.f, 0.f, 0.f};
         if (s > 0) {
-            if (!sh_wait_flag(L.flag + tile, (unsigned)NU, L.flag + L.ntile) && lane == 0)
-                __hip_atomic_store(L.flag + L.ntile, 1u, __ATOMIC_RELAXED, __HIP_MEMORY_SCOPE_AGENT);
+            if (!sh_wait_flag(L.flag + tile, (unsigned)NU, L.flag + L.err_off) && lane == 0)
+                __hip_atomic_store(L.flag + L.err_off, 1u, __ATOMIC_RELAXED, __HIP_MEMORY_SCOPE_AGENT);
             __builtin_amdgcn_fence(__ATOMIC_ACQUIRE, "agent");
             const float *hs = L.hstate + ((long long)tile * NU + u) * 256 + lane * 4;
 #pragma unroll
@@ -806,8 +806,8 @@
         else myT2 = tl ? ((myT2 & 0xffffu) | ((unsigned)mt << 16)) : ((myT2 & 0xffff0000u) | ((unsigned)mt & 0xffffu));
         if (!c[tl].ok) return;
         if (c[tl].s > 0) {
-            if (!sh_wait_flag(L.flag + c[tl].tile, (unsigned)NU, L.flag + L.ntile) && lane == 0)
-                __hip_atomic_store(L.flag + L.ntile, 1u, __ATOMIC_RELAXED, __HIP_MEMORY_SCOPE_AGENT);
+            if (!sh_wait_flag(L.flag + c[tl].tile, (unsigned)NU, L.flag + L.err_off) && lane == 0)
+                __hip_atomic_store(L.flag + L.err_off, 1u, __ATOMIC_RELAXED, __HIP_MEMORY_SCOPE_AGENT);
             __builtin_amdgcn_fence(__ATOMIC_ACQUIRE, "agent");
             const float *hs = L.hstate + ((long long)c[tl].tile * NU + u) * 256 + lane * 4;
 #pragma unroll
diff --git a/scrappie_amd/csrc/sh_gru_free.h b/scrappie_amd/csrc/sh_gru_free.h
--- a/scrappie_amd/csrc/sh_gru_free.h
+++ b/scrappie_amd/csrc/sh_gru_free.h
@@ -167,8 +167,8 @@
         else myT2 = tl ? ((myT2 & 0xffffu) | ((unsigned)mt << 16)) : ((myT2 & 0xffff0000u) | ((unsigned)mt & 0xffffu));
         if (!c[tl].ok) return;
         if (c[tl].s > 0) {
-            if (!sh_wait_flag(L.flag + c[tl].tile, (unsigned)NU, L.flag + L.ntile) && lane == 0)
-                __hip_atomic_store(L.flag + L.ntile, 1u, __ATOMIC_RELAXED, __HIP_MEMORY_SCOPE_AGENT);
+            if (!sh_wait_flag(L.flag + c[tl].tile, (unsigned)NU, L.flag + L.err_off) && lane == 0)
+                __hip_atomic_store(L.flag + L.err_off, 1u, __ATOMIC_RELAXED, __HIP_MEMORY_SCOPE_AGENT);
             __builtin_amdgcn_fence(__ATOMIC_ACQUIRE, "agent");
             const float *hs = L.hstate + ((long long)c[tl].tile * NU + u) * 256 + lane * 4;
 #pragma unroll
diff --git a/scrappie_amd/csrc/sh_gru_mx.h b/scrappie_amd/csrc/sh_gru_mx.h
--- a/scrappie_amd/csrc/sh_gru_mx.h
+++ b/scrappie_amd/csrc/sh_gru_mx.h
@@ -176,8 +176,8 @@
         myT = co.ok ? md.rT[co.tile * 16 + (lane & 15)] : 0;
         if (!co.ok) return;
         if (co.s > 0) {
-            if (!sh_wait_flag(L.flag + co.tile, (unsigned)NU, L.flag + L.ntile) && lane == 0)
-                __hip_atomic_store(L.flag + L.ntile, 1u, __ATOMIC_RELAXED, __HIP_MEMORY_SCOPE_AGENT);
+            if (!sh_wait_flag(L.flag + co.tile, (unsigned)NU, L.flag + L.err_off) && lane == 0)
+                __hip_atomic_store(L.flag + L.err_off, 1u, __ATOMIC_RELAXED, __HIP_MEMORY_SCOPE_AGENT);
             __builtin_amdgcn_fence(__ATOMIC_ACQUIRE, "agent");
 #pragma unroll
             for (int k = 0; k < 3; k++) {
diff --git a/scrappie_amd/csrc/sh_lstm.h b/scrappie_amd/csrc/sh_lstm.h
--- a/scrappie_amd/csrc/sh_lstm.h
+++ b/scrappie_amd/csrc/sh_lstm.h
@@ -97,8 +97,8 @@
     auto take_over = [&]() {
         h = (f32x4){0.f, 0.f, 0.f, 0.f}; c = h;
         if (s > 0) {
-            if (!sh_wait_flag(L.flag + tile, (unsigned)NU, L.flag + L.ntile) && lane == 0)
-                __hip_atomic_store(L.flag + L.ntile, 1u, __ATOMIC_RELAXED, __HIP_MEMORY_SCOPE_AGENT);
+            if (!sh_wait_flag(L.flag + tile, (unsigned)NU, L.flag + L.err_off) && lane == 0)
+                __hip_atomic_store(L.flag + L.err_off, 1u, __ATOMIC_RELAXED, __HIP_MEMORY_SCOPE_AGENT);
             __builtin_amdgcn_fence(__ATOMIC_ACQUIRE, "agent");
             const float *hs = L.hstate + ((long long)tile * 2 * NU + u) * 256 + lane * 4;
 #pragma unroll
@@ -338,8 +338,8 @@
         if (!c.ok) return;
         myT = md.rT[c.tile * 16 + (lane & 15)];
         if (c.s > 0) {
-            if (!sh_wait_flag(L.flag + c.tile, (unsigned)NU, L.flag + L.ntile) && lane == 0)
-                __hip_atomic_store(L.flag + L.ntile, 1u, __ATOMIC_RELAXED, __HIP_MEMORY_SCOPE_AGENT);
+            if (!sh_wait_flag(L.flag + c.tile, (unsigned)NU, L.flag + L.err_off) && lane == 0)
+                __hip_atomic_store(L.flag + L.err_off, 1u, __ATOMIC_RELAXED, __HIP_MEMORY_SCOPE_AGENT);
             __builtin_amdgcn_fence(__ATOMIC_ACQUIRE, "agent");
             const float *hs = L.hstate + ((long long)c.tile * 2 * NU + u) * 256 + lane * 4;
 #pragma unroll
diff --git a/scrappie_amd/csrc/sh_sched.h b/scrappie_amd/csrc/sh_sched.h
--- a/scrappie_amd/csrc/sh_sched.h
+++ b/scrappie_amd/csrc/sh_sched.h
@@ -88,18 +88,28 @@
     return best;
 }
 static inline void sh_piece_schedule(const int *tile_T, size_t ntile, int ncu, std::vector<ShGruSeg> &seg,
-                                     bool allow_split = true) {
+                                     bool allow_split = true, const ShGruSchedule *sched1 = nullptr) {
     seg.clear();
     long long nlive = 0;
     for (size_t t = 0; t < ntile; t++) nlive += tile_T[t] > 0;
     const int K = allow_split ? sh_pieces_per_tile(nlive, ncu) : 1;
-    for (int k = 0; k < K; k++)
-        for (size_t t = 0; t < ntile; t++) {
-            const int T = tile_T[t];
-            if (T <= 0) continue;
-            const int len = (T + K - 1) / K;
-            const int s0 = std::min(T, k * len), s1 = std::min(T, (k + 1) * len);
-            if (s1 > s0) seg.push_back({(int)t, s0, s1, k});
+    if (K < 2) {
+        for (size_t t = 0; t < ntile; t++) if (tile_T[t] > 0) seg.push_back({(int)t, 0, tile_T[t], 0});
+        return;
+    }
+    ShGruSchedule own;
+    if (!sched1) { sh_lane_schedule(tile_T, ntile, ncu, 1, own); sched1 = &own; }
+    struct Piece { int start, lane; ShGruSeg sg; };
+    std::vector<Piece> pc;
+    for (int ln = 0; ln + 1 < (int)sched1->lane_off.size(); ln++) {
+        int t0 = 0;
+        for (int i = sched1->lane_off[ln]; i < sched1->lane_off[ln + 1]; i++) {
+            const ShGruSeg &sg = sched1->seg[i];
+            pc.push_back({t0, ln, {sg.tile, sg.s0, sg.s1, sg.s0 > 0 ? 1 : 0}});
+            t0 += sg.s1 - sg.s0;
         }
+    }
+    std::stable_sort(pc.begin(), pc.end(), [](const Piece &x, const Piece &y) { return x.start != y.start ? x.start < y.start : x.lane < y.lane; });
+    for (const Piece &p : pc) seg.push_back(p.sg);
 }
 #endif
```
